# PeterouZh/CIPS-3D

Measured on AMD Instinct MI355X. Metric: rendered imgs/sec (G fwd+bwd), higher is better.
Workload: dtype f32 (dense layers as 3-pass split-operand MFMA with fp32 accumulate: SIREN forward on fp16 hi/lo planes, ~2e-7 rel., sigma in the fp32 class; INR head and all backward GEMMs on bf16 hi/lo planes, ~5e-6 rel. per layer; everything else fp32); 1 GPU; FFHQ r64, 24 SIREN evals/ray (num_steps 24, hierarchical False), batch 32/GPU, G fwd+bwd, all 9 CIPS blocks; global_batch=32, parallelism=dp1, rccl_ranks=0, inr_gemm_mode=bf16x3, launch=hipGraph replay, grad_reduce=none

## Files before the change

cips3d_amd/_lib.py:

```python
import ctypes as C
import os

_HERE = os.path.dirname(os.path.abspath(__file__))
LIB_PATH = os.path.join(_HERE, "lib", "libcips3d_hip.so")

vp = C.c_void_p
i32 = C.c_int
i64 = C.c_longlong
f32 = C.c_float


class SirenWeights(C.Structure):
    _fields_ = [(n, vp) for n in
                ("w0", "b0", "w1", "b1", "ws", "bs", "wc", "bc", "wf", "bf",
                 "g0", "p0", "g1", "p1", "gc", "pc")] + [("box_scale", f32), ("trig_mode", i32)]


class SirenGrads(C.Structure):
    _fields_ = [(n, vp) for n in ("dg0", "dp0", "dg1", "dp1", "dgc", "dpc", "dw0", "db0", "dw1", "db1", "dws", "dbs", "dwc",
                                  "dbc", "dwf", "dbf")]


class RayParams(C.Structure):
    _fields_ = [("xg", vp), ("yg", vp), ("zg", vp), ("cam2world", vp), ("jitter", vp), ("zvals", vp), ("zc", f32), ("H", i32),
                ("W", i32), ("S", i32)]


class GlinJob(C.Structure):
    _fields_ = [("x", vp), ("w", vp), ("bias", vp), ("y", vp), ("dy", vp), ("dw", vp), ("db", vp), ("in_dim", i32),
                ("out_dim", i32)]


class GemmDesc(C.Structure):
    _fields_ = [
        ("A", vp), ("B", vp), ("C", vp),
        ("M", i32), ("N", i32), ("K", i32),
        ("lda", i32), ("ldb", i32), ("ldc", i32),
        ("strideA", i64), ("strideB", i64), ("strideC", i64),
        ("batch", i32), ("a_kmajor", i32), ("b_nmajor", i32),
        ("alpha", f32), ("bias", vp), ("bias_m", vp),
        ("act", i32), ("slope", f32), ("act_gain", f32),
        ("resid", vp), ("C2", vp), ("add", vp),
        ("rgb_g", vp), ("rgb_w", vp), ("C_unmasked", vp), ("mask", vp),
    ]


class ModfcPrepJob(C.Structure):
    _fields_ = [("weight", C.c_void_p), ("s", C.c_void_p), ("wb_hi", C.c_void_p), ("wb_lo", C.c_void_p),
                ("wbt_hi", C.c_void_p), ("wbt_lo", C.c_void_p), ("demod", C.c_void_p), ("in_dim", C.c_int),
                ("out_dim", C.c_int)]


class ModfcBwdJob(C.Structure):
    _fields_ = [("weight", C.c_void_p), ("s", C.c_void_p), ("demod", C.c_void_p), ("gwb", C.c_void_p),
                ("cbuf", C.c_void_p), ("dweight", C.c_void_p), ("ds", C.c_void_p), ("in_dim", C.c_int),
                ("out_dim", C.c_int)]


class GemmX3Desc(C.Structure):
    _fields_ = [
        ("A_hi", vp), ("A_lo", vp), ("B_hi", vp), ("B_lo", vp),
        ("M", i32), ("N", i32), ("K", i32), ("lda", i32), ("ldb", i32),
        ("strideA", i64), ("strideB", i64), ("batch", i32),
        ("C", vp), ("ldc", i32), ("strideC", i64),
        ("P_hi", vp), ("P_lo", vp), ("ldp", i32), ("strideP", i64),
        ("T_hi", vp), ("T_lo", vp), ("ldt", i32), ("strideT", i64),
        ("mask_out", vp), ("add", vp), ("rgb_g", vp), ("rgb_w", vp), ("C_unmasked", vp), ("mask", vp),
        ("act", i32), ("slope", f32), ("res_hi", vp), ("res_lo", vp), ("gate_bits", i32),
        ("torgb_w", vp), ("torgb_part", vp),
        ("addp_hi", vp), ("addp_lo", vp), ("addp_gate", vp), ("addp_gain", f32),
        ("kernel", i32),
    ]


class ConvX3Desc(C.Structure):
    _fields_ = [("w_hi", vp), ("w_lo", vp), ("x_hi", vp), ("x_lo", vp), ("y", vp),
                ("B", i32), ("C", i32), ("H", i32), ("W", i32), ("O", i32), ("kh", i32), ("kw", i32),
                ("stride", i32), ("pad", i32), ("ksplit", i32), ("part", vp), ("bias", vp), ("act", i32), ("slope", f32),
                ("act_scale", f32)]


class ConvDgradS2Desc(C.Structure):
    _fields_ = [("w_hi", vp), ("w_lo", vp), ("dy_hi", vp), ("dy_lo", vp), ("dxp", vp),
                ("B", i32), ("C", i32), ("H", i32), ("W", i32), ("O", i32), ("kh", i32), ("kw", i32),
                ("w_off", i64 * 4), ("out_off", i64 * 4)]


class WPrepJob(C.Structure):
    _fields_ = [("w", vp), ("fwd_hi", vp), ("fwd_lo", vp), ("alt_hi", vp), ("alt_lo", vp), ("scale", f32),
                ("O", i32), ("C", i32), ("kh", i32), ("kw", i32), ("alt_kind", i32), ("bank_off", i32 * 4)]


class ConvWgradDesc(C.Structure):
    _fields_ = [("dy_hi", vp), ("dy_lo", vp), ("x_hi", vp), ("x_lo", vp), ("part", vp),
                ("B", i32), ("C", i32), ("H", i32), ("W", i32), ("O", i32), ("kh", i32), ("kw", i32),
                ("stride", i32), ("pad", i32), ("nchunks", i32)]


SIGNATURES = {
    "cips_version": (i32, []),
    "cips_arch": (C.c_char_p, []),
    "cips_rays_fwd": (i32, [vp, vp, vp, f32, vp, vp, vp, vp, vp, i32, i32, i32, i32, vp]),
    "cips_siren_fwd": (i32, [C.POINTER(SirenWeights), vp, vp, vp, i32, i32, vp]),
    "cips_siren_fwd_x3": (i32, [C.POINTER(SirenWeights), vp, vp, vp, i32, i32, vp]),
    "cips_siren_bwd_rows": (i32, [i32, i32]),
    "cips_siren_bwd_x3_chunks": (i32, [i32, i32]),
    "cips_siren_bwd_x3_gpart": (i32, []),
    "cips_siren_bwd_x3_sred": (i32, []),
    "cips_siren_bwd_x3": (i32, [C.POINTER(SirenWeights), vp, vp, vp, vp, vp, i32, i32, vp]),
    "cips_siren_fwd_x3_rays": (i32, [C.POINTER(SirenWeights), C.POINTER(RayParams), vp, vp, vp, i32, vp]),
    "cips_siren_bwd_x3_rays": (i32, [C.POINTER(SirenWeights), C.POINTER(RayParams), vp, vp, vp, vp, i32, vp]),
    "cips_siren_bwd_x3_finalize": (i32, [C.POINTER(SirenWeights), vp, vp, i32, i32, C.POINTER(SirenGrads), vp]),
    "cips_march_fwd_x3": (i32, [C.POINTER(SirenWeights), C.POINTER(RayParams), vp, f32, i32, i32, vp, vp, vp, vp, vp, vp, i32, vp, vp, vp]),
    "cips_siren_bwd_data": (i32, [C.POINTER(SirenWeights)] + [vp] * 14 + [i32, i32, vp]),
    "cips_siren_bwd_data_f32": (i32, [C.POINTER(SirenWeights)] + [vp] * 9 + [i32, i32, vp]),
    "cips_resample_fwd": (i32, [vp, vp, vp, f32, vp, vp, vp, vp, vp, vp, vp, vp, i32, i32, i32, i32, vp, C.POINTER(RayParams), vp]),
    "cips_composite_fwd": (i32, [vp, vp, vp, vp, vp, vp, vp, f32, vp, vp, vp, vp, vp, i32, i32, i32, i32, vp, vp, vp]),
    "cips_composite_bwd": (i32, [vp, vp, vp, vp, vp, vp, vp, f32, vp, vp, vp, vp, vp, vp, i32, i32, i32, i32, vp, vp]),
    "cips_gemm_f32": (i32, [C.POINTER(GemmDesc), vp]),
    "cips_gemm_bf16x3": (i32, [C.POINTER(GemmX3Desc), vp]),
    "cips_gemm_bf16x3_fuses_torgb": (i32, [C.POINTER(GemmX3Desc)]),
    "cips_gemm_bf16x3_takes_addp": (i32, [C.POINTER(GemmX3Desc)]),
    "cips_torgb_finish": (i32, [vp, i32, vp, vp, i64, i32, vp]),
    "cips_equal_linear_scratch": (i64, [i32, i32, i32, i32]),
    "cips_equal_linear": (i32, [i32, vp, vp, vp, f32, f32, vp, vp, i32, i32, i32, vp]),
    "cips_gemm_bf16x3_km": (i32, [C.POINTER(GemmX3Desc), vp]),
    "cips_gemm_bf16x3_km_grouped": (i32, [C.POINTER(GemmX3Desc), i32, vp]),
    "cips_gemm_bf16": (i32, [C.POINTER(GemmX3Desc), vp]),
    "cips_gemm_bf16_fuses_torgb": (i32, [C.POINTER(GemmX3Desc)]),
    "cips_gemm_bf16_takes_addp": (i32, [C.POINTER(GemmX3Desc)]),
    "cips_gemm_bf16_km": (i32, [C.POINTER(GemmX3Desc), vp]),
    "cips_gemm_bf16_km_grouped": (i32, [C.POINTER(GemmX3Desc), i32, vp]),
    "cips_lrelu_bwd_bias_slices": (i32, [i32]),
    "cips_lrelu_bwd_bias": (i32, [vp, vp, vp, vp, i64, i32, f32, f32, vp]),
    "cips_lrelu_bwd_bias_finish": (i32, [vp, vp, i32, i32, i32, vp]),
    "cips_lrelu_bwd_bias_nhwc_tiles": (i32, [i32]),
    "cips_lrelu_bwd_bias_nhwc": (i32, [vp, vp, vp, vp, vp, i32, i32, i32, f32, f32, vp]),
    "cips_conv1x1_smallk": (i32, [vp, vp, vp, i32, i32, i32, i32, vp]),
    "cips_conv1x1_smallk_bwd_data": (i32, [vp, vp, vp, i32, i32, i32, i32, vp]),
    "cips_conv1x1_smallk_bwd_weight_splits": (i32, [i32, i32]),
    "cips_conv1x1_smallk_bwd_weight": (i32, [vp, vp, vp, i32, i32, i32, i32, vp]),
    "cips_conv2d_x3": (i32, [C.POINTER(ConvX3Desc), vp]),
    "cips_conv2d_x3_wgrad": (i32, [C.POINTER(ConvWgradDesc), vp]),
    "cips_split_planes": (i32, [vp, vp, vp, vp, vp, i32, i32, i32, i32, i32, i32, i64, i64, i64, vp]),
    "cips_split_planes_nhwc": (i32, [vp, vp, vp, i32, i32, i32, vp]),
    "cips_conv2d_x3_ksplit": (i32, [i32, i32, i32, i32]),
    "cips_conv_weight_prep_max_jobs": (i32, []),
    "cips_conv_weight_prep_batch": (i32, [C.POINTER(WPrepJob), i32, vp]),
    "cips_conv2d_x3_dgrad_s2": (i32, [C.POINTER(ConvDgradS2Desc), vp]),
    "cips_conv_wgrad_finish": (i32, [vp, vp, i32, i32, i32, i32, f32, vp]),
    "cips_modfc_prep_x3": (i32, [vp, vp, vp, vp, vp, vp, vp, i32, i32, i32, f32, vp]),
    "cips_torgb_fwd_x3": (i32, [vp, vp, vp, vp, vp, i64, i32, i32, vp]),
    "cips_torgb_bwd_w_x3": (i32, [vp, vp, vp, vp, vp, vp, i64, i32, vp]),
    "cips_modfc_prep": (i32, [vp, vp, vp, vp, vp, i32, i32, i32, f32, vp]),
    "cips_modfc_prep_bwd": (i32, [vp, vp, vp, vp, vp, vp, vp, i32, i32, i32, vp]),
    "cips_modfc_max_jobs": (i32, []),
    "cips_modfc_prep_x3_batch": (i32, [C.POINTER(ModfcPrepJob), i32, i32, C.c_float, vp]),
    "cips_modfc_prep_bwd_batch": (i32, [C.POINTER(ModfcBwdJob), i32, i32, vp]),
    "cips_modfc_prep_bwd_batch_cores": (i32, [C.POINTER(ModfcBwdJob), i32, i32, vp]),
    "cips_cores_colsum_parts": (i32, []),
    "cips_opt_chunk": (i32, []),
    "cips_opt_step": (i32, [vp, vp, vp, i32, vp, vp, f32, f32, f32, f32, f32, f32, i32, vp, vp]),
    "cips_camera_pose": (i32, [vp, vp, i32, f32, f32, f32, f32, vp, vp, vp, i32, vp]),
    "cips_grouped_linear_max_jobs": (i32, []),
    "cips_grouped_linear_fwd": (i32, [C.POINTER(GlinJob), i32, i32, vp]),
    "cips_grouped_linear_scratch": (i64, [C.POINTER(GlinJob), i32, i32]),
    "cips_grouped_linear_bwd": (i32, [C.POINTER(GlinJob), i32, i32, vp, vp, i64, vp]),
    "cips_rownorm_fwd": (i32, [vp, vp, vp, vp, vp, i32, i32, i32, f32, vp]),
    "cips_rownorm_bwd": (i32, [vp] * 9 + [i32, i32, i32, f32, vp]),
    "cips_torgb_fwd": (i32, [vp, vp, vp, vp, i64, i32, i32, vp]),
    "cips_torgb_bwd_partials": (i32, [i64]),
    "cips_torgb_bwd_w": (i32, [vp, vp, vp, vp, vp, i64, i32, vp]),
    "cips_torgb_bwd_x": (i32, [vp, vp, vp, vp, f32, vp, vp, i64, i32, vp]),
    "cips_torgb_bwd_w_x3_batch": (i32, [vp, vp, i32, vp, vp, vp, vp, i64, i32, vp]),
    "cips_torgb_bwd_w_x3_batch_cores": (i32, [vp, vp, i32, vp, vp, vp, vp, i64, i32, vp]),
    "cips_torgb_bwd_x_x3": (i32, [vp, vp, vp, f32, vp, vp, vp, i64, i32, vp]),
    "cips_fused_bias_act": (i32, [vp, vp, vp, vp, i64, i32, i32, i32, i32, f32, f32, vp]),
    "cips_diffaug": (i32, [vp] * 10 + [i32] * 8 + [vp]),
    "cips_avgpool2": (i32, [vp, vp, i64, i32, i32, i32, vp]),
    "cips_axpby": (i32, [vp, vp, vp, f32, f32, i64, vp]),
    "cips_image_to_u8": (i32, [vp, vp, i32, i32, i32, i32, f32, f32, vp]),
    "cips_upfirdn2d": (i32, [vp, vp, vp] + [i32] * 14 + [vp]),
    "cips_upfirdn2d_parity": (i32, [vp, C.POINTER(i64 * 4), vp, vp] + [i32] * 7 + [vp]),
    "cips_im2col": (i32, [vp, vp] + [i32] * 8 + [vp]),
    "cips_im2col_x3": (i32, [vp, vp, vp, i32, i32, i32, i32, i32, i32, i32, i32, vp]),
    "cips_col2im": (i32, [vp, vp] + [i32] * 8 + [vp]),
}

_lib = None


def load():
    global _lib
    if _lib is not None:
        return _lib
    if not os.path.exists(LIB_PATH):
        raise RuntimeError(
            f"cips3d_amd: HIP extension not built ({LIB_PATH} missing). "
            "Run `python -m cips3d_amd.build` (needs hipcc). There is no CPU fallback.")
    lib = C.CDLL(LIB_PATH)
    for name, (res, args) in SIGNATURES.items():
        try:
            fn = getattr(lib, name)
        except AttributeError as e:
            raise RuntimeError(f"cips3d_amd: symbol {name} missing from {LIB_PATH}") from e
        fn.restype = res
        fn.argtypes = args
    _lib = lib
    return lib


def check(err, what):
    if err != 0:
        raise RuntimeError(f"cips3d_amd: {what} failed with hipError {err}")
```

cips3d_amd/csrc/render.hip:

```cpp
#include "common.h"
#include "../../include/cips3d_hip.h"
#include "raygen.h"

namespace {

__global__ __launch_bounds__(256) void rays_kernel(const float* __restrict__ xg, const float* __restrict__ yg,
                                                   const float* __restrict__ zg, float zc,
                                                   const float* __restrict__ c2w, const float* __restrict__ jitter,
                                                   float* __restrict__ points, float* __restrict__ zout,
                                                   float* __restrict__ dirs, int B, int H, int W, int S) {
  const long long total = (long long)B * H * W * S;
  const int n = H * W;
  for (long long idx = (long long)blockIdx.x * blockDim.x + threadIdx.x; idx < total;
       idx += (long long)gridDim.x * blockDim.x) {
    const int i = (int)(idx % S);
    const long long rr = idx / S;
    const int ray = (int)(rr % n);
    const int b = (int)(rr / n);
    const int row = ray / W, col = ray % W;
    const float x = xg[col], y = yg[row];
    const float nrm = sqrtf(x * x + y * y + zc * zc);
    const float dx = x / nrm, dy = y / nrm, dz = zc / nrm;
    float z = zg[i];
    float px = dx * z, py = dy * z, pz = dz * z;
    if (jitter) {
      const float off = (jitter[idx] - 0.5f) * (zg[1] - zg[0]);
      z = z + off;
      px = px + off * dx; py = py + off * dy; pz = pz + off * dz;
    }
    const float* M = c2w + (long long)b * 16;
    points[idx * 3 + 0] = ((M[0] * px + M[1] * py) + M[2] * pz) + M[3];
    points[idx * 3 + 1] = ((M[4] * px + M[5] * py) + M[6] * pz) + M[7];
    points[idx * 3 + 2] = ((M[8] * px + M[9] * py) + M[10] * pz) + M[11];
    zout[idx] = z;
    if (i == 0) {
      dirs[rr * 3 + 0] = (M[0] * dx + M[1] * dy) + M[2] * dz;
      dirs[rr * 3 + 1] = (M[4] * dx + M[5] * dy) + M[6] * dz;
      dirs[rr * 3 + 2] = (M[8] * dx + M[9] * dy) + M[10] * dz;
    }
  }
}

__device__ __forceinline__ float clamp_density(float x, int mode) {
  if (mode == 1) return (x > 20.f) ? x : log1pf(expf(x));
  return fmaxf(x, 0.f);
}
__device__ __forceinline__ float clamp_density_grad(float x, int mode) {
  if (mode == 1) return (x > 20.f) ? 1.f : 1.f / (1.f + expf(-x));
  return x > 0.f ? 1.f : 0.f;
}

struct ResampleArgs {
  const float *sigma, *z, *noise, *u, *origins, *dirs;
  const float* cdf_in;
  RayGen rg;
  int have_rg;
  float noise_std;
  float *fine_z, *fine_pts, *weights_out, *cdf_out;
  long long* inds_out;
  int B, n, S, clamp_mode;
};

constexpr int SEG = 8;

__global__ __launch_bounds__(256) void resample_kernel(ResampleArgs a) {
  extern __shared__ __attribute__((aligned(16))) float sm[];
  const int S = a.S;
  const int rays_per_block = blockDim.x / SEG;
  const int lr = threadIdx.x / SEG, sub = threadIdx.x % SEG;
  const long long R = (long long)a.B * a.n;
  const long long ray_raw = (long long)blockIdx.x * rays_per_block + lr;
  const bool active = ray_raw < R;
  const long long ray = active ? ray_raw : R - 1;
  float* zs = sm + lr * (4 * S);
  float* ws = zs + S;
  float* cdf = ws + S;
  float* bins = cdf + S;

  for (int i = sub; i < S; i += SEG) {
    zs[i] = a.z[ray * S + i];
    float sg = a.sigma[ray * S + i];
    if (a.noise) sg += a.noise[ray * S + i] * a.noise_std;
    ws[i] = sg;
  }
  __syncthreads();
  if (sub == 0) {
    double T = 1.0;
    for (int i = 0; i < S; ++i) {
      const float delta = (i + 1 < S) ? (zs[i + 1] - zs[i]) : 1e10f;
      const float dens = clamp_density(ws[i], a.clamp_mode);
      const float alpha = 1.f - expf(-delta * dens);
      const float Tf = (float)T;
      T *= (double)(1.f - alpha + 1e-10f);
      ws[i] = alpha * Tf;
    }
    float sum = 0.f;
    for (int k = 0; k < S - 2; ++k) sum += (ws[k + 1] + 1e-5f) + 1e-5f;
    double acc = 0.0;
    cdf[0] = 0.f;
    for (int k = 0; k < S - 2; ++k) {
      const float pdf = ((ws[k + 1] + 1e-5f) + 1e-5f) / sum;
      acc += (double)pdf;
      cdf[k + 1] = (float)acc;
    }
    for (int j = 0; j < S - 1; ++j) bins[j] = 0.5f * (zs[j] + zs[j + 1]);
    if (a.cdf_in)
      for (int j = 0; j < S - 1; ++j) cdf[j] = a.cdf_in[ray * (S - 1) + j];
  }
  __syncthreads();
  const int b = (int)(ray / a.n);
  float ox, oy, oz, dx, dy, dz;
  if (a.have_rg) {
    const float* M = a.rg.c2w + (long long)b * 16;
    const RayDir d = ray_dir(a.rg, (int)(ray - (long long)b * a.n));
    dx = (M[0] * d.dx + M[1] * d.dy) + M[2] * d.dz;
    dy = (M[4] * d.dx + M[5] * d.dy) + M[6] * d.dz;
    dz = (M[8] * d.dx + M[9] * d.dy) + M[10] * d.dz;
    ox = M[3]; oy = M[7]; oz = M[11];
  } else {
    ox = a.origins[b * 3 + 0]; oy = a.origins[b * 3 + 1]; oz = a.origins[b * 3 + 2];
    dx = a.dirs[ray * 3 + 0]; dy = a.dirs[ray * 3 + 1]; dz = a.dirs[ray * 3 + 2];
  }
  for (int i = sub; i < S; i += SEG) {
    const float u = a.u[ray * S + i];
    int ind = 0;
    for (int j = 0; j < S - 1; ++j) ind += (cdf[j] < u) ? 1 : 0;
    const int below = max(ind - 1, 0);
    const int above = min(ind, S - 2);
    const float c0 = cdf[below], c1 = cdf[above];
    const float b0 = bins[below], b1 = bins[above];
    float denom = c1 - c0;
    if (denom < 1e-5f) denom = 1.f;
    const float smp = b0 + (u - c0) / denom * (b1 - b0);
    if (!active) continue;
    a.fine_z[ray * S + i] = smp;
    if (a.fine_pts) {
      float* fp = a.fine_pts + (ray * S + i) * 3;
      fp[0] = ox + dx * smp; fp[1] = oy + dy * smp; fp[2] = oz + dz * smp;
    }
    if (a.inds_out) a.inds_out[ray * S + i] = ind;
    if (a.weights_out) a.weights_out[ray * S + i] = ws[i];
  }
  if (a.cdf_out && active)
    for (int j = sub; j < S - 1; j += SEG) a.cdf_out[ray * (S - 1) + j] = cdf[j];
}

struct CompArgs {
  const float *feat_c, *sig_c, *z_c, *feat_f, *sig_f, *z_f, *noise;
  float noise_std;
  float *fea, *depth, *weights, *zsorted;
  int* order;
  const int* order_in;
  const float* dfea;
  float *dfeat_c, *dsig_c, *dfeat_f, *dsig_f;
  long long R;
  int S, E, clamp_mode, flags;
  const unsigned char* clamp_pin;
  unsigned char* clamp_rec;
};

__device__ __forceinline__ bool clamp_pass(const CompArgs& a, float x, long long idx, bool store) {
  bool pass = x > 0.f;
  if (a.clamp_pin) pass = a.clamp_pin[idx] != 0;
  if (a.clamp_rec && store) a.clamp_rec[idx] = pass ? 1 : 0;
  return pass;
}

__device__ __forceinline__ const float* feat_row(const CompArgs& a, long long ray, int i) {
  if (a.feat_f) return (i < a.S) ? a.feat_f + (ray * a.S + i) * 32 : a.feat_c + (ray * a.S + (i - a.S)) * 32;
  return a.feat_c + (ray * a.S + i) * 32;
}

__global__ __launch_bounds__(256) void composite_fwd_kernel(CompArgs a) {
  extern __shared__ __attribute__((aligned(16))) float sm[];
  const int S = a.S, E = a.E;
  const int rays_per_block = blockDim.x / SEG;
  const int lr = threadIdx.x / SEG, sub = threadIdx.x % SEG;
  const long long ray_raw = (long long)blockIdx.x * rays_per_block + lr;
  const bool active = ray_raw < a.R;
  const long long ray = active ? ray_raw : a.R - 1;
  float* zall = sm + lr * (4 * E);
  float* sall = zall + E;
  int* ord = reinterpret_cast<int*>(sall + E);

  for (int i = sub; i < E; i += SEG) {
    if (a.feat_f) {
      zall[i] = (i < S) ? a.z_f[ray * S + i] : a.z_c[ray * S + (i - S)];
      sall[i] = (i < S) ? a.sig_f[ray * S + i] : a.sig_c[ray * S + (i - S)];
    } else {
      zall[i] = a.z_c[ray * S + i];
      sall[i] = a.sig_c[ray * S + i];
      ord[i] = i;
    }
  }
  __syncthreads();
  if (a.feat_f) {
    for (int i = sub; i < E; i += SEG) {
      const float zi = zall[i];
      int rank = 0;
      for (int j = 0; j < E; ++j) {
        const float zj = zall[j];
        rank += (zj < zi || (zj == zi && j < i)) ? 1 : 0;
      }
      ord[rank] = i;
    }
  }
  __syncthreads();

  float* al = reinterpret_cast<float*>(ord + E);
  for (int k = sub; k < E; k += SEG) {
    const int i = ord[k];
    const float zk = zall[i];
    const float delta = (k + 1 < E) ? (zall[ord[k + 1]] - zk) : 1e10f;
    float sg = sall[i];
    if (a.noise) sg += a.noise[ray * E + k] * a.noise_std;
    float dens = clamp_density(sg, a.clamp_mode);
    if ((a.clamp_pin || a.clamp_rec) && a.clamp_mode == 0) dens = clamp_pass(a, sg, ray * E + k, active) ? sg : 0.f;
    al[k] = 1.f - expf(-delta * dens);
  }
  __syncthreads();

  float4 F = make_float4(0.f, 0.f, 0.f, 0.f);
  float depth = 0.f, wsum = 0.f, wlast = 0.f, zlast = 0.f;
  float4 flast = make_float4(0.f, 0.f, 0.f, 0.f);
  double T = 1.0;
  for (int k0 = 0; k0 < E; k0 += 8) {
    float4 f[8];
#pragma unroll
    for (int j = 0; j < 8; ++j) {
      const int k = (k0 + j < E) ? k0 + j : E - 1;
      f[j] = *reinterpret_cast<const float4*>(feat_row(a, ray, ord[k]) + 4 * sub);
    }
#pragma unroll
    for (int j = 0; j < 8; ++j) {
      const int k = k0 + j;
      if (k < E) {
        const int i = ord[k];
        const float zk = zall[i];
        const float alpha = al[k];
        const float w = alpha * (float)T;
        T *= (double)(1.f - alpha + 1e-10f);
        F.x = fmaf(w, f[j].x, F.x); F.y = fmaf(w, f[j].y, F.y); F.z = fmaf(w, f[j].z, F.z); F.w = fmaf(w, f[j].w, F.w);
        depth = fmaf(w, zk, depth);
        wsum += w;
        if (k == E - 1) { wlast = w; zlast = zk; flast = f[j]; }
        if ((k % SEG) == sub && active) {
          if (a.weights && !(k == E - 1 && (a.flags & 1))) a.weights[ray * E + k] = w;
          if (a.order) a.order[ray * E + k] = i;
          if (a.zsorted) a.zsorted[ray * E + k] = zk;
        }
      }
    }
  }
  if (a.flags & 1) {
    const float extra = 1.f - wsum;
    F.x = fmaf(extra, flast.x, F.x); F.y = fmaf(extra, flast.y, F.y);
    F.z = fmaf(extra, flast.z, F.z); F.w = fmaf(extra, flast.w, F.w);
    depth = fmaf(extra, zlast, depth);
    if (a.weights && ((E - 1) % SEG) == sub && active) a.weights[ray * E + E - 1] = wlast + extra;
  }
  if (a.flags & 2) {
    const float extra = 1.f - wsum;
    F.x += extra; F.y += extra; F.z += extra; F.w += extra;
  }
  if (active) {
    *reinterpret_cast<float4*>(a.fea + ray * 32 + 4 * sub) = F;
    if (sub == 0 && a.depth) a.depth[ray] = depth;
  }
}

__global__ __launch_bounds__(256) void composite_bwd_kernel(CompArgs a) {
  extern __shared__ __attribute__((aligned(16))) float sm[];
  const int S = a.S, E = a.E;
  const int rays_per_block = blockDim.x / SEG;
  const int lr = threadIdx.x / SEG, sub = threadIdx.x % SEG;
  const long long ray_raw = (long long)blockIdx.x * rays_per_block + lr;
  const bool active = ray_raw < a.R;
  const long long ray = active ? ray_raw : a.R - 1;
  float* zall = sm + lr * (6 * E);
  float* xs = zall + E;
  float* Ts = xs + E;
  float* al = Ts + E;
  float* ss = al + E;
  int* ord = reinterpret_cast<int*>(ss + E);

  for (int k = sub; k < E; k += SEG) {
    const int i = a.order_in ? a.order_in[ray * E + k] : k;
    ord[k] = i;
    float zz, sg;
    if (a.feat_f) {
      zz = (i < S) ? a.z_f[ray * S + i] : a.z_c[ray * S + (i - S)];
      sg = (i < S) ? a.sig_f[ray * S + i] : a.sig_c[ray * S + (i - S)];
    } else {
      zz = a.z_c[ray * S + i];
      sg = a.sig_c[ray * S + i];
    }
    if (a.noise) sg += a.noise[ray * E + k] * a.noise_std;
    zall[k] = zz;
    xs[k] = sg;
  }
  __syncthreads();

  const float4 G = *reinterpret_cast<const float4*>(a.dfea + ray * 32 + 4 * sub);
  float gsum = G.x + G.y + G.z + G.w;
  gsum += __shfl_xor(gsum, 1);
  gsum += __shfl_xor(gsum, 2);
  gsum += __shfl_xor(gsum, 4);
  float wsum = 0.f;
  double T = 1.0;
  for (int k = 0; k < E; ++k) {
    const float delta = (k + 1 < E) ? (zall[k + 1] - zall[k]) : 1e10f;
    float dens = clamp_density(xs[k], a.clamp_mode);
    if (a.clamp_pin && a.clamp_mode == 0) dens = a.clamp_pin[ray * E + k] ? xs[k] : 0.f;
    const float alpha = 1.f - expf(-delta * dens);
    const float Tf = (float)T;
    wsum += alpha * Tf;
    T *= (double)(1.f - alpha + 1e-10f);
    const float4 f = *reinterpret_cast<const float4*>(feat_row(a, ray, ord[k]) + 4 * sub);
    float s = G.x * f.x + G.y * f.y + G.z * f.z + G.w * f.w;
    s += __shfl_xor(s, 1);
    s += __shfl_xor(s, 2);
    s += __shfl_xor(s, 4);
    if (sub == 0) { Ts[k] = Tf; al[k] = alpha; ss[k] = s; }
  }
  __syncthreads();
  float Q = 0.f;
  const float s_off = ((a.flags & 1) ? ss[E - 1] : 0.f) + ((a.flags & 2) ? gsum : 0.f);
  for (int k = E - 1; k >= 0; --k) {
    const int i = ord[k];
    const float alpha = al[k], Tk = Ts[k], s = ss[k] - s_off;
    float w = alpha * Tk;
    if ((a.flags & 1) && k == E - 1) w += 1.f - wsum;

    const float dalpha = Tk * (s - Q);
    Q = fmaf(alpha, s, (1.f - alpha + 1e-10f) * Q);
    float* drow;
    float* dsg;
    if (a.feat_f) {
      drow = (i < S) ? a.dfeat_f + (ray * S + i) * 32 : a.dfeat_c + (ray * S + (i - S)) * 32;
      dsg = (i < S) ? a.dsig_f + ray * S + i : a.dsig_c + ray * S + (i - S);
    } else {
      drow = a.dfeat_c + (ray * S + i) * 32;
      dsg = a.dsig_c + ray * S + i;
    }
    if (active) *reinterpret_cast<float4*>(drow + 4 * sub) = make_float4(w * G.x, w * G.y, w * G.z, w * G.w);
    if ((k % SEG) == sub && active) {
      const float delta = (k + 1 < E) ? (zall[k + 1] - zall[k]) : 1e10f;
      const float x = xs[k];
      float dens = clamp_density(x, a.clamp_mode);
      float dgrad = clamp_density_grad(x, a.clamp_mode);
      if (a.clamp_pin && a.clamp_mode == 0) {
        const bool pass = a.clamp_pin[ray * E + k] != 0;
        dens = pass ? x : 0.f;
        dgrad = pass ? 1.f : 0.f;
      }
      *dsg = dalpha * (delta * expf(-delta * dens)) * dgrad;
    }
  }
}

inline int rays_per_block_for(size_t bytes_per_ray) {
  int r = 32;
  while (r > 1 && (size_t)r * bytes_per_ray > 60 * 1024) r >>= 1;
  return r;
}

}

extern "C" int cips_rays_fwd(const float* xg, const float* yg, const float* zg, float zc,
                             const float* cam2world, const float* jitter, float* points, float* z,
                             float* dirs, int B, int H, int W, int S, cips_stream_t stream) {
  if (B <= 0 || H <= 0 || W <= 0 || S <= 1) return (int)hipErrorInvalidValue;
  long long total = (long long)B * H * W * S;
  int blocks = (int)((total + 255) / 256 < 8192 ? (total + 255) / 256 : 8192);
  hipLaunchKernelGGL(rays_kernel, dim3(blocks), dim3(256), 0, (hipStream_t)stream, xg, yg, zg, zc,
                     cam2world, jitter, points, z, dirs, B, H, W, S);
  return CIPS_CHECK_LAUNCH();
}

extern "C" int cips_resample_fwd(const float* sigma, const float* z, const float* noise, float noise_std,
                                 const float* u, const float* origins, const float* dirs, float* fine_z,
                                 float* fine_pts, float* weights_out, float* cdf_out, long long* inds_out,
                                 int B, int n, int S, int clamp_mode, const float* cdf_in, const cips_ray_params* rays,
                                 cips_stream_t stream) {
  if (B <= 0 || n <= 0 || S < 3 || !fine_z || (!rays && (!origins || !dirs || !fine_pts))) return (int)hipErrorInvalidValue;
  ResampleArgs a;
  a.cdf_in = cdf_in;
  a.rg = RayGen{}; a.have_rg = 0;
  if (rays) { const int rc = fill_raygen(a.rg, rays); if (rc) return rc; if (a.rg.n != n) return (int)hipErrorInvalidValue; a.have_rg = 1; }
  a.sigma = sigma; a.z = z; a.noise = noise; a.noise_std = noise_std; a.u = u; a.origins = origins;
  a.dirs = dirs; a.fine_z = fine_z; a.fine_pts = fine_pts; a.weights_out = weights_out;
  a.cdf_out = cdf_out; a.inds_out = inds_out; a.B = B; a.n = n; a.S = S; a.clamp_mode = clamp_mode;
  size_t per_ray = (size_t)4 * S * sizeof(float);
  int rpb = rays_per_block_for(per_ray);
  long long R = (long long)B * n;
  int blocks = (int)((R + rpb - 1) / rpb);
  hipLaunchKernelGGL(resample_kernel, dim3(blocks), dim3(rpb * SEG), rpb * per_ray, (hipStream_t)stream, a);
  return CIPS_CHECK_LAUNCH();
}

extern "C" int cips_composite_fwd(const float* feat_c, const float* sig_c, const float* z_c,
                                  const float* feat_f, const float* sig_f, const float* z_f,
                                  const float* noise, float noise_std, float* fea, float* depth,
                                  float* weights, int* order, float* zsorted, int R, int S,
                                  int clamp_mode, int flags, const unsigned char* clamp_in, unsigned char* clamp_out,
                                  cips_stream_t stream) {
  if (R <= 0 || S <= 0) return (int)hipErrorInvalidValue;
  CompArgs a = {};
  a.feat_c = feat_c; a.sig_c = sig_c; a.z_c = z_c; a.feat_f = feat_f; a.sig_f = sig_f; a.z_f = z_f;
  a.noise = noise; a.noise_std = noise_std; a.fea = fea; a.depth = depth; a.weights = weights;
  a.order = order; a.zsorted = zsorted; a.R = R; a.S = S; a.E = feat_f ? 2 * S : S;
  a.clamp_mode = clamp_mode; a.flags = flags;
  a.clamp_pin = clamp_in; a.clamp_rec = clamp_out;
  size_t per_ray = (size_t)4 * a.E * sizeof(float);
  int rpb = rays_per_block_for(per_ray);
  int blocks = (R + rpb - 1) / rpb;
  hipLaunchKernelGGL(composite_fwd_kernel, dim3(blocks), dim3(rpb * SEG), rpb * per_ray, (hipStream_t)stream, a);
  return CIPS_CHECK_LAUNCH();
}

extern "C" int cips_composite_bwd(const float* feat_c, const float* sig_c, const float* z_c,
                                  const float* feat_f, const float* sig_f, const float* z_f,
                                  const float* noise, float noise_std, const int* order, const float* dfea,
                                  float* dfeat_c, float* dsig_c, float* dfeat_f, float* dsig_f, int R, int S,
                                  int clamp_mode, int flags, const unsigned char* clamp_in, cips_stream_t stream) {
  if (R <= 0 || S <= 0 || (!order && feat_f)) return (int)hipErrorInvalidValue;
  CompArgs a = {};
  a.feat_c = feat_c; a.sig_c = sig_c; a.z_c = z_c; a.feat_f = feat_f; a.sig_f = sig_f; a.z_f = z_f;
  a.noise = noise; a.noise_std = noise_std; a.order_in = order; a.dfea = dfea;
  a.dfeat_c = dfeat_c; a.dsig_c = dsig_c; a.dfeat_f = dfeat_f; a.dsig_f = dsig_f;
  a.R = R; a.S = S; a.E = feat_f ? 2 * S : S; a.clamp_mode = clamp_mode; a.flags = flags;
  a.clamp_pin = clamp_in; a.clamp_rec = nullptr;
  size_t per_ray = (size_t)6 * a.E * sizeof(float);
  int rpb = rays_per_block_for(per_ray);
  int blocks = (R + rpb - 1) / rpb;
  hipLaunchKernelGGL(composite_bwd_kernel, dim3(blocks), dim3(rpb * SEG), rpb * per_ray, (hipStream_t)stream, a);
  return CIPS_CHECK_LAUNCH();
}
```

cips3d_amd/csrc/siren_bwd_x3.hip:

```cpp
#include "common.h"
#include "../../include/cips3d_hip.h"
#include "raygen.h"
#include <type_traits>

#ifdef CIPS_X3_PRIO
#define X3_PRIO(p) __builtin_amdgcn_s_setprio(p)
#else
#define X3_PRIO(p)
#endif

namespace {

typedef __bf16 bf16x8 __attribute__((ext_vector_type(8)));
typedef __bf16 bf16x2 __attribute__((ext_vector_type(2)));
typedef float f32x2 __attribute__((ext_vector_type(2)));
typedef short short4v __attribute__((ext_vector_type(4)));
typedef unsigned int u32x4 __attribute__((ext_vector_type(4)));
typedef unsigned char uchar;

constexpr int H = 128, HC = 64, CF = 32;

constexpr int O_W1H = 0, O_W1L = 32768;
constexpr int O_WCH = 65536, O_WCL = 81920;
constexpr int O_WFH = 98304, O_WFL = 102400;
// ... 151 lines not shown
    acc[m] = __builtin_amdgcn_mfma_f32_32x32x16_bf16(ah, bh, acc[m], 0, 0, 0);
    __builtin_amdgcn_sched_barrier(0);
    side(3 * it + 2);
    __builtin_amdgcn_sched_barrier(0);
  }
}

__device__ __forceinline__ unsigned opaque(unsigned v) { asm volatile("" : "+v"(v)); return v; }

struct LaneAddr {
  unsigned fb[2][2];
  unsigned tb[2][2];
  unsigned sb[2];
  unsigned ab;
  unsigned v16, v64;
};
__device__ __forceinline__ LaneAddr lane_addr(int lane, unsigned sbase) {
  const int l31 = lane & 31, hf = lane >> 5, s16 = lane & 15, mhalf = (lane >> 4) & 1;
  const int ul = 4 * mhalf + (s16 & 3);
  LaneAddr A;
  const int e = hf ^ ((l31 >> 2) & 7);
#pragma unroll
  for (int t = 0; t < 2; ++t)
#pragma unroll
    for (int sec = 0; sec < 2; ++sec) {
      A.fb[t][sec] = sbase + l31 * 64 + ((e ^ (4 * t) ^ (2 * sec)) << 3);
      A.tb[t][sec] = sbase + (4 * hf + (s16 >> 2)) * 64 + (((ul ^ hf) ^ (4 * t) ^ (2 * sec)) << 3);
    }
  const int gs = 4 * hf + (s16 >> 3);
  A.sb[0] = opaque(sbase + O_STG + (8 * hf + (s16 >> 2)) * 64 + ((ul ^ gs) << 3));
  A.sb[1] = opaque(sbase + O_STG + (8 * hf + (s16 >> 2)) * 64 + ((ul ^ gs ^ 2) << 3));
  A.ab = opaque(sbase + O_AUX + (8 * hf + (s16 >> 2)) * 16 + (s16 & 1) * 8);
  A.v16 = opaque(sbase + O_L0 + 16 * hf);
  A.v64 = opaque(sbase + O_L0 + 64 * hf);
  return A;
}

template <int NM, int Q, int R, int IMG, int PLANE, bool F16 = false>
__device__ __forceinline__ void layer_fwd(const LaneAddr& A, const Act<Q>& in, f32x16 (&acc)[NM]) {
  const unsigned b[2][2] = {{opaque(A.fb[0][0] + IMG), opaque(A.fb[0][1] + IMG)}, {opaque(A.fb[1][0] + IMG), opaque(A.fb[1][1] + IMG)}};
  auto load = [&](int s, int m, Frag& f) {
    const int c = (s >> 1) * R * 64 + m * 2048;
    put(f.h, 0, lds_b64(b[s & 1][0] + c));
    put(f.h, 2, lds_b64(b[s & 1][1] + c));
    put(f.l, 0, lds_b64(b[s & 1][0] + c + PLANE));
    put(f.l, 2, lds_b64(b[s & 1][1] + c + PLANE));
  };
  run_layer<NM, 2 * Q, F16>(load, in, acc);
}

template <int NM, int Q, int R, int IMG, int PLANE, typename SideF>
__device__ __forceinline__ void layer_fwd_mm(const LaneAddr& A, const Act<Q>& in, f32x16 (&acc)[NM], SideF side) {
  const unsigned b[2][2] = {{opaque(A.fb[0][0] + IMG), opaque(A.fb[0][1] + IMG)}, {opaque(A.fb[1][0] + IMG), opaque(A.fb[1][1] + IMG)}};
  auto load = [&](int s, int m, Frag& f) {
    const int c = (s >> 1) * R * 64 + m * 2048;
    put(f.h, 0, lds_b64(b[s & 1][0] + c));
    put(f.h, 2, lds_b64(b[s & 1][1] + c));
    put(f.l, 0, lds_b64(b[s & 1][0] + c + PLANE));
    put(f.l, 2, lds_b64(b[s & 1][1] + c + PLANE));
  };
  run_layer_mm<NM, 2 * Q>(load, in, acc, side);
}

template <int NM, int KS, int R, int IMG, int PLANE>
__device__ __forceinline__ void layer_tr(const LaneAddr& A, const Act<(KS + 1) / 2>& in, f32x16 (&acc)[NM]) {
  const unsigned b[2][2] = {{opaque(A.tb[0][0] + IMG), opaque(A.tb[0][1] + IMG)}, {opaque(A.tb[1][0] + IMG), opaque(A.tb[1][1] + IMG)}};
  auto load = [&](int ks, int m, Frag& f) {
    const int c = m * R * 64 + ks * 1024;
    put(f.h, 0, lds_tr(b[ks & 1][0] + c));
    put(f.h, 2, lds_tr(b[ks & 1][1] + c + 512));
    put(f.l, 0, lds_tr(b[ks & 1][0] + c + PLANE));
    put(f.l, 2, lds_tr(b[ks & 1][1] + c + 512 + PLANE));
  };
  run_layer<NM, KS>(load, in, acc);
}

template <int NM, int KS, int R, int IMG, int PLANE, typename SideF>
__device__ __forceinline__ void layer_tr_mm(const LaneAddr& A, const Act<(KS + 1) / 2>& in, f32x16 (&acc)[NM], SideF side) {
  const unsigned b[2][2] = {{opaque(A.tb[0][0] + IMG), opaque(A.tb[0][1] + IMG)}, {opaque(A.tb[1][0] + IMG), opaque(A.tb[1][1] + IMG)}};
  auto load = [&](int ks, int m, Frag& f) {
    const int c = m * R * 64 + ks * 1024;
    put(f.h, 0, lds_tr(b[ks & 1][0] + c));
    put(f.h, 2, lds_tr(b[ks & 1][1] + c + 512));
    put(f.l, 0, lds_tr(b[ks & 1][0] + c + PLANE));
    put(f.l, 2, lds_tr(b[ks & 1][1] + c + 512 + PLANE));
  };
  run_layer_mm<NM, KS>(load, in, acc, side);
}

template <int Q, int R, int HI, int LO>
__device__ __forceinline__ void stage(unsigned sbase, int row, int hf, const Act<Q>& v) {
  const unsigned rb = opaque(sbase + O_STG + row * 64);
  const int g = (row >> 1) & 7;
#pragma unroll
  for (int gg = 0; gg < 4; ++gg) {
    const unsigned o = rb + (((2 * gg + hf) ^ g) << 3);
#pragma unroll
    for (int q = 0; q < Q; ++q) {
      lds_st64(o + HI + q * R * 64, v.hi[q][2 * gg], v.hi[q][2 * gg + 1]);
      lds_st64(o + LO + q * R * 64, v.lo[q][2 * gg], v.lo[q][2 * gg + 1]);
    }
  }
}

template <int R, int HI, int LO>
__device__ __forceinline__ void stg_frag(unsigned sb0, unsigned sb1, int col0, int ks, Frag& f) {
  const int c = (col0 >> 5) * R * 64 + ks * 1024;
  put(f.h, 0, lds_tr(sb0 + HI + c)); put(f.h, 2, lds_tr(sb1 + HI + c + 256));
  put(f.l, 0, lds_tr(sb0 + LO + c)); put(f.l, 2, lds_tr(sb1 + LO + c + 256));
}
__device__ __forceinline__ f32x16 x3f(f32x16 acc, const Frag& a, const Frag& b) {
  return x3(acc, mk8(a.h[0], a.h[1], a.h[2], a.h[3]), mk8(a.l[0], a.l[1], a.l[2], a.l[3]),
            mk8(b.h[0], b.h[1], b.h[2], b.h[3]), mk8(b.l[0], b.l[1], b.l[2], b.l[3]));
}

template <bool HW>
__device__ __forceinline__ void bsincos(float x, float* s, float* c) {
  if (HW) {
    float rv = x * CIPS_INV_2PI;
    rv = rv - rintf(rv);
    *s = __builtin_amdgcn_sinf(rv);
    *c = __builtin_amdgcn_cosf(rv);
  } else {
    sincos_reduced(reduce_2pi(x), s, c);
  }
}

__device__ __forceinline__ void aux_frag(unsigned ab, int ks, unsigned mask, Frag& f) {
  const int c = ks * 256;
  put(f.h, 0, lds_tr(ab + c)); put(f.h, 2, lds_tr(ab + c + 64));
  put(f.l, 0, lds_tr(ab + c + 2048)); put(f.l, 2, lds_tr(ab + c + 2048 + 64));
#pragma unroll
  for (int i = 0; i < 4; ++i) { f.h[i] &= mask; f.l[i] &= mask; }
}
__device__ __forceinline__ f32x16 x2f(f32x16 acc, const Frag& a, const Frag& b) {
  const bf16x8 bh = mk8(b.h[0], b.h[1], b.h[2], b.h[3]);
  acc = __builtin_amdgcn_mfma_f32_32x32x16_bf16(mk8(a.l[0], a.l[1], a.l[2], a.l[3]), bh, acc, 0, 0, 0);
  acc = __builtin_amdgcn_mfma_f32_32x32x16_bf16(mk8(a.h[0], a.h[1], a.h[2], a.h[3]), bh, acc, 0, 0, 0);
  return acc;
}
__device__ __forceinline__ float4 ld4(const float* p) { return *reinterpret_cast<const float4*>(p); }

struct BwdX3Args {
  cips_siren_weights w;
  const float* points;
  const float* dfeat;
  const float* dsigma;
  float* sred;
  float* gpart;
  int B, P, chunk, chunks;
  unsigned long long* prof;
  int dbg;
  RayGen rg;
};
constexpr int GP_G1 = 0, GP_GC = H * H, GP_GF0 = GP_GC + HC * H, GP_GF1 = GP_GF0 + CF * HC, GPART = GP_GF1 + CF * HC;
constexpr int SRED = 4 * 32 * 8 + 8;

__device__ __forceinline__ float pow2_scale_for(float m, int& k) {
  const unsigned u = __float_as_uint(m);
  const int e = (int)((u >> 23) & 0xffu) - 127;
  k = 13 - e;
  if (!(m > 0.f) || e == 128) k = 0;
  k = k > 100 ? 100 : (k < -100 ? -100 : k);
  return __uint_as_float((unsigned)(k + 127) << 23);
}
template <bool PRE = false, bool F16 = false>
__device__ __forceinline__ void stage_weights_x3(uchar* sm, const cips_siren_weights& w, int b) {
  const int tid = threadIdx.x, nt = blockDim.x;
  const float pre = PRE ? CIPS_INV_2PI : 1.f;
  float s1 = 1.f, sc = 1.f, sf = 1.f, i1 = 1.f, ic = 1.f, isf = 1.f;
  if constexpr (F16) {
    float m1 = 0.f, mc = 0.f, mf = 0.f;
    for (int i = tid; i < H * 32; i += nt) {
      const float4 v = *reinterpret_cast<const float4*>(w.w1 + 4 * i);
      m1 = fmaxf(fmaxf(m1, fmaxf(fabsf(v.x), fabsf(v.y))), fmaxf(fabsf(v.z), fabsf(v.w)));
    }
    for (int i = tid; i < HC * 32; i += nt) {
      const float4 v = *reinterpret_cast<const float4*>(w.wc + 4 * i);
      mc = fmaxf(fmaxf(mc, fmaxf(fabsf(v.x), fabsf(v.y))), fmaxf(fabsf(v.z), fabsf(v.w)));
    }
    for (int i = tid; i < CF * 16; i += nt) {
      const float4 v = *reinterpret_cast<const float4*>(w.wf + 4 * i);
      mf = fmaxf(fmaxf(mf, fmaxf(fabsf(v.x), fabsf(v.y))), fmaxf(fabsf(v.z), fabsf(v.w)));
    }
#pragma unroll
    for (int o = 32; o > 0; o >>= 1) {
      m1 = fmaxf(m1, __shfl_xor(m1, o)); mc = fmaxf(mc, __shfl_xor(mc, o)); mf = fmaxf(mf, __shfl_xor(mf, o));
    }
    float* red = reinterpret_cast<float*>(sm + O_W1H);
    const int wv = tid >> 6, nw = nt >> 6;
    if ((tid & 63) == 0) { red[3 * wv] = m1; red[3 * wv + 1] = mc; red[3 * wv + 2] = mf; }
    __syncthreads();
    m1 = 0.f; mc = 0.f; mf = 0.f;
    for (int i = 0; i < nw; ++i) { m1 = fmaxf(m1, red[3 * i]); mc = fmaxf(mc, red[3 * i + 1]); mf = fmaxf(mf, red[3 * i + 2]); }
    __syncthreads();
    int k1, kc, kf;
    s1 = pow2_scale_for(m1 * pre, k1); sc = pow2_scale_for(mc * pre, kc); sf = pow2_scale_for(mf, kf);
    i1 = __uint_as_float((unsigned)(127 - k1) << 23); ic = __uint_as_float((unsigned)(127 - kc) << 23);
    isf = __uint_as_float((unsigned)(127 - kf) << 23);
  }
  for (int i = tid; i < H * 32; i += nt) {
    const int row = i >> 5, u = i & 31;
    float4 v = *reinterpret_cast<const float4*>(w.w1 + row * H + 4 * u);
    if (PRE) { v.x *= pre; v.y *= pre; v.z *= pre; v.w *= pre; }
    if (F16) { v.x *= s1; v.y *= s1; v.z *= s1; v.w *= s1; }
    uint2 ph, pl;
    split2t<F16>(v.x, v.y, ph.x, pl.x); split2t<F16>(v.z, v.w, ph.y, pl.y);
    const int o = img_addr<2>(row, u, H);
    *reinterpret_cast<uint2*>(sm + O_W1H + o) = ph;
    *reinterpret_cast<uint2*>(sm + O_W1L + o) = pl;
  }
  for (int i = tid; i < HC * 32; i += nt) {
    const int row = i >> 5, u = i & 31;
    float4 v = *reinterpret_cast<const float4*>(w.wc + row * H + 4 * u);
    if (PRE) { v.x *= pre; v.y *= pre; v.z *= pre; v.w *= pre; }
    if (F16) { v.x *= sc; v.y *= sc; v.z *= sc; v.w *= sc; }
    uint2 ph, pl;
    split2t<F16>(v.x, v.y, ph.x, pl.x); split2t<F16>(v.z, v.w, ph.y, pl.y);
    const int o = img_addr<2>(row, u, HC);
    *reinterpret_cast<uint2*>(sm + O_WCH + o) = ph;
    *reinterpret_cast<uint2*>(sm + O_WCL + o) = pl;
  }
  for (int i = tid; i < CF * 16; i += nt) {
    const int row = i >> 4, u = i & 15;
    float4 v = *reinterpret_cast<const float4*>(w.wf + row * HC + 4 * u);
    if (F16) { v.x *= sf; v.y *= sf; v.z *= sf; v.w *= sf; }
    uint2 ph, pl;
    split2t<F16>(v.x, v.y, ph.x, pl.x); split2t<F16>(v.z, v.w, ph.y, pl.y);
    const int o = img_addr<2>(row, u, CF);
    *reinterpret_cast<uint2*>(sm + O_WFH + o) = ph;
    *reinterpret_cast<uint2*>(sm + O_WFL + o) = pl;
  }
  float* L0 = reinterpret_cast<float*>(sm + O_L0);
  float* G1 = reinterpret_cast<float*>(sm + O_G1); float* C1 = reinterpret_cast<float*>(sm + O_C1);
  float* WS = reinterpret_cast<float*>(sm + O_WS);
  float* GC = reinterpret_cast<float*>(sm + O_GC); float* CC = reinterpret_cast<float*>(sm + O_CC);
  for (int f = tid; f < H; f += nt) {
    const float g0 = w.g0[b * H + f], gs = g0 * w.box_scale;
    float4 pk;
    pk.x = gs * w.w0[f * 3 + 0]; pk.y = gs * w.w0[f * 3 + 1]; pk.z = gs * w.w0[f * 3 + 2];
    pk.w = fmaf(g0, w.b0[f], w.p0[b * H + f]);
    if (PRE) { pk.x *= pre; pk.y *= pre; pk.z *= pre; pk.w *= pre; }
    reinterpret_cast<float4*>(L0)[f] = pk;
    const float g1 = w.g1[b * H + f];
    G1[f] = F16 ? g1 * i1 : g1; C1[f] = fmaf(g1, w.b1[f], w.p1[b * H + f]) * pre; WS[f] = w.ws[f];
  }
  for (int f = tid; f < HC; f += nt) {
    const float gc = w.gc[b * HC + f];
    GC[f] = F16 ? gc * ic : gc; CC[f] = fmaf(gc, w.bc[f], w.pc[b * HC + f]) * pre;
  }
  if (F16 && tid == 0) *reinterpret_cast<float*>(sm + O_AUX + 128) = isf;
}

#ifdef CIPS_TUNING
#define X3_TS(i)                                                                                   \
  __builtin_amdgcn_sched_barrier(0);                                                               \
  if (a.prof && blockIdx.x == 0 && blockIdx.y == 0 && lane0 == 0 && rnd < 8)                       \
    a.prof[(rnd * 4 + wave) * 16 + (i)] = __builtin_amdgcn_s_memtime();                            \
  __builtin_amdgcn_sched_barrier(0);
#else
#define X3_TS(i) __builtin_amdgcn_sched_barrier(0);
#endif

#include "siren_bwd_x4.inc"
#define X3F_TS(i)


struct FwdX3Args {
  cips_siren_weights w;
  const float* points;
  float* feat;
  float* sigma;
  float* zout;
  RayGen rg;
  int B, P, chunk;
};

template <bool HW, bool F16>
__global__ __launch_bounds__(512) void siren_fwd_x3_kernel(FwdX3Args a) {
  extern __shared__ __attribute__((aligned(1024))) uchar smem[];
  const int b = blockIdx.y;
  stage_weights_x3<HW, F16>(smem, a.w, b);
  if (threadIdx.x < CF) reinterpret_cast<float*>(smem + O_AUX)[threadIdx.x] = a.w.bf[threadIdx.x];
  __syncthreads();
  const int lane0 = threadIdx.x & 63, wave = __builtin_amdgcn_readfirstlane(threadIdx.x >> 6);
  const unsigned sbase = (unsigned)(uintptr_t)((__attribute__((address_space(3))) uchar*)smem);
  const float bs = a.w.bs[0];
  const float isf = F16 ? reinterpret_cast<const float*>(smem + O_AUX)[32] : 1.f;
  const int cstart = blockIdx.x * a.chunk;
  const int cend = min(cstart + a.chunk, a.P);
  for (int pbase = cstart + wave * 32; pbase < cend; pbase += 8 * 32) {
    int lane = lane0;
    asm volatile("" : "+v"(lane));
    const int l31 = lane & 31, hf = lane >> 5;
    const LaneAddr LA = lane_addr(lane, sbase);
    const int p = pbase + l31;
    const bool valid = p < cend;
    const long long gp = (long long)b * a.P + (valid ? p : cend - 1);
    float px, py, pz, zpt = 0.f;
    if (a.points) { px = a.points[gp * 3 + 0]; py = a.points[gp * 3 + 1]; pz = a.points[gp * 3 + 2]; }
    else gen_point(a.rg, b, valid ? p : cend - 1, px, py, pz, zpt);

#include "siren_fwd_chain.inc"
    if (valid) {
      float* fo = a.feat + gp * CF + 4 * hf;
      const float* bfv = reinterpret_cast<const float*>(smem + O_AUX);
// ... 135 lines not shown
          if (a.weights && !(s == S - 1 && (a.flags & 1))) a.weights[rs + s] = w;
        }
      }
      wx = nx; wy = ny; wz = nz; zs = zn;
      X3F_TS(7)
      __builtin_amdgcn_sched_barrier(0);
    }
    if (a.flags & 1) {
      const float extra = 1.f - wsum;
#pragma unroll
      for (int r = 0; r < 16; ++r) F[r] = fmaf(extra, flast[r], F[r]);
      depth = fmaf(extra, zlast, depth);
      if (a.weights && valid && hfs == 0) a.weights[rs + S - 1] = wlast + extra;
    }
    if (a.flags & 2) {
      const float extra = 1.f - wsum;
#pragma unroll
      for (int r = 0; r < 16; ++r) F[r] += extra;
    }
    if (valid) {
      float* o = a.fea + ((long long)b * n + ray) * CF + 4 * hfs;
#pragma unroll
      for (int gq = 0; gq < 4; ++gq)
        *reinterpret_cast<float4*>(o + 8 * gq) = make_float4(F[4 * gq], F[4 * gq + 1], F[4 * gq + 2], F[4 * gq + 3]);
      if (hfs == 0 && a.depth) a.depth[(long long)b * n + ray] = depth;
    }
  }
}

struct FinArgs {
  cips_siren_weights w;
  const float* sred; const float* gpart;
  cips_siren_grads o;
  int B, chunks;
};

__global__ __launch_bounds__(128) void siren_bwd_finalize_kernel(FinArgs a) {
  __shared__ float cols[8];
  __shared__ float red[128];
  const int task = blockIdx.x, j = threadIdx.x;
  const int B = a.B, C = a.chunks;
  auto colsum = [&](int b, int f, int col) {
    float s = 0.f;
    const float* p = a.sred + (long long)b * C * SRED + (f >> 5) * 256 + (f & 31) * 8 + col;
    for (int c = 0; c < C; ++c) s += p[(long long)c * SRED];
    return s;
  };
  auto block_sum = [&](float v) {
    red[j] = v;
    __syncthreads();
    for (int s_ = 64; s_ > 0; s_ >>= 1) {
      if (j < s_) red[j] += red[j + s_];
      __syncthreads();
    }
    const float r = red[0];
    __syncthreads();
    return r;
  };
  if (task < 192) {
    const bool l1 = task < 128;
    const int f = l1 ? task : task - 128;
    const int goff = l1 ? GP_G1 : GP_GC;
    const float* Wrow = (l1 ? a.w.w1 : a.w.wc) + f * H;
    const float* gain = l1 ? a.w.g1 : a.w.gc;
    const int gdim = l1 ? H : HC;
    const float bias = l1 ? a.w.b1[f] : a.w.bc[f];
    const float wj = Wrow[j];
    float acc_w = 0.f, acc_b = 0.f, acc_ws = 0.f, acc_b0 = 0.f, acc_w0[3] = {0.f, 0.f, 0.f};
    for (int b = 0; b < B; ++b) {
      float v = 0.f;
      const float* gp = a.gpart + (long long)b * C * GPART + goff + f * H + j;
      for (int c = 0; c < C; ++c) v += gp[(long long)c * GPART];
      const float gn = gain[b * gdim + f];
      acc_w = fmaf(gn, v, acc_w);
      if (j < 8) cols[j] = colsum(b, f, j);
      const float dot = block_sum(v * wj);
      if (j == 0) {
        const float dph = l1 ? cols[4] : cols[6];
        (l1 ? a.o.dp1 : a.o.dpc)[b * gdim + f] = dph;
        (l1 ? a.o.dg1 : a.o.dgc)[b * gdim + f] = fmaf(bias, dph, dot);
        acc_b = fmaf(gn, dph, acc_b);
        if (l1) {
          const float dp0 = cols[0], g0 = a.w.g0[b * H + f];
          float s0[3], dg0 = a.w.b0[f] * dp0;
#pragma unroll
          for (int c = 0; c < 3; ++c) { s0[c] = cols[1 + c] * a.w.box_scale; dg0 = fmaf(s0[c], a.w.w0[f * 3 + c], dg0); acc_w0[c] = fmaf(g0, s0[c], acc_w0[c]); }
          a.o.dp0[b * H + f] = dp0;
          a.o.dg0[b * H + f] = dg0;
          acc_b0 = fmaf(g0, dp0, acc_b0);
          acc_ws += cols[5];
        }
      }
      __syncthreads();
    }
    (l1 ? a.o.dw1 : a.o.dwc)[f * H + j] = acc_w;
    if (j == 0) {
      (l1 ? a.o.db1 : a.o.dbc)[f] = acc_b;
      if (l1) {
        a.o.db0[f] = acc_b0; a.o.dws[f] = acc_ws;
        a.o.dw0[f * 3 + 0] = acc_w0[0]; a.o.dw0[f * 3 + 1] = acc_w0[1]; a.o.dw0[f * 3 + 2] = acc_w0[2];
      }
    }
  } else if (task < 224) {
    const int ch = task - 192;
    if (j < HC) {
      float v = 0.f;
      for (int b = 0; b < B; ++b) {
        float vb = 0.f;
        const float* gp = a.gpart + (long long)b * C * GPART + ch * HC + j;
        for (int c = 0; c < C; ++c) vb += gp[(long long)c * GPART + GP_GF0] + gp[(long long)c * GPART + GP_GF1];
        v += vb;
      }
      a.o.dwf[ch * HC + j] = v;
    }
    if (j == 0) {
      float s = 0.f;
      for (int b = 0; b < B; ++b) s += colsum(b, ch, 7) + colsum(b, 64 + ch, 7);
      a.o.dbf[ch] = s;
    }
  } else if (j == 0) {
    float s = 0.f;
    for (int b = 0; b < B; ++b)
      for (int c = 0; c < C; ++c) {
        const float* p = a.sred + ((long long)b * C + c) * SRED + 1024;
        s += (p[0] + p[1]) + (p[2] + p[3]);
      }
    a.o.dbs[0] = s;
  }
}

}

static int x3_chunk(int B, int P) {
  int chunk = 4096;
  while (chunk > 512 && (long long)B * ((P + chunk - 1) / chunk) < 768) chunk >>= 1;
  return chunk;
}
extern "C" int cips_siren_bwd_x3_chunks(int B, int P) {
  const int chunk = x3_chunk(B, P);
  return (P + chunk - 1) / chunk;
}
extern "C" int cips_siren_bwd_x3_gpart(void) { return GPART; }
#ifdef CIPS_TUNING
static unsigned long long* g_prof = nullptr;
extern "C" int cips_siren_bwd_x3_prof(unsigned long long* host_out) {
  if (!g_prof) return (int)hipErrorNotReady;
  return (int)hipMemcpy(host_out, g_prof, 8 * 4 * 16 * 8, hipMemcpyDeviceToHost);
}
#endif
extern "C" int cips_siren_bwd_x3_sred(void) { return SRED; }


static int siren_bwd_x3_launch(const cips_siren_weights* w, const float* points, const cips_ray_params* rays,
                               const float* dfeat, const float* dsigma, float* sred, float* gpart, int B, int P,
                               cips_stream_t stream);

extern "C" int cips_siren_bwd_x3(const cips_siren_weights* w, const float* points, const float* dfeat,
                                 const float* dsigma, float* sred, float* gpart, int B, int P,
                                 cips_stream_t stream) {
  if (!points) return (int)hipErrorInvalidValue;
  return siren_bwd_x3_launch(w, points, nullptr, dfeat, dsigma, sred, gpart, B, P, stream);
}

extern "C" int cips_siren_bwd_x3_rays(const cips_siren_weights* w, const cips_ray_params* rays, const float* dfeat,
                                      const float* dsigma, float* sred, float* gpart, int B, cips_stream_t stream) {
  if (!rays) return (int)hipErrorInvalidValue;
  return siren_bwd_x3_launch(w, nullptr, rays, dfeat, dsigma, sred, gpart, B, rays->W * rays->H * rays->S, stream);
}

static int siren_bwd_x3_launch(const cips_siren_weights* w, const float* points, const cips_ray_params* rays,
                               const float* dfeat, const float* dsigma, float* sred, float* gpart, int B, int P,
                               cips_stream_t stream) {
  if (!w || !dfeat || !dsigma || !sred || !gpart || B <= 0 || P <= 0) return (int)hipErrorInvalidValue;
  BwdX3Args a;
  a.w = *w; a.points = points; a.dfeat = dfeat; a.dsigma = dsigma; a.sred = sred; a.gpart = gpart;
  a.B = B; a.P = P;
  a.rg = RayGen{};
  if (!points) { const int rc = fill_raygen(a.rg, rays); if (rc) return rc; }
  a.dbg = 0; a.prof = nullptr;
#ifdef CIPS_TUNING
  a.dbg = cips_tune_env("CIPS_X3_DBG", 0);
  static unsigned long long* prof = nullptr;
  static int want_prof = -1;
  if (want_prof < 0) {
    want_prof = cips_tune_env("CIPS_X3_PROF", 0) ? 1 : 0;
    if (want_prof && hipMalloc(&prof, 8 * 4 * 16 * 8) != hipSuccess) prof = nullptr;
  }
  a.prof = prof; g_prof = prof;
#endif
  a.chunk = x3_chunk(B, P);
  a.chunks = (P + a.chunk - 1) / a.chunk;
  dim3 grid(a.chunks, B);
  static bool attr4 = false;
  CIPS_PER_DEVICE(attr4, false);
  if (!attr4) {
    hipFuncSetAttribute((const void*)siren_bwd_x4_kernel<false>, hipFuncAttributeMaxDynamicSharedMemorySize, SMEM_BYTES);
    hipFuncSetAttribute((const void*)siren_bwd_x4_kernel<true>, hipFuncAttributeMaxDynamicSharedMemorySize, SMEM_BYTES);
    attr4 = true;
  }
  if (w->trig_mode & 1)
    hipLaunchKernelGGL(siren_bwd_x4_kernel<true>, grid, dim3(256), SMEM_BYTES, (hipStream_t)stream, a);
  else
    hipLaunchKernelGGL(siren_bwd_x4_kernel<false>, grid, dim3(256), SMEM_BYTES, (hipStream_t)stream, a);
  return CIPS_CHECK_LAUNCH();
}

static int siren_fwd_x3_launch(const cips_siren_weights* w, const float* points, const cips_ray_params* rays, float* feat,
                               float* sigma, float* zout, int B, int P, cips_stream_t stream);

extern "C" int cips_siren_fwd_x3(const cips_siren_weights* w, const float* points, float* feat, float* sigma, int B, int P,
                                 cips_stream_t stream) {
  if (!points) return (int)hipErrorInvalidValue;
  return siren_fwd_x3_launch(w, points, nullptr, feat, sigma, nullptr, B, P, stream);
}

extern "C" int cips_siren_fwd_x3_rays(const cips_siren_weights* w, const cips_ray_params* rays, float* feat, float* sigma,
                                      float* zout, int B, cips_stream_t stream) {
  if (!rays) return (int)hipErrorInvalidValue;
  return siren_fwd_x3_launch(w, nullptr, rays, feat, sigma, zout, B, rays->W * rays->H * rays->S, stream);
}

static int siren_fwd_x3_launch(const cips_siren_weights* w, const float* points, const cips_ray_params* rays, float* feat,
                               float* sigma, float* zout, int B, int P, cips_stream_t stream) {
  if (!w || !feat || !sigma || B <= 0 || P <= 0) return (int)hipErrorInvalidValue;
  FwdX3Args a;
  a.w = *w; a.points = points; a.feat = feat; a.sigma = sigma; a.zout = zout; a.B = B; a.P = P;
  a.rg = RayGen{};
  if (!points) { const int rc = fill_raygen(a.rg, rays); if (rc) return rc; }
  a.chunk = 4096;
  while (a.chunk > 512 && (long long)B * ((P + a.chunk - 1) / a.chunk) < 768) a.chunk >>= 1;
  dim3 grid((P + a.chunk - 1) / a.chunk, B);
  const int smem = O_STG;
  const bool hw = (w->trig_mode & 1) != 0, f16 = (w->trig_mode & 2) == 0;
  auto go = [&](auto HW_, auto F16_) {
    constexpr bool HW = decltype(HW_)::value, F16 = decltype(F16_)::value;
    static bool attr_set = false;
    CIPS_PER_DEVICE(attr_set, false);
    if (!attr_set) {
      (void)hipFuncSetAttribute((const void*)siren_fwd_x3_kernel<HW, F16>, hipFuncAttributeMaxDynamicSharedMemorySize, smem);
      attr_set = true;
    }
    hipLaunchKernelGGL((siren_fwd_x3_kernel<HW, F16>), grid, dim3(512), smem, (hipStream_t)stream, a);
  };
  using T = std::true_type; using F = std::false_type;
  if (hw) { if (f16) go(T{}, T{}); else go(T{}, F{}); }
  else { if (f16) go(F{}, T{}); else go(F{}, F{}); }
  return CIPS_CHECK_LAUNCH();
}

#ifdef CIPS_TUNING
static unsigned long long* g_mprof = nullptr;
extern "C" int cips_march_x3_prof(unsigned long long* host_out) {
  if (!g_mprof) return (int)hipErrorNotReady;
  return (int)hipMemcpy(host_out, g_mprof, 4 * 8 * 8 * 8, hipMemcpyDeviceToHost);
}
#endif
extern "C" int cips_march_fwd_x3(const cips_siren_weights* w, const cips_ray_params* rays, const float* noise,
                                 float noise_std, int clamp_mode, int flags, float* fea, float* depth, float* weights,
                                 float* feat, float* sigma, float* z, int B, const unsigned char* clamp_in,
                                 unsigned char* clamp_out, cips_stream_t stream) {
  if (!w || !fea || B <= 0) return (int)hipErrorInvalidValue;
  MarchArgs a;
  a.w = *w;
  const int rc = fill_raygen(a.rg, rays);
  if (rc) return rc;
  a.noise = noise; a.noise_std = noise_std; a.clamp_mode = clamp_mode; a.flags = flags;
  a.fea = fea; a.depth = depth; a.weights = weights; a.feat = feat; a.sigma = sigma; a.zout = z; a.B = B;
  a.clamp_pin = clamp_in; a.clamp_rec = clamp_out;
  a.desync = 0; a.one_wave = 0; a.prof = nullptr;
#ifdef CIPS_TUNING
  a.desync = cips_tune_env("CIPS_X3_MDESYNC", 0);
  a.one_wave = cips_tune_env("CIPS_X3_MONE", 0);
  if (cips_tune_env("CIPS_X3_MPROF", 0)) {
    if (!g_mprof && hipMalloc(&g_mprof, 4 * 8 * 8 * 8) != hipSuccess) g_mprof = nullptr;
    a.prof = g_mprof;
  }
#endif
  a.rays_per_wg = 256;
  const int n = a.rg.n;
  dim3 grid((n + a.rays_per_wg - 1) / a.rays_per_wg, B);
  const int smem = O_STG;
  const bool dbg = a.clamp_pin || a.clamp_rec;
  const bool hw = (w->trig_mode & 1) != 0, f16 = (w->trig_mode & 2) == 0;
  auto go = [&](auto HW_, auto DBG_, auto F16_) {
    constexpr bool HW = decltype(HW_)::value, DBG = decltype(DBG_)::value, F16 = decltype(F16_)::value;
    static bool attr_set = false;
    CIPS_PER_DEVICE(attr_set, false);
    if (!attr_set) {
      (void)hipFuncSetAttribute((const void*)siren_march_x3_kernel<HW, DBG, F16>, hipFuncAttributeMaxDynamicSharedMemorySize, smem);
      attr_set = true;
    }
    hipLaunchKernelGGL((siren_march_x3_kernel<HW, DBG, F16>), grid, dim3(512), smem, (hipStream_t)stream, a);
  };
  using T = std::true_type; using F = std::false_type;
  if (hw) {
    if (dbg) { if (f16) go(T{}, T{}, T{}); else go(T{}, T{}, F{}); }
    else { if (f16) go(T{}, F{}, T{}); else go(T{}, F{}, F{}); }
  } else {
    if (dbg) { if (f16) go(F{}, T{}, T{}); else go(F{}, T{}, F{}); }
    else { if (f16) go(F{}, F{}, T{}); else go(F{}, F{}, F{}); }
  }
  return CIPS_CHECK_LAUNCH();
}

extern "C" int cips_siren_bwd_x3_finalize(const cips_siren_weights* w, const float* sred, const float* gpart, int B,
                                          int chunks, const cips_siren_grads* out, cips_stream_t stream) {
  if (!w || !sred || !gpart || !out || B <= 0 || chunks <= 0) return (int)hipErrorInvalidValue;
  const float* const* po = reinterpret_cast<const float* const*>(out);
  for (int i = 0; i < 16; ++i) if (!po[i]) return (int)hipErrorInvalidValue;
  FinArgs a;
  a.w = *w; a.sred = sred; a.gpart = gpart; a.o = *out; a.B = B; a.chunks = chunks;
  hipLaunchKernelGGL(siren_bwd_finalize_kernel, dim3(225), dim3(128), 0, (hipStream_t)stream, a);
  return CIPS_CHECK_LAUNCH();
}
```

cips3d_amd/csrc/siren_bwd_x4.inc:

```
__device__ __forceinline__ void pinf(float& x) { asm volatile("" : "+v"(x)); }
__device__ __forceinline__ void pinf(float& a, float& b) { asm volatile("" : "+v"(a), "+v"(b)); }
__device__ __forceinline__ void pinf(float& a, float& b, float& c, float& d) { asm volatile("" : "+v"(a), "+v"(b), "+v"(c), "+v"(d)); }
__device__ __forceinline__ void pinu(unsigned& a, unsigned& b) { asm volatile("" : "+v"(a), "+v"(b)); }
__device__ __forceinline__ void pinu(unsigned& a, unsigned& b, unsigned& c, unsigned& d) { asm volatile("" : "+v"(a), "+v"(b), "+v"(c), "+v"(d)); }

template <bool HW> __device__ __forceinline__ float sin_rev(float x) {
  if (HW) return __builtin_amdgcn_sinf(__builtin_amdgcn_fractf(x));
  float s_, c_; sincos_reduced(reduce_2pi(x), &s_, &c_); return s_;
}

template <bool HW>
__global__ __launch_bounds__(256, 1) void siren_bwd_x4_kernel(BwdX3Args a) {
  extern __shared__ __attribute__((aligned(1024))) uchar smem[];
  const int b = blockIdx.y;
  stage_weights_x3<HW>(smem, a.w, b);
  __syncthreads();
  constexpr float TWO_PI = 6.283185307179586f;

  const int lane0 = threadIdx.x & 63, wave = __builtin_amdgcn_readfirstlane(threadIdx.x >> 6);
  const int cstart = blockIdx.x * a.chunk;
  const int cend = min(cstart + a.chunk, a.P);
  const unsigned sbase = (unsigned)(uintptr_t)((__attribute__((address_space(3))) uchar*)smem);

  f32x16 aG1[4], aGc[2], aGf[1], aS[1];
  zero_acc(aG1); zero_acc(aGc); zero_acc(aGf); zero_acc(aS);
  float r_dsg = 0.f;

  float px, py, pz, dsg;
  {
    const int p = cstart + wave * 32 + (lane0 & 31);
    const bool valid = p < cend;
    const long long gp = (long long)b * a.P + (valid ? p : cend - 1);
    if (a.points) { px = a.points[gp * 3 + 0]; py = a.points[gp * 3 + 1]; pz = a.points[gp * 3 + 2]; }
    else gen_point(a.rg, b, valid ? p : cend - 1, px, py, pz);
    dsg = valid ? a.dsigma[gp] : 0.f;
  }

  constexpr int NPRE = 0;
  Act<4> h1n;
  auto l0_groups = [&](auto G0c, auto G1c, float x, float y, float z) __attribute__((always_inline)) {
    constexpr int G0 = decltype(G0c)::value, G1 = decltype(G1c)::value;
    if (G0 >= G1) return;
    int ln = lane0;
    asm volatile("" : "+v"(ln));
    const unsigned sbase_ = (unsigned)(uintptr_t)((__attribute__((address_space(3))) uchar*)smem);
    const unsigned v64 = opaque(sbase_ + O_L0 + 64 * (ln >> 5));
    float4 pn[4];
#pragma unroll
    for (int e = 0; e < 4; ++e) pn[e] = lds_ld4(v64 + 128 * G0 + 16 * e);
#pragma unroll
    for (int grp = G0; grp < G1; ++grp) {
      float4 pk[4];
#pragma unroll
      for (int e = 0; e < 4; ++e) pk[e] = pn[e];
      if (grp + 1 < G1) {
#pragma unroll
        for (int e = 0; e < 4; ++e) pn[e] = lds_ld4(v64 + 128 * (grp + 1) + 16 * e);
      }
      __builtin_amdgcn_sched_barrier(0);
      float s4[4];
#pragma unroll
      for (int e = 0; e < 4; ++e) s4[e] = sin_rev<HW>(fmaf(pk[e].x, x, fmaf(pk[e].y, y, fmaf(pk[e].z, z, pk[e].w))));
      const int q = grp >> 2, g = grp & 3;
      split2(s4[0], s4[1], h1n.hi[q][2 * g], h1n.lo[q][2 * g]);
      split2(s4[2], s4[3], h1n.hi[q][2 * g + 1], h1n.lo[q][2 * g + 1]);
      pinu(h1n.hi[q][2 * g], h1n.lo[q][2 * g], h1n.hi[q][2 * g + 1], h1n.lo[q][2 * g + 1]);
      __builtin_amdgcn_sched_barrier(0);
    }
  };
  using IC0 = std::integral_constant<int, 0>; using ICA = std::integral_constant<int, (NPRE + 2) / 3>;
  using ICB = std::integral_constant<int, (2 * NPRE + 2) / 3>; using ICN = std::integral_constant<int, NPRE>;
  using IC16 = std::integral_constant<int, 16>;
  l0_groups(IC0{}, ICN{}, px, py, pz);

  int rnd = -1;
  for (int pbase = cstart; pbase < cend; pbase += 128) {
    ++rnd;
    X3_TS(0)
    int lane = lane0;
    asm volatile("" : "+v"(lane));
    const int l31 = lane & 31, hf = lane >> 5;
    const LaneAddr LA = lane_addr(lane, sbase);
    const int prow = wave * 32 + l31;
    const unsigned c7 = l31 & 7;
    const unsigned m_d1 = c7 < 4 ? ~0u : 0u, m_d2 = c7 == 4 ? ~0u : 0u, m_h2 = c7 == 5 ? ~0u : 0u;
    const unsigned m_dc = c7 == 6 ? ~0u : 0u, m_df = c7 == 7 ? ~0u : 0u;

    float4 df4[4];
    {
      const int p = pbase + prow;
      const bool valid = p < cend;
      const float* dp = a.dfeat + ((long long)b * a.P + (valid ? p : cend - 1)) * CF + 4 * hf;
#pragma unroll
      for (int g = 0; g < 4; ++g) df4[g] = valid ? ld4(dp + 8 * g) : make_float4(0.f, 0.f, 0.f, 0.f);
    }
    if (hf == 0) {
      uint4 ah, al;
      split2(1.f, px, ah.x, al.x); split2(py, pz, ah.y, al.y); split2(1.f, dsg, ah.z, al.z); split2(1.f, 1.f, ah.w, al.w);
      const u32x4 vh = {ah.x, ah.y, ah.z, ah.w}, vl = {al.x, al.y, al.z, al.w};
      *LDS_PTR(u32x4, sbase + O_AUX + prow * 16) = vh;
      *LDS_PTR(u32x4, sbase + O_AUX + 2048 + prow * 16) = vl;
      r_dsg += dsg;
    }

    const float dsg_s = HW ? dsg * CIPS_INV_2PI : dsg;

    f32x16 acc[4];
    zero_acc(acc);
    float cs2[4][16];
    Act<4> h2p;
    float rv[4], sn[4];
    float4 gq, cq;
    auto film2_slot = [&](int q, int g, int j) __attribute__((always_inline)) {
      const float gg[4] = {gq.x, gq.y, gq.z, gq.w}, cc[4] = {cq.x, cq.y, cq.z, cq.w};
      if (HW) {
        if (j == 0) {
#pragma unroll
          for (int e = 0; e < 4; ++e) rv[e] = fmaf(gg[e], acc[q][4 * g + e], cc[e]);
          rv[0] = __builtin_amdgcn_fractf(rv[0]); rv[1] = __builtin_amdgcn_fractf(rv[1]);
          pinf(rv[0], rv[1], rv[2], rv[3]);
        } else if (j == 1) {
          rv[2] = __builtin_amdgcn_fractf(rv[2]); rv[3] = __builtin_amdgcn_fractf(rv[3]);
          sn[0] = __builtin_amdgcn_sinf(rv[0]); sn[1] = __builtin_amdgcn_sinf(rv[1]);
          pinf(rv[2], rv[3], sn[0], sn[1]);
        } else if (j == 2) {
          cs2[q][4 * g + 0] = __builtin_amdgcn_cosf(rv[0]); cs2[q][4 * g + 1] = __builtin_amdgcn_cosf(rv[1]);
          sn[2] = __builtin_amdgcn_sinf(rv[2]);
          pinf(cs2[q][4 * g + 0], cs2[q][4 * g + 1]); pinf(sn[2]);
        } else if (j == 3) {
          sn[3] = __builtin_amdgcn_sinf(rv[3]);
          cs2[q][4 * g + 2] = __builtin_amdgcn_cosf(rv[2]); cs2[q][4 * g + 3] = __builtin_amdgcn_cosf(rv[3]);
          pinf(cs2[q][4 * g + 2], cs2[q][4 * g + 3]); pinf(sn[3]);
        }
      } else if (j == 0) {
#pragma unroll
        for (int e = 0; e < 4; ++e) bsincos<false>(fmaf(gg[e], acc[q][4 * g + e], cc[e]), &sn[e], &cs2[q][4 * g + e]);
        pinf(sn[0], sn[1], sn[2], sn[3]);
      }
      if (j == 4) { split2(sn[0], sn[1], h2p.hi[q][2 * g], h2p.lo[q][2 * g]); pinu(h2p.hi[q][2 * g], h2p.lo[q][2 * g]); }
      if (j == 5) {
        split2(sn[2], sn[3], h2p.hi[q][2 * g + 1], h2p.lo[q][2 * g + 1]);
        pinu(h2p.hi[q][2 * g + 1], h2p.lo[q][2 * g + 1]);
        if (4 * q + g + 1 < 16) {
          gq = lds_ld4(LA.v16 + (O_G1 - O_L0) + 32 * (4 * q + g + 1)); cq = lds_ld4(LA.v16 + (O_C1 - O_L0) + 32 * (4 * q + g + 1));
        }
      }
    };
    {
      l0_groups(ICN{}, IC16{}, px, py, pz);
      gq = lds_ld4(LA.v16 + (O_G1 - O_L0)); cq = lds_ld4(LA.v16 + (O_C1 - O_L0));
      layer_fwd_mm<4, 4, H, O_W1H, O_W1L - O_W1H>(LA, h1n, acc, [&](int slot) __attribute__((always_inline)) {
        const int m = slot / 24, j = slot % 24;
        if (m >= 1) film2_slot(m - 1, j / 6, j % 6);
      });
    }
    X3_TS(1)
#pragma unroll
    for (int j = 0; j < 6; ++j) { film2_slot(3, 0, j); __builtin_amdgcn_sched_barrier(0); }

    X3_TS(2)
    f32x16 accc[2];
    zero_acc(accc);
    float csc[2][16];
    Act<2> hcp;
    float4 gcq, ccq;
    auto filmc_slot = [&](int q, int g, int j) __attribute__((always_inline)) {
      const float gg[4] = {gcq.x, gcq.y, gcq.z, gcq.w}, cc[4] = {ccq.x, ccq.y, ccq.z, ccq.w};
      if (HW) {
        if (j == 0) {
#pragma unroll
          for (int e = 0; e < 4; ++e) rv[e] = fmaf(gg[e], accc[q][4 * g + e], cc[e]);
          rv[0] = __builtin_amdgcn_fractf(rv[0]); rv[1] = __builtin_amdgcn_fractf(rv[1]);
          pinf(rv[0], rv[1], rv[2], rv[3]);
        } else if (j == 1) {
          rv[2] = __builtin_amdgcn_fractf(rv[2]); rv[3] = __builtin_amdgcn_fractf(rv[3]);
          sn[0] = __builtin_amdgcn_sinf(rv[0]); sn[1] = __builtin_amdgcn_sinf(rv[1]);
          pinf(rv[2], rv[3], sn[0], sn[1]);
        } else if (j == 2) {
          csc[q][4 * g + 0] = __builtin_amdgcn_cosf(rv[0]); csc[q][4 * g + 1] = __builtin_amdgcn_cosf(rv[1]);
          sn[2] = __builtin_amdgcn_sinf(rv[2]);
          pinf(csc[q][4 * g + 0], csc[q][4 * g + 1]); pinf(sn[2]);
        } else if (j == 3) {
          sn[3] = __builtin_amdgcn_sinf(rv[3]);
          csc[q][4 * g + 2] = __builtin_amdgcn_cosf(rv[2]); csc[q][4 * g + 3] = __builtin_amdgcn_cosf(rv[3]);
          pinf(csc[q][4 * g + 2], csc[q][4 * g + 3]); pinf(sn[3]);
        }
      } else if (j == 0) {
#pragma unroll
        for (int e = 0; e < 4; ++e) bsincos<false>(fmaf(gg[e], accc[q][4 * g + e], cc[e]), &sn[e], &csc[q][4 * g + e]);
        pinf(sn[0], sn[1], sn[2], sn[3]);
      }
      if (j == 4) { split2(sn[0], sn[1], hcp.hi[q][2 * g], hcp.lo[q][2 * g]); pinu(hcp.hi[q][2 * g], hcp.lo[q][2 * g]); }
      if (j == 5) {
        split2(sn[2], sn[3], hcp.hi[q][2 * g + 1], hcp.lo[q][2 * g + 1]);
        pinu(hcp.hi[q][2 * g + 1], hcp.lo[q][2 * g + 1]);
        if (4 * q + g + 1 < 8) {
          gcq = lds_ld4(LA.v16 + (O_GC - O_L0) + 32 * (4 * q + g + 1)); ccq = lds_ld4(LA.v16 + (O_CC - O_L0) + 32 * (4 * q + g + 1));
        }
      }
    };
    gcq = lds_ld4(LA.v16 + (O_GC - O_L0)); ccq = lds_ld4(LA.v16 + (O_CC - O_L0));
    layer_fwd_mm<2, 4, HC, O_WCH, O_WCL - O_WCH>(LA, h2p, accc, [&](int slot) __attribute__((always_inline)) {
      if (slot < 18) film2_slot(3, 1 + slot / 6, slot % 6);
      else if (slot >= 24) filmc_slot(0, (slot - 24) / 6, (slot - 24) % 6);
    });
#pragma unroll
    for (int j = 0; j < 24; ++j) { filmc_slot(1, j / 6, j % 6); __builtin_amdgcn_sched_barrier(0); }

    X3_TS(3)
    Act<1> dfp;
#pragma unroll
    for (int g = 0; g < 4; ++g) {
      split2(df4[g].x, df4[g].y, dfp.hi[0][2 * g], dfp.lo[0][2 * g]);
      split2(df4[g].z, df4[g].w, dfp.hi[0][2 * g + 1], dfp.lo[0][2 * g + 1]);
    }

    if (!CIPS_TUNE(a.dbg & 1)) {
      constexpr int DFH = 0, DFL = 8192, HCH = 16384, HCL = 32768;
      stage<1, 128, DFH, DFL>(sbase, prow, hf, dfp);
      stage<2, 128, HCH, HCL>(sbase, prow, hf, hcp);
      __syncthreads();
      const int jt = wave & 1, kh = wave >> 1;
      const unsigned mdf = jt == 0 ? m_df : 0u;
      Frag fa[2], fb[2], fx[2];
      const unsigned d0 = opaque(LA.sb[0] + kh * 4096), d1 = opaque(LA.sb[1] + kh * 4096);
      const unsigned h0 = opaque(d0 + jt * 8192), h1_ = opaque(d1 + jt * 8192);
      const unsigned ax = opaque(LA.ab + kh * 1024);
      stg_frag<128, DFH, DFL>(d0, d1, 0, 0, fa[0]);
      stg_frag<128, HCH, HCL>(h0, h1_, 0, 0, fb[0]);
      aux_frag(ax, 0, mdf, fx[0]);
#pragma unroll
      for (int k = 0; k < 4; ++k) {
        if (k + 1 < 4) {
          stg_frag<128, DFH, DFL>(d0, d1, 0, k + 1, fa[(k + 1) & 1]);
          stg_frag<128, HCH, HCL>(h0, h1_, 0, k + 1, fb[(k + 1) & 1]);
          aux_frag(ax, k + 1, mdf, fx[(k + 1) & 1]);
        }
        __builtin_amdgcn_sched_barrier(0);
        aGf[0] = x3f(aGf[0], fa[k & 1], fb[k & 1]);
        aS[0] = x2f(aS[0], fa[k & 1], fx[k & 1]);
        __builtin_amdgcn_sched_barrier(0);
      }
      __syncthreads();
    }

    X3_TS(4)
    zero_acc(accc);
    layer_tr<2, 2, CF, O_WFH, O_WFL - O_WFH>(LA, dfp, accc);
    Act<2> dacp, dpcp;
    {
      float4 gn = lds_ld4(LA.v16 + (O_GC - O_L0));
#pragma unroll
      for (int grp = 0; grp < 8; ++grp) {
        const float4 g4 = gn;
        if (grp + 1 < 8) gn = lds_ld4(LA.v16 + (O_GC - O_L0) + 32 * (grp + 1));
        __builtin_amdgcn_sched_barrier(0);
        const int q = grp >> 2, g = grp & 3;
        const float gg[4] = {g4.x, g4.y, g4.z, g4.w};
        float v[4], w_[4];
#pragma unroll
        for (int e = 0; e < 4; ++e) { v[e] = accc[q][4 * g + e] * csc[q][4 * g + e]; w_[e] = gg[e] * v[e]; }
        split2(v[0], v[1], dacp.hi[q][2 * g], dacp.lo[q][2 * g]);
        split2(v[2], v[3], dacp.hi[q][2 * g + 1], dacp.lo[q][2 * g + 1]);
        split2(w_[0], w_[1], dpcp.hi[q][2 * g], dpcp.lo[q][2 * g]);
        split2(w_[2], w_[3], dpcp.hi[q][2 * g + 1], dpcp.lo[q][2 * g + 1]);
        __builtin_amdgcn_sched_barrier(0);
      }
    }

    pin(dacp); pin(h2p);
    X3_TS(5)
    if (!CIPS_TUNE(a.dbg & 2)) {
      constexpr int DAH = 0, DAL = 8192, H2H = 16384, H2L = 32768;
      const int it = wave & 1, jt0 = 2 * (wave >> 1);
      const unsigned mdc = wave < 2 ? m_dc : 0u;
      const unsigned i0 = opaque(LA.sb[0] + it * 4096), i1 = opaque(LA.sb[1] + it * 4096);
      const unsigned j0 = opaque(LA.sb[0] + jt0 * 4096), j1 = opaque(LA.sb[1] + jt0 * 4096);
      const unsigned w0 = opaque(LA.sb[0] + wave * 4096), w1 = opaque(LA.sb[1] + wave * 4096);
#pragma unroll
      for (int sp = 0; sp < 2; ++sp) {
        if ((wave >> 1) == sp) {
          stage<2, 64, DAH, DAL>(sbase, (wave & 1) * 32 + l31, hf, dacp);
          stage<4, 64, H2H, H2L>(sbase, (wave & 1) * 32 + l31, hf, h2p);
        }
        __syncthreads();
        Frag fa, fb0, fb1, fh, fx, fy;
        stg_frag<64, DAH, DAL>(i0, i1, 0, 0, fa);
        stg_frag<64, H2H, H2L>(j0, j1, 0, 0, fb0);
        stg_frag<64, H2H, H2L>(j0, j1, 32, 0, fb1);
#pragma unroll
        for (int k = 0; k < 4; ++k) {
          stg_frag<64, H2H, H2L>(w0, w1, 0, k, fh);
          aux_frag(LA.ab, 4 * sp + k, m_h2, fx);
          aux_frag(LA.ab, 4 * sp + k, mdc, fy);
          __builtin_amdgcn_sched_barrier(0);
          aGc[0] = x3f(aGc[0], fa, fb0);
          aGc[1] = x3f(aGc[1], fa, fb1);
          aS[0] = x2f(aS[0], fa, fy);
          __builtin_amdgcn_sched_barrier(0);
          if (k + 1 < 4) {
            stg_frag<64, DAH, DAL>(i0, i1, 0, k + 1, fa);
            stg_frag<64, H2H, H2L>(j0, j1, 0, k + 1, fb0);
            stg_frag<64, H2H, H2L>(j0, j1, 32, k + 1, fb1);
          }
          __builtin_amdgcn_sched_barrier(0);
          aS[0] = x3f(aS[0], fh, fx);
          __builtin_amdgcn_sched_barrier(0);
        }
        __syncthreads();
      }
    }

    X3_TS(6)
    zero_acc(acc);
    Act<4> da2p;
    Act<4> h1p;
    Act<4> da1p;
    float npx, npy, npz, ndsg;
    {
      Act<4> dp2p;
      float v4[4], w4_[4];
      float4 gq2, wq2;
      auto dh2_slot = [&](int q, int g, int j) __attribute__((always_inline)) {
        if (j == 0) {
          const float gg[4] = {gq2.x, gq2.y, gq2.z, gq2.w}, ww[4] = {wq2.x, wq2.y, wq2.z, wq2.w};
#pragma unroll
          for (int e = 0; e < 4; ++e) {
            v4[e] = fmaf(ww[e], dsg_s, acc[q][4 * g + e]) * cs2[q][4 * g + e];
            w4_[e] = gg[e] * v4[e];
          }
          pinf(v4[0], v4[1], v4[2], v4[3]); pinf(w4_[0], w4_[1], w4_[2], w4_[3]);
          if (4 * q + g + 1 < 16) {
            gq2 = lds_ld4(LA.v16 + (O_G1 - O_L0) + 32 * (4 * q + g + 1)); wq2 = lds_ld4(LA.v16 + (O_WS - O_L0) + 32 * (4 * q + g + 1));
          }
        } else if (j == 1) {
          split2(v4[0], v4[1], da2p.hi[q][2 * g], da2p.lo[q][2 * g]);
          split2(v4[2], v4[3], da2p.hi[q][2 * g + 1], da2p.lo[q][2 * g + 1]);
          pinu(da2p.hi[q][2 * g], da2p.lo[q][2 * g], da2p.hi[q][2 * g + 1], da2p.lo[q][2 * g + 1]);
        } else {
          split2(w4_[0], w4_[1], dp2p.hi[q][2 * g], dp2p.lo[q][2 * g]);
          split2(w4_[2], w4_[3], dp2p.hi[q][2 * g + 1], dp2p.lo[q][2 * g + 1]);
          pinu(dp2p.hi[q][2 * g], dp2p.lo[q][2 * g], dp2p.hi[q][2 * g + 1], dp2p.lo[q][2 * g + 1]);
        }
      };
      gq2 = lds_ld4(LA.v16 + (O_G1 - O_L0)); wq2 = lds_ld4(LA.v16 + (O_WS - O_L0));
      layer_tr_mm<4, 4, HC, O_WCH, O_WCL - O_WCH>(LA, dpcp, acc, [&](int slot) __attribute__((always_inline)) {
        const int m = slot / 12, j = slot % 12;
        if (m >= 1) dh2_slot(m - 1, j / 3, j % 3);
      });
#pragma unroll
      for (int j = 0; j < 12; ++j) { dh2_slot(3, j / 3, j % 3); __builtin_amdgcn_sched_barrier(0); }

      {
        const int p = pbase + 128 + prow;
        const bool valid = p < cend;
        const long long gp = (long long)b * a.P + (valid ? p : cend - 1);
        if (a.points) { npx = a.points[gp * 3 + 0]; npy = a.points[gp * 3 + 1]; npz = a.points[gp * 3 + 2]; }
        else gen_point(a.rg, b, valid ? p : cend - 1, npx, npy, npz);
        ndsg = valid ? a.dsigma[gp] : 0.f;
      }
      f32x16 acc1[4];
      zero_acc(acc1);
      float4 pq[4];
      float ar[4], s1[4], c1[4], d1[4];
      auto dh1_slot = [&](int q, int g, int j) __attribute__((always_inline)) {
// ... 185 lines not shown
```

cips3d_amd/csrc/small_ops.hip:

```cpp
#include "common.h"
#include "../../include/cips3d_hip.h"

namespace {

constexpr int GL_MAX = 32;
constexpr int GL_ROWS = 32;

struct GLJobs {
  const float* x[GL_MAX]; const float* w[GL_MAX]; const float* bias[GL_MAX]; float* y[GL_MAX];
  const float* dy[GL_MAX]; float* dw[GL_MAX]; float* db[GL_MAX];
  int in_dim[GL_MAX], out_dim[GL_MAX];
  int tile0[GL_MAX + 1];
  int njobs;
};

__device__ __forceinline__ int find_job(const GLJobs& J, int tile) {
  int j = 0;
  while (j + 1 < J.njobs && tile >= J.tile0[j + 1]) ++j;
  return j;
}

__global__ __launch_bounds__(256) void glin_fwd_kernel(GLJobs J, int B, int opw) {
  extern __shared__ __attribute__((aligned(16))) float xs[];
  const int job = find_job(J, blockIdx.x);
// ... 124 lines not shown
  for (int oo = 0; oo < oend; ++oo) {
    const float4 wv = on ? reinterpret_cast<const float4*>(w + (long long)oo * in_dim)[i4] : make_float4(0.f, 0.f, 0.f, 0.f);
#pragma unroll
    for (int r = 0; r < GLX_ROWS; ++r) {
      const float g = (b0 + r < B) ? dy[(long long)(b0 + r) * out_dim + oo] : 0.f;
      acc[r].x = fmaf(g, wv.x, acc[r].x); acc[r].y = fmaf(g, wv.y, acc[r].y);
      acc[r].z = fmaf(g, wv.z, acc[r].z); acc[r].w = fmaf(g, wv.w, acc[r].w);
    }
  }
  if (on) {
#pragma unroll
    for (int r = 0; r < GLX_ROWS; ++r)
      if (b0 + r < B) reinterpret_cast<float4*>(part + ((long long)blockIdx.x * B + b0 + r) * in_dim)[i4] = acc[r];
  }
}

__global__ __launch_bounds__(256) void glin_sum_kernel(const float* __restrict__ part, float* __restrict__ dx, int nchunks, long long n) {
  const long long i = (long long)blockIdx.x * 256 + threadIdx.x;
  if (i >= n) return;
  float s = 0.f;
  for (int c = 0; c < nchunks; ++c) s += part[(long long)c * n + i];
  dx[i] = s;
}

int fill(GLJobs& J, const cips_glin_job* jobs, int njobs, int outs_per_tile) {
  if (!jobs || njobs <= 0 || njobs > GL_MAX) return (int)hipErrorInvalidValue;
  J.njobs = njobs;
  int t = 0;
  for (int j = 0; j < njobs; ++j) {
    const cips_glin_job& q = jobs[j];
    if (!q.x || !q.w || q.in_dim <= 0 || q.out_dim <= 0 || (q.in_dim & 3) || q.in_dim > 512) return (int)hipErrorInvalidValue;
    J.x[j] = q.x; J.w[j] = q.w; J.bias[j] = q.bias; J.y[j] = q.y; J.dy[j] = q.dy; J.dw[j] = q.dw; J.db[j] = q.db;
    J.in_dim[j] = q.in_dim; J.out_dim[j] = q.out_dim;
    J.tile0[j] = t;
    t += (q.out_dim + outs_per_tile - 1) / outs_per_tile;
  }
  J.tile0[njobs] = t;
  return 0;
}


constexpr int RN_MAXC = 1024;

__device__ __forceinline__ float rn_block_sum(float v, float* red) {
  const int t = threadIdx.x;
  red[t] = v;
  __syncthreads();
  for (int s_ = 128; s_ > 0; s_ >>= 1) {
    if (t < s_) red[t] += red[t + s_];
    __syncthreads();
  }
  const float r = red[0];
  __syncthreads();
  return r;
}

__global__ __launch_bounds__(256) void rownorm_fwd_kernel(const float* __restrict__ x, const float* __restrict__ gamma,
                                                          const float* __restrict__ beta, float* __restrict__ y,
                                                          float* __restrict__ stats, int cols, int mode, float slope) {
  __shared__ float red[256];
  const int row = blockIdx.x, t = threadIdx.x;
  const float* xr = x + (long long)row * cols;
  float v[RN_MAXC / 256];
#pragma unroll
  for (int q = 0; q < RN_MAXC / 256; ++q) v[q] = (t + 256 * q < cols) ? xr[t + 256 * q] : 0.f;
  float out[RN_MAXC / 256];
  if (mode & 4) {
    float ss = 0.f;
#pragma unroll
    for (int q = 0; q < RN_MAXC / 256; ++q) ss = fmaf(v[q], v[q], ss);
    const float r = rsqrtf(rn_block_sum(ss, red) / (float)cols + 1e-8f);
#pragma unroll
    for (int q = 0; q < RN_MAXC / 256; ++q) out[q] = v[q] * r;
    if (t == 0) { stats[2 * row] = 0.f; stats[2 * row + 1] = r; }
  } else {
    float mean = 0.f, rstd = 1.f;
    if (mode & 1) {
      float s1 = 0.f;
#pragma unroll
      for (int q = 0; q < RN_MAXC / 256; ++q) s1 += v[q];
      mean = rn_block_sum(s1, red) / (float)cols;
      float s2 = 0.f;
#pragma unroll
      for (int q = 0; q < RN_MAXC / 256; ++q) { const float dlt = (t + 256 * q < cols) ? v[q] - mean : 0.f; s2 = fmaf(dlt, dlt, s2); }
      rstd = rsqrtf(rn_block_sum(s2, red) / (float)cols + 1e-5f);
    }
#pragma unroll
    for (int q = 0; q < RN_MAXC / 256; ++q) {
      const int c = t + 256 * q;
      float o = v[q];
      if ((mode & 1) && c < cols) o = (v[q] - mean) * rstd * gamma[c] + beta[c];
      if (mode & 2) o = o > 0.f ? o : o * slope;
      out[q] = o;
    }
    if (t == 0) { stats[2 * row] = mean; stats[2 * row + 1] = rstd; }
  }
#pragma unroll
  for (int q = 0; q < RN_MAXC / 256; ++q)
    if (t + 256 * q < cols) y[(long long)row * cols + t + 256 * q] = out[q];
}

__global__ __launch_bounds__(64) void rownorm_bwd_kernel(const float* __restrict__ x, const float* __restrict__ yout,
                                                         const float* __restrict__ gamma, const float* __restrict__ stats,
                                                         const float* __restrict__ dy, float* __restrict__ dx,
                                                         float* __restrict__ dyhat, int cols, int mode, float slope) {
  const int row = blockIdx.x, t = threadIdx.x;
  const long long base = (long long)row * cols;
  auto gate = [&](int c) {
    float gg = dy[base + c];
    if (mode & 2) gg *= (yout[base + c] > 0.f) ? 1.f : slope;
    return gg;
  };
  if (mode & 4) {
    const float r = stats[2 * row + 1];
    float s = 0.f;
    for (int c = t; c < cols; c += 64) s = fmaf(gate(c), x[base + c] * r, s);
    const float m = wave_sum_dpp(s) / (float)cols;
    for (int c = t; c < cols; c += 64) dx[base + c] = r * (gate(c) - x[base + c] * r * m);
    return;
  }
  if (!(mode & 1)) {
    for (int c = t; c < cols; c += 64) dx[base + c] = gate(c);
    return;
  }
  const float mean = stats[2 * row], rstd = stats[2 * row + 1];
  float s1 = 0.f, s2 = 0.f;
  for (int c = t; c < cols; c += 64) {
    const float g = gate(c);
    const float gx = g * gamma[c];
    dyhat[base + c] = g;
    s1 += gx;
    s2 = fmaf(gx, (x[base + c] - mean) * rstd, s2);
  }
  const float m1 = wave_sum_dpp(s1) / (float)cols;
  const float m2 = wave_sum_dpp(s2) / (float)cols;
  for (int c = t; c < cols; c += 64) {
    const float gx = dyhat[base + c] * gamma[c];
    dx[base + c] = rstd * (gx - m1 - (x[base + c] - mean) * rstd * m2);
  }
}

__global__ __launch_bounds__(256) void rownorm_bwd_affine_kernel(const float* __restrict__ x, const float* __restrict__ stats,
                                                                 const float* __restrict__ dyhat, float* __restrict__ dgamma,
                                                                 float* __restrict__ dbeta, int rows, int cols) {
  const int c = blockIdx.x * 256 + threadIdx.x;
  if (c >= cols) return;
  float a = 0.f, b = 0.f;
  for (int r = 0; r < rows; ++r) {
    const float g = dyhat[(long long)r * cols + c];
    a = fmaf(g, (x[(long long)r * cols + c] - stats[2 * r]) * stats[2 * r + 1], a);
    b += g;
  }
  dgamma[c] = a; dbeta[c] = b;
}


__global__ __launch_bounds__(64) void camera_pose_kernel(const float* __restrict__ th_raw, const float* __restrict__ ph_raw,
                                                         int uniform, float hs, float hm, float vs, float vm,
                                                         float phi_lo, float phi_hi, float* __restrict__ pitch_yaw,
                                                         float* __restrict__ origin, float* __restrict__ c2w, int B) {
  const int i = blockIdx.x * 64 + threadIdx.x;
  if (i >= B) return;
  float th, ph;
  if (uniform) {
    th = __fadd_rn(__fmul_rn(__fmul_rn(__fsub_rn(th_raw[i], 0.5f), 2.f), hs), hm);
    ph = __fadd_rn(__fmul_rn(__fmul_rn(__fsub_rn(ph_raw[i], 0.5f), 2.f), vs), vm);
  } else {
    th = __fadd_rn(__fmul_rn(th_raw[i], hs), hm);
    ph = __fadd_rn(__fmul_rn(ph_raw[i], vs), vm);
  }
  ph = fminf(fmaxf(ph, phi_lo), phi_hi);
  const float sp = sinf(ph), cp = cosf(ph), st = sinf(th), ct = cosf(th);
  const float ox = __fmul_rn(sp, ct), oy = cp, oz = __fmul_rn(sp, st);
  auto norm3 = [](float x, float y, float z) { return sqrtf(__fadd_rn(__fadd_rn(__fmul_rn(x, x), __fmul_rn(y, y)), __fmul_rn(z, z))); };
  float n = norm3(-ox, -oy, -oz);
  float fx = -ox / n, fy = -oy / n, fz = -oz / n;
  n = norm3(fx, fy, fz);
  fx /= n; fy /= n; fz /= n;
  float lx = fz, ly = 0.f, lz = -fx;
  n = norm3(lx, ly, lz);
  lx /= n; ly /= n; lz /= n;
  float ux = __fsub_rn(__fmul_rn(fy, lz), __fmul_rn(fz, ly));
  float uy = __fsub_rn(__fmul_rn(fz, lx), __fmul_rn(fx, lz));
  float uz = __fsub_rn(__fmul_rn(fx, ly), __fmul_rn(fy, lx));
  n = norm3(ux, uy, uz);
  ux /= n; uy /= n; uz /= n;
  pitch_yaw[2 * i] = ph; pitch_yaw[2 * i + 1] = th;
  origin[3 * i] = ox; origin[3 * i + 1] = oy; origin[3 * i + 2] = oz;
  float* m = c2w + 16 * i;
  m[0] = -lx; m[1] = ux; m[2] = -fx; m[3] = ox;
  m[4] = -ly; m[5] = uy; m[6] = -fy; m[7] = oy;
  m[8] = -lz; m[9] = uz; m[10] = -fz; m[11] = oz;
  m[12] = 0.f; m[13] = 0.f; m[14] = 0.f; m[15] = 1.f;
}

}

extern "C" int cips_grouped_linear_max_jobs(void) { return GL_MAX; }

extern "C" int cips_grouped_linear_fwd(const cips_glin_job* jobs, int njobs, int B, cips_stream_t stream) {
  GLJobs J;
  int rc = fill(J, jobs, njobs, 16);
  if (rc) return rc;
  if (B <= 0) return (int)hipErrorInvalidValue;
  int opw = 4;
  if (J.tile0[njobs] < 128) { opw = 1; rc = fill(J, jobs, njobs, 4); if (rc) return rc; }
  int max_in = 0;
  for (int j = 0; j < njobs; ++j) { if (!jobs[j].y) return (int)hipErrorInvalidValue; max_in = jobs[j].in_dim > max_in ? jobs[j].in_dim : max_in; }
  const size_t smem = (size_t)GL_ROWS * max_in * sizeof(float);
  static bool attr_set = false;
  CIPS_PER_DEVICE(attr_set, false);
  if (!attr_set) { (void)hipFuncSetAttribute((const void*)glin_fwd_kernel, hipFuncAttributeMaxDynamicSharedMemorySize, GL_ROWS * 512 * 4); attr_set = true; }
  hipLaunchKernelGGL(glin_fwd_kernel, dim3(J.tile0[njobs]), dim3(256), smem, (hipStream_t)stream, J, B, opw);
  return CIPS_CHECK_LAUNCH();
}

extern "C" int cips_grouped_linear_bwd(const cips_glin_job* jobs, int njobs, int B, float* dx, float* scratch,
                                       long long scratch_floats, cips_stream_t stream) {
  GLJobs J;
  int rc = fill(J, jobs, njobs, 16);
  if (rc) return rc;
  if (B <= 0) return (int)hipErrorInvalidValue;
  for (int j = 0; j < njobs; ++j) if (!jobs[j].dy || !jobs[j].dw) return (int)hipErrorInvalidValue;
  rc = fill(J, jobs, njobs, 4);
  if (rc) return rc;
  hipLaunchKernelGGL(glin_bwd_w_kernel<4>, dim3(J.tile0[njobs]), dim3(128), 0, (hipStream_t)stream, J, B);
  if (dx) {
    const int in_dim = jobs[0].in_dim;
    for (int j = 1; j < njobs; ++j) if (jobs[j].in_dim != in_dim || jobs[j].x != jobs[0].x) return (int)hipErrorInvalidValue;
    GLJobs K;
    rc = fill(K, jobs, njobs, 64);
    if (rc) return rc;
    const bool fine = K.tile0[njobs] < 64;
    if (fine) { rc = fill(K, jobs, njobs, 16); if (rc) return rc; }
    const int nchunks = K.tile0[njobs];
    if (!scratch || scratch_floats < (long long)nchunks * B * in_dim) return (int)hipErrorInvalidValue;
    const dim3 gx(nchunks, (B + GLX_ROWS - 1) / GLX_ROWS);
    if (fine) hipLaunchKernelGGL(glin_bwd_x_kernel<16>, gx, dim3(128), 0, (hipStream_t)stream, K, B, in_dim, scratch);
    else hipLaunchKernelGGL(glin_bwd_x_kernel<64>, gx, dim3(128), 0, (hipStream_t)stream, K, B, in_dim, scratch);
    const long long n = (long long)B * in_dim;
    hipLaunchKernelGGL(glin_sum_kernel, dim3((unsigned)((n + 255) / 256)), dim3(256), 0, (hipStream_t)stream, scratch, dx, nchunks, n);
  }
  return CIPS_CHECK_LAUNCH();
}

extern "C" long long cips_grouped_linear_scratch(const cips_glin_job* jobs, int njobs, int B) {
  if (!jobs || njobs <= 0) return 0;
  long long chunks = 0;
  for (int j = 0; j < njobs; ++j) chunks += (jobs[j].out_dim + 63) / 64;
  if (chunks < 64) {
    chunks = 0;
    for (int j = 0; j < njobs; ++j) chunks += (jobs[j].out_dim + 15) / 16;
  }
  return chunks * B * jobs[0].in_dim;
}

extern "C" int cips_rownorm_fwd(const float* x, const float* gamma, const float* beta, float* y, float* stats, int rows,
                                int cols, int mode, float slope, cips_stream_t stream) {
  if (!x || !y || !stats || rows <= 0 || cols <= 0 || cols > RN_MAXC || ((mode & 1) && (!gamma || !beta)) || ((mode & 4) && (mode & 3)))
    return (int)hipErrorInvalidValue;
  hipLaunchKernelGGL(rownorm_fwd_kernel, dim3(rows), dim3(256), 0, (hipStream_t)stream, x, gamma, beta, y, stats, cols, mode, slope);
  return CIPS_CHECK_LAUNCH();
}

extern "C" int cips_rownorm_bwd(const float* x, const float* y, const float* gamma, const float* stats, const float* dy,
                                float* dx, float* dyhat, float* dgamma, float* dbeta, int rows, int cols, int mode, float slope,
                                cips_stream_t stream) {
  if (!x || !y || !stats || !dy || !dx || rows <= 0 || cols <= 0 || cols > RN_MAXC || ((mode & 4) && (mode & 3))) return (int)hipErrorInvalidValue;
  if ((mode & 1) && (!gamma || !dyhat || !dgamma || !dbeta)) return (int)hipErrorInvalidValue;
  hipStream_t st = (hipStream_t)stream;
  hipLaunchKernelGGL(rownorm_bwd_kernel, dim3(rows), dim3(64), 0, st, x, y, gamma, stats, dy, dx, dyhat, cols, mode, slope);
  if (mode & 1)
    hipLaunchKernelGGL(rownorm_bwd_affine_kernel, dim3((cols + 255) / 256), dim3(256), 0, st, x, stats, dyhat, dgamma, dbeta, rows, cols);
  return CIPS_CHECK_LAUNCH();
}

namespace {
__global__ __launch_bounds__(256) void eql_sum_chunks_kernel(const float* __restrict__ part, float* __restrict__ y, int nch, int n,
                                                             int O, const float* __restrict__ bias, float bias_scale) {
  for (int i = blockIdx.x * 256 + threadIdx.x; i < n; i += gridDim.x * 256) {
    float v = part[i];
    for (int c = 1; c < nch; ++c) v += part[(long long)c * n + i];
    if (bias) v += bias[i % O] * bias_scale;
    y[i] = v;
  }
}
__global__ __launch_bounds__(256) void eql_fwd_small_kernel(const float* __restrict__ x, const float* __restrict__ w,
                                                            const float* __restrict__ bias, float bias_scale, float s,
                                                            float* __restrict__ y, int K, int O) {
  __shared__ float red[256];
  const int b = blockIdx.x;
  for (int o = 0; o < O; ++o) {
    float t = 0.f;
    for (int k = threadIdx.x; k < K; k += 256) t = fmaf(x[(long long)b * K + k], w[(long long)o * K + k], t);
    red[threadIdx.x] = t;
    __syncthreads();
    for (int h = 128; h > 0; h >>= 1) {
      if ((int)threadIdx.x < h) red[threadIdx.x] += red[threadIdx.x + h];
      __syncthreads();
    }
    if (threadIdx.x == 0) y[(long long)b * O + o] = s * red[0] + (bias ? bias[o] * bias_scale : 0.f);
    __syncthreads();
  }
}
__global__ __launch_bounds__(256) void eql_dx_small_kernel(const float* __restrict__ g, const float* __restrict__ w, float s,
                                                           float* __restrict__ dx, int B, int K, int O) {
  const long long n = (long long)B * K;
  for (long long i = (long long)blockIdx.x * 256 + threadIdx.x; i < n; i += (long long)gridDim.x * 256) {
    const int b = (int)(i / K), k = (int)(i - (long long)b * K);
    float t = 0.f;
    for (int o = 0; o < O; ++o) t = fmaf(g[(long long)b * O + o], w[(long long)o * K + k], t);
    dx[i] = s * t;
  }
}
__global__ __launch_bounds__(256) void eql_dw_small_kernel(const float* __restrict__ g, const float* __restrict__ x, float s,
                                                           float* __restrict__ dw, int B, int K, int O) {
  const long long n = (long long)O * K;
  for (long long i = (long long)blockIdx.x * 256 + threadIdx.x; i < n; i += (long long)gridDim.x * 256) {
    const int o = (int)(i / K), k = (int)(i - (long long)o * K);
    float t = 0.f;
    for (int b = 0; b < B; ++b) t = fmaf(g[(long long)b * O + o], x[(long long)b * K + k], t);
    dw[i] = s * t;
  }
}
__host__ int eql_chunks(int K) { return (K >= 2048 && K % 512 == 0) ? K / 512 : 1; }
}

extern "C" long long cips_equal_linear_scratch(int mode, int B, int K, int O) {
  if (mode != 0 || (O & 3) || (K & 3)) return 0;
  const int nch = eql_chunks(K);
  return nch > 1 ? (long long)nch * B * O : 0;
}

extern "C" int cips_equal_linear(int mode, const float* a, const float* b, const float* bias, float bias_scale, float s,
                                 float* out, float* scratch, int B, int K, int O, cips_stream_t stream) {
  if (!a || !b || !out || B <= 0 || K <= 0 || O <= 0 || mode < 0 || mode > 2) return (int)hipErrorInvalidValue;
  hipStream_t st = (hipStream_t)stream;
  const bool wide = !(O & 3) && !(K & 3);
  if (!wide) {
    if (mode == 0) hipLaunchKernelGGL(eql_fwd_small_kernel, dim3(B), dim3(256), 0, st, a, b, bias, bias_scale, s, out, K, O);
    else {
      const long long n = mode == 1 ? (long long)B * K : (long long)O * K;
      const int blocks = (int)((n + 255) / 256 < 2048 ? (n + 255) / 256 : 2048);
      if (mode == 1) hipLaunchKernelGGL(eql_dx_small_kernel, dim3(blocks), dim3(256), 0, st, a, b, s, out, B, K, O);
      else hipLaunchKernelGGL(eql_dw_small_kernel, dim3(blocks), dim3(256), 0, st, a, b, s, out, B, K, O);
    }
    return CIPS_CHECK_LAUNCH();
  }
  cips_gemm_desc d = {};
  d.alpha = s; d.batch = 1;
  if (mode == 0) {
    const int nch = eql_chunks(K);
    if (nch > 1 && !scratch) return (int)hipErrorInvalidValue;
    d.A = a; d.B = b; d.C = nch > 1 ? scratch : out;
    d.M = B; d.N = O; d.K = K / nch; d.lda = K; d.ldb = K; d.ldc = O; d.b_nmajor = 1;
    d.batch = nch; d.strideA = K / nch; d.strideB = K / nch; d.strideC = (long long)B * O;
    if (nch == 1 && bias) {  }
    int rc = cips_gemm_f32(&d, stream);
    if (rc) return rc;
    if (nch > 1 || bias) {
      const int n = B * O;
      hipLaunchKernelGGL(eql_sum_chunks_kernel, dim3((n + 255) / 256 < 1024 ? (n + 255) / 256 : 1024), dim3(256), 0, st,
                         nch > 1 ? scratch : out, out, nch, n, O, bias, bias_scale);
    }
    return CIPS_CHECK_LAUNCH();
  }
  if (mode == 1) {
    d.A = a; d.B = b; d.C = out; d.M = B; d.N = K; d.K = O; d.lda = O; d.ldb = K; d.ldc = K;
  } else {
    d.A = a; d.B = b; d.C = out; d.M = O; d.N = K; d.K = B; d.lda = O; d.ldb = K; d.ldc = K; d.a_kmajor = 1;
  }
  return cips_gemm_f32(&d, stream);
}

extern "C" int cips_camera_pose(const float* theta_raw, const float* phi_raw, int uniform, float h_stddev, float h_mean,
                                float v_stddev, float v_mean, float* pitch_yaw, float* origin, float* cam2world, int B,
                                cips_stream_t stream) {
  if (!theta_raw || !phi_raw || !pitch_yaw || !origin || !cam2world || B <= 0) return (int)hipErrorInvalidValue;
  const float lo = 1e-5f, hi = (float)(3.14159265358979323846 - 1e-5);
  hipLaunchKernelGGL(camera_pose_kernel, dim3((B + 63) / 64), dim3(64), 0, (hipStream_t)stream, theta_raw, phi_raw, uniform,
                     h_stddev, h_mean, v_stddev, v_mean, lo, hi, pitch_yaw, origin, cam2world, B);
  return CIPS_CHECK_LAUNCH();
}
```

cips3d_amd/generator.py:

```python
import math
import os
import random
from collections import OrderedDict

import numpy as np
import torch
import torch.nn as nn
import torch.nn.functional as F

from . import ops


def frequency_init(freq):
    def init(m):
        with torch.no_grad():
            if isinstance(m, nn.Linear):
                num_input = m.weight.size(-1)
                m.weight.uniform_(-np.sqrt(6 / num_input) / freq, np.sqrt(6 / num_input) / freq)
    return init


def kaiming_leaky_init(m):
    if m.__class__.__name__.find('Linear') != -1:
        torch.nn.init.kaiming_normal_(m.weight, a=0.2, mode='fan_in', nonlinearity='leaky_relu')


class PixelNorm(nn.Module):

    def forward(self, input):
        assert input.dim() == 2
        return input * torch.rsqrt(torch.mean(input ** 2, dim=1, keepdim=True) + 1e-8)


class MultiHeadMappingNetwork(nn.Module):

    def __init__(self, z_dim, hidden_dim, base_layers, head_layers, head_dim_dict,
                 add_norm=False, norm_out=False, **kwargs):
        super().__init__()
        self.z_dim = z_dim
        self.head_dim_dict = head_dim_dict
        out_dim = z_dim
        self.module_name_list = []
        self.norm = PixelNorm()
        base_net = []
        for i in range(base_layers):
            in_dim = out_dim
            out_dim = hidden_dim
            layer = nn.Linear(in_features=in_dim, out_features=out_dim)
            layer.apply(kaiming_leaky_init)
            base_net.append(layer)
            if head_layers > 0 or i != base_layers - 1:
                if add_norm:
                    base_net.append(nn.LayerNorm(out_dim))
                base_net.append(nn.LeakyReLU(0.2, inplace=True))
        if len(base_net) > 0:
            if norm_out and head_layers <= 0:
                base_net.append(nn.LayerNorm(out_dim))
            self.base_net = nn.Sequential(*base_net)
            self.num_z = 1
            self.module_name_list.append('base_net')
        else:
            self.base_net = None
            self.num_z = len(head_dim_dict)
        head_in_dim = out_dim
        for name, head_dim in head_dim_dict.items():
            if head_layers > 0:
                head_net = []
                out_dim = head_in_dim
                for i in range(head_layers):
                    in_dim = out_dim
                    out_dim = head_dim if i == head_layers - 1 else hidden_dim
                    hl = nn.Linear(in_features=in_dim, out_features=out_dim)
                    hl.apply(kaiming_leaky_init)
                    head_net.append(hl)
                    if i != head_layers - 1:
                        head_net.append(nn.LeakyReLU(0.2, inplace=True))
                    elif norm_out:
                        head_net.append(nn.LayerNorm(out_dim))
                head_net = nn.Sequential(*head_net)
                self.module_name_list.append(name)
            else:
                head_net = nn.Identity()
            self.add_module(name, head_net)

    def _base_hip(self, z):
        x = ops.RowNormFunction.apply(z, None, None, 4)
        mods = list(self.base_net)
        i = 0
        while i < len(mods):
            m = mods[i]
            if isinstance(m, nn.Linear):
                x = ops.grouped_linear([(x, m)])[0]
                i += 1
                ln = mods[i] if i < len(mods) and isinstance(mods[i], nn.LayerNorm) else None
                if ln is not None:
                    i += 1
                act = i < len(mods) and isinstance(mods[i], nn.LeakyReLU)
                if act:
                    i += 1
                if ln is not None or act:
                    x = ops.RowNormFunction.apply(x, ln.weight if ln is not None else None, ln.bias if ln is not None else None,
                                                  (1 if ln is not None else 0) | (2 if act else 0))
            else:
                x = m(x)
                i += 1
        return x

    def _hip_ok(self, z):
        return (z.is_cuda and z.dim() == 2 and z.dtype == torch.float32 and z.shape[0] <= 256 and z.shape[1] <= 512 and z.shape[1] % 4 == 0
                and all(not isinstance(m, nn.Linear) or (m.in_features <= 512 and m.in_features % 4 == 0 and m.out_features <= 1024)
                        for m in self.base_net))

    def forward(self, z):
        if self.base_net is not None:
            if self._hip_ok(z):
                base_fea = self._base_hip(z)
            else:
                z = self.norm(z)
                base_fea = self.base_net(z)
            head_inputs = {name: base_fea for name in self.head_dim_dict.keys()}
        else:
            head_inputs = {name: self.norm(z[idx]) for idx, name in enumerate(self.head_dim_dict.keys())}
        return {name: getattr(self, name)(head_inputs[name]) for name in self.head_dim_dict.keys()}


class FiLMLayer(nn.Module):

    def __init__(self, in_dim, out_dim, style_dim, use_style_fc=True, **kwargs):
        super().__init__()
        assert use_style_fc
        self.in_dim, self.out_dim, self.style_dim, self.use_style_fc = in_dim, out_dim, style_dim, use_style_fc
        self.linear = nn.Linear(in_dim, out_dim)
        self.linear.apply(frequency_init(25))
        self.gain_fc = nn.Linear(style_dim, out_dim)
        self.bias_fc = nn.Linear(style_dim, out_dim)
        self.gain_fc.weight.data.mul_(0.25)
        self.bias_fc.weight.data.mul_(0.25)

    def film(self, style):
        return self.gain_fc(style) * 15 + 30, self.bias_fc(style)


def _film_all(layers, styles):
    ys = ops.grouped_linear([(st, m) for lay, st in zip(layers, styles) for m in (lay.gain_fc, lay.bias_fc)])
    return [(ys[2 * i] * 15 + 30, ys[2 * i + 1]) for i in range(len(layers))]


class NeRFNetwork(nn.Module):

    def __init__(self, in_dim=3, hidden_dim=256, hidden_layers=2, style_dim=512, rgb_dim=3, device=None,
                 name_prefix='nerf', **kwargs):
        super().__init__()
        if not (in_dim == 3 and rgb_dim == 32 and hidden_layers >= 1):
            raise NotImplementedError(
                "the ray set-up produces 3-vectors and the composite / CIPS head take 32 colour features "
                "(in_dim 3, rgb_dim 32: every shipped config, ffhq_exp.yaml:51-58)")
        self.fused = hidden_dim == 128 and hidden_layers == 2
        self.device = device
        self.in_dim, self.hidden_dim, self.rgb_dim = in_dim, hidden_dim, rgb_dim
        self.style_dim, self.hidden_layers, self.name_prefix = style_dim, hidden_layers, name_prefix
        self.module_name_list = []
        self.style_dim_dict = {}
        self.network = nn.ModuleList()
        self.module_name_list.append('network')
        _out = in_dim
        for idx in range(hidden_layers):
            _in, _out = _out, hidden_dim
            layer = FiLMLayer(in_dim=_in, out_dim=_out, style_dim=style_dim, use_style_fc=True)
            self.network.append(layer)
            self.style_dim_dict[f'{name_prefix}_w{idx}'] = layer.style_dim
        self.final_layer = nn.Linear(hidden_dim, 1)
        self.module_name_list.append('final_layer')
        self.color_layer_sine = FiLMLayer(in_dim=hidden_dim, out_dim=hidden_dim // 2, style_dim=style_dim,
                                          use_style_fc=True)
        self.style_dim_dict[f'{name_prefix}_rgb'] = self.color_layer_sine.style_dim
        self.module_name_list.append('color_layer_sine')
        self.color_layer_linear = nn.Sequential(nn.Linear(hidden_dim // 2, rgb_dim))
        self.color_layer_linear.apply(kaiming_leaky_init)
        self.module_name_list.append('color_layer_linear')
        self.dim_styles = sum(self.style_dim_dict.values())

    def _evaluate_unfused(self, points, style_dict):
        if not points.is_cuda:
            raise RuntimeError("NeRFNetwork runs on the GPU only (there is no CPU path)")
        p = self.name_prefix
        x = points * (2.0 / 0.24)
        for idx, layer in enumerate(self.network):
            gain, bias = layer.film(style_dict[f'{p}_w{idx}'])
            x = torch.sin(gain.unsqueeze(1) * layer.linear(x) + bias.unsqueeze(1))
        sigma = self.final_layer(x).squeeze(-1)
        gain, bias = self.color_layer_sine.film(style_dict[f'{p}_rgb'])
        c = torch.sin(gain.unsqueeze(1) * self.color_layer_sine.linear(x) + bias.unsqueeze(1))
        return self.color_layer_linear(c), sigma

    def evaluate(self, points, style_dict):
        if not self.fused:
            return self._evaluate_unfused(points, style_dict)
        p = self.name_prefix
        (g0, p0), (g1, p1), (gc, pc) = _film_all([self.network[0], self.network[1], self.color_layer_sine],
                                                 [style_dict[f'{p}_w0'], style_dict[f'{p}_w1'], style_dict[f'{p}_rgb']])
        return ops.SirenFunction.apply(
            points, g0, p0, g1, p1, gc, pc,
            self.network[0].linear.weight, self.network[0].linear.bias,
            self.network[1].linear.weight, self.network[1].linear.bias,
            self.final_layer.weight, self.final_layer.bias,
            self.color_layer_sine.linear.weight, self.color_layer_sine.linear.bias,
            self.color_layer_linear[0].weight, self.color_layer_linear[0].bias)

    def evaluate_rays(self, style_dict, geom, xg, yg, zg, cam2world, jitter=None, zvals=None):
        p = self.name_prefix
        (g0, p0), (g1, p1), (gc, pc) = _film_all([self.network[0], self.network[1], self.color_layer_sine],
                                                 [style_dict[f'{p}_w0'], style_dict[f'{p}_w1'], style_dict[f'{p}_rgb']])
        return ops.SirenRaysFunction.apply(
            geom, xg, yg, zg, cam2world, jitter, zvals, g0, p0, g1, p1, gc, pc,
            self.network[0].linear.weight, self.network[0].linear.bias,
            self.network[1].linear.weight, self.network[1].linear.bias,
            self.final_layer.weight, self.final_layer.bias,
            self.color_layer_sine.linear.weight, self.color_layer_sine.linear.bias,
            self.color_layer_linear[0].weight, self.color_layer_linear[0].bias)

    def march(self, style_dict, geom, xg, yg, zg, cam2world, jitter, noise):
        p = self.name_prefix
        (g0, p0), (g1, p1), (gc, pc) = _film_all([self.network[0], self.network[1], self.color_layer_sine],
                                                 [style_dict[f'{p}_w0'], style_dict[f'{p}_w1'], style_dict[f'{p}_rgb']])
        return ops.RayMarchFunction.apply(
            geom, xg, yg, zg, cam2world, jitter, noise, g0, p0, g1, p1, gc, pc,
            self.network[0].linear.weight, self.network[0].linear.bias,
            self.network[1].linear.weight, self.network[1].linear.bias,
            self.final_layer.weight, self.final_layer.bias,
            self.color_layer_sine.linear.weight, self.color_layer_sine.linear.bias,
            self.color_layer_linear[0].weight, self.color_layer_linear[0].bias)

    def forward(self, input, style_dict, ray_directions=None, **kwargs):
        feat, sigma = self.evaluate(input, style_dict)
        return torch.cat([feat, sigma.unsqueeze(-1)], dim=-1)

    forward_with_frequencies_phase_shifts = forward


class SinStyleMod(nn.Module):
# ... 593 lines not shown
```

cips3d_amd/ops.py:

```python
import ctypes as C
import ctypes as _ct
import math
import os as _os
import weakref

import torch

from . import _lib
from ._lib import GemmDesc, GemmX3Desc, SirenWeights, check

LRELU_SLOPE = 0.2


def _p(t):
    return C.c_void_p(t.data_ptr()) if t is not None else None


def _stream():
    return C.c_void_p(torch.cuda.current_stream().cuda_stream)


def _chk(*tensors):
    for t in tensors:
        if t is None:
# ... 1 lines not shown
        if not t.is_cuda:
            raise RuntimeError("cips3d_amd ops need tensors on the GPU (no CPU fallback)")
        if t.device.index != torch.cuda.current_device():
            raise RuntimeError(f"tensor on {t.device} but the current device is cuda:{torch.cuda.current_device()}; "
                               "call torch.cuda.set_device first")
        if t.dtype != torch.float32 and t.dtype not in (torch.int32, torch.int64, torch.bfloat16):
            raise RuntimeError(f"cips3d_amd ops are fp32 (got {t.dtype})")
        if not t.is_contiguous():
            raise RuntimeError("cips3d_amd ops need contiguous tensors")


def _c(t):
    return t.contiguous().float() if t is not None else None




def camera_pose(theta_raw, phi_raw, uniform, h_stddev, h_mean, v_stddev, v_mean):
    lib = _lib.load()
    dev = theta_raw.device
    B = theta_raw.shape[0]
    th, ph = _c(theta_raw), _c(phi_raw)
    py = torch.empty(B, 2, device=dev); origin = torch.empty(B, 3, device=dev); c2w = torch.empty(B, 4, 4, device=dev)
    check(lib.cips_camera_pose(_p(th), _p(ph), 1 if uniform else 0, float(h_stddev), float(h_mean), float(v_stddev),
                               float(v_mean), _p(py), _p(origin), _p(c2w), B, _stream()), "cips_camera_pose")
    return py, origin, c2w


_GRIDS = {}


def pixel_grids(W, H, S, ray_start, ray_end, device):
    key = (W, H, S, float(ray_start), float(ray_end), str(device))
    g = _GRIDS.get(key)
    if g is None:
        g = (torch.linspace(-1, 1, W, device=device), torch.linspace(1, -1, H, device=device),
             torch.linspace(ray_start, ray_end, S, device=device))
        if torch.device(device).type == "cuda" and torch.cuda.is_current_stream_capturing():
            return g
        if len(_GRIDS) > 64:
            _GRIDS.clear()
        _GRIDS[key] = g
    return g

def rays_fwd(xg, yg, zg, zc, cam2world, jitter, B, H, W, S):
    lib = _lib.load()
    dev = cam2world.device
    n = H * W
    points = torch.empty(B, n, S, 3, device=dev)
    z = torch.empty(B, n, S, device=dev)
    dirs = torch.empty(B, n, 3, device=dev)
    xg, yg, zg, cam2world, jitter = _c(xg), _c(yg), _c(zg), _c(cam2world), _c(jitter)
    _chk(xg, yg, zg, cam2world, jitter)
    check(lib.cips_rays_fwd(_p(xg), _p(yg), _p(zg), float(zc), _p(cam2world), _p(jitter),
                            _p(points), _p(z), _p(dirs), B, H, W, S, _stream()), "cips_rays_fwd")
    return points, z, dirs


def gemm(A, Bm, Cm, M, N, K, lda, ldb, ldc, batch=1, strideA=0, strideB=0, strideC=0,
         a_kmajor=False, b_nmajor=False, alpha=1.0, bias=None, bias_m=None, act=0, slope=LRELU_SLOPE,
         act_gain=1.0, resid=None, C2=None, add=None, rgb_g=None, rgb_w=None, C_unmasked=None, mask=None):
    lib = _lib.load()
    d = GemmDesc()
    d.A, d.B, d.C = _p(A), _p(Bm), _p(Cm)
    d.M, d.N, d.K = M, N, K
    d.lda, d.ldb, d.ldc = lda, ldb, ldc
    d.strideA, d.strideB, d.strideC = strideA, strideB, strideC
    d.batch = batch
    d.a_kmajor = 1 if a_kmajor else 0
    d.b_nmajor = 1 if b_nmajor else 0
    d.alpha = alpha
    d.bias, d.bias_m = _p(bias), _p(bias_m)
    d.act, d.slope, d.act_gain = act, slope, act_gain
    d.resid, d.C2, d.add = _p(resid), _p(C2), _p(add)
    d.rgb_g, d.rgb_w = _p(rgb_g), _p(rgb_w)
    d.C_unmasked, d.mask = _p(C_unmasked), _p(mask)
    check(lib.cips_gemm_f32(C.byref(d), _stream()), "cips_gemm_f32")
    return Cm


def bmm_nn(x, w, out=None, **epi):
    B, M, K = x.shape
    N = w.shape[-1]
    if out is None:
        out = torch.empty(B, M, N, device=x.device)
    gemm(x, w, out, M, N, K, K, N, N, batch=B, strideA=M * K, strideB=K * N, strideC=M * N, **epi)
    return out


def bmm_tn(a, b, out=None):
    B, K, Ma = a.shape
    N = b.shape[-1]
    if out is None:
        out = torch.empty(B, Ma, N, device=a.device)
    gemm(a, b, out, Ma, N, K, Ma, N, N, batch=B, strideA=K * Ma, strideB=K * N, strideC=Ma * N, a_kmajor=True)
    return out


_SIREN_NAMES = ("w0", "b0", "w1", "b1", "ws", "bs", "wc", "bc", "wf", "bf", "g0", "p0", "g1", "p1", "gc", "pc")
BOX_SCALE = 2.0 / 0.24
TRIG_MODE = 1


def _siren_struct(t):
    s = SirenWeights()
    for n in _SIREN_NAMES:
        setattr(s, n, _p(t[n]))
    s.box_scale = BOX_SCALE
    s.trig_mode = TRIG_MODE
    return s


def _split_k(P, target=8):
    for s in range(target, 0, -1):
        if P % s == 0 and (P // s) % 32 == 0:
            return s
    return 1


SIREN_FWD_MODE = __import__("os").environ.get("CIPS_SIREN_FWD", "x3")
SIREN_BWD_MODE = __import__("os").environ.get("CIPS_SIREN_BWD", "x3")


class SirenFunction(torch.autograd.Function):

    @staticmethod
    def forward(ctx, points, g0, p0, g1, p1, gc, pc, w0, b0, w1, b1, ws, bs, wc, bc, wf, bf):
        lib = _lib.load()
        t = dict(w0=w0, b0=b0, w1=w1, b1=b1, ws=ws, bs=bs, wc=wc, bc=bc, wf=wf, bf=bf,
                 g0=g0, p0=p0, g1=g1, p1=p1, gc=gc, pc=pc)
        t = {k: _c(v.detach()) for k, v in t.items()}
        points = _c(points.detach())
        _chk(points, *t.values())
        B, P, _ = points.shape
        feat = torch.empty(B, P, 32, device=points.device)
        sigma = torch.empty(B, P, device=points.device)
        sw = _siren_struct(t)
        fwd = lib.cips_siren_fwd_x3 if SIREN_FWD_MODE == "x3" else lib.cips_siren_fwd
        check(fwd(C.byref(sw), _p(points), _p(feat), _p(sigma), B, P, _stream()), "cips_siren_fwd")
        ctx.save_for_backward(points, *[t[n] for n in _SIREN_NAMES])
        return feat, sigma

    @staticmethod
    def backward(ctx, dfeat, dsigma):
        points = ctx.saved_tensors[0]
        t = dict(zip(_SIREN_NAMES, ctx.saved_tensors[1:]))
        B, P, _ = points.shape
        dev = points.device
        dfeat = _c(dfeat) if dfeat is not None else torch.zeros(B, P, 32, device=dev)
        dsigma = _c(dsigma) if dsigma is not None else torch.zeros(B, P, device=dev)
        return (None,) + _siren_backward(t, dfeat, dsigma, B, P, points=points)


def _siren_backward(t, dfeat, dsigma, B, P, points=None, rays=None):
    lib = _lib.load()
    dev = dfeat.device
    sw = _siren_struct(t)
    if True:
        if SIREN_BWD_MODE == "x3" or points is None:
            chunks = lib.cips_siren_bwd_x3_chunks(B, P)
            gw = lib.cips_siren_bwd_x3_gpart()
            sw_ = lib.cips_siren_bwd_x3_sred()
            sred = torch.empty(B * chunks, sw_, device=dev)
            gpart = torch.empty(B * chunks, gw, device=dev)
            if points is not None:
                check(lib.cips_siren_bwd_x3(C.byref(sw), _p(points), _p(dfeat), _p(dsigma), _p(sred), _p(gpart), B, P,
                                            _stream()), "cips_siren_bwd_x3")
            else:
                check(lib.cips_siren_bwd_x3_rays(C.byref(sw), C.byref(rays), _p(dfeat), _p(dsigma), _p(sred), _p(gpart), B,
                                                 _stream()), "cips_siren_bwd_x3_rays")
            from ._lib import SirenGrads
            shapes = dict(dg0=(B, 128), dp0=(B, 128), dg1=(B, 128), dp1=(B, 128), dgc=(B, 64), dpc=(B, 64), dw0=(128, 3),
                          db0=(128,), dw1=(128, 128), db1=(128,), dws=(1, 128), dbs=(1,), dwc=(64, 128), dbc=(64,),
                          dwf=(32, 64), dbf=(32,))
            outs = {k: torch.empty(*v, device=dev) for k, v in shapes.items()}
            sg = SirenGrads()
            for k, v in outs.items():
                setattr(sg, k, _p(v))
            SRr = sred.view(B, chunks, sw_).sum(1) if chunks > 1 else sred
            Gpr = gpart.view(B, chunks, gw).sum(1) if chunks > 1 else gpart
            check(lib.cips_siren_bwd_x3_finalize(C.byref(sw), _p(SRr), _p(Gpr), B, 1, C.byref(sg), _stream()),
                  "cips_siren_bwd_x3_finalize")
            return tuple(outs[k] for k in ("dg0", "dp0", "dg1", "dp1", "dgc", "dpc", "dw0", "db0", "dw1", "db1", "dws",
                                           "dbs", "dwc", "dbc", "dwf", "dbf"))
        elif SIREN_BWD_MODE == "staged_f32":
            BP = B * P
            h1, h2, da2 = (torch.empty(BP, 128, device=dev) for _ in range(3))
            hc, dac = (torch.empty(BP, 64, device=dev) for _ in range(2))
            rows = lib.cips_siren_bwd_rows(B, P)
            red = torch.empty(rows, 868, device=dev)
            check(lib.cips_siren_bwd_data_f32(C.byref(sw), _p(points), _p(dfeat), _p(dsigma), _p(h1), _p(h2), _p(hc), _p(da2), _p(dac),
                                              _p(red), B, P, _stream()), "cips_siren_bwd_data_f32")
            R = red.view(B, rows // B, 868).sum(1)
            sp = _split_k(P, 16)
            Kc = P // sp
            G1 = torch.empty(B * sp, 128, 128, device=dev)
            gemm(da2, h1, G1, 128, 128, Kc, 128, 128, 128, batch=B * sp, strideA=Kc * 128, strideB=Kc * 128, strideC=128 * 128,
                 a_kmajor=True)
            G1 = G1.view(B, sp, 128, 128).sum(1)
            Gc = torch.empty(B * sp, 64, 128, device=dev)
            gemm(dac, h2, Gc, 64, 128, Kc, 64, 128, 128, batch=B * sp, strideA=Kc * 64, strideB=Kc * 128, strideC=64 * 128,
                 a_kmajor=True)
            Gc = Gc.view(B, sp, 64, 128).sum(1)
            spf = _split_k(BP, 1024)
            Kf = BP // spf
            Gf = torch.empty(spf, 32, 64, device=dev)
            gemm(dfeat, hc, Gf, 32, 64, Kf, 32, 64, 64, batch=spf, strideA=Kf * 32, strideB=Kf * 64, strideC=32 * 64, a_kmajor=True)
            dwf = Gf.sum(0)
        else:
            BP = B * P
            h1, h2, da2 = (Planes.empty(BP, 128, device=dev) for _ in range(3))
            hc, dac = (Planes.empty(BP, 64, device=dev) for _ in range(2))
            rows = lib.cips_siren_bwd_rows(B, P)
            red = torch.empty(rows, 868, device=dev)
            check(lib.cips_siren_bwd_data(C.byref(sw), _p(points), _p(dfeat), _p(dsigma), _p(h1.hi), _p(h1.lo),
                                          _p(h2.hi), _p(h2.lo), _p(hc.hi), _p(hc.lo), _p(da2.hi), _p(da2.lo),
                                          _p(dac.hi), _p(dac.lo), _p(red), B, P, _stream()), "cips_siren_bwd_data")
            R = red.view(B, rows // B, 868).sum(1)
            sp = _split_k(P, 16)
            Kc = P // sp
            G1 = torch.empty(B * sp, 128, 128, device=dev)
            gemm_x3_km(da2, h1, 128, 128, Kc, 128, 128, B * sp, Kc * 128, Kc * 128, G1)
            G1 = G1.view(B, sp, 128, 128).sum(1)
            Gc = torch.empty(B * sp, 64, 128, device=dev)
            gemm_x3_km(dac, h2, 64, 128, Kc, 64, 128, B * sp, Kc * 64, Kc * 128, Gc)
            Gc = Gc.view(B, sp, 64, 128).sum(1)
            hcf = hc.float()
            spf = _split_k(BP, 1024)
            Kf = BP // spf
            Gf = torch.empty(spf, 32, 64, device=dev)
            gemm(dfeat, hcf, Gf, 32, 64, Kf, 32, 64, 64, batch=spf, strideA=Kf * 32, strideB=Kf * 64,
                 strideC=32 * 64, a_kmajor=True)
            dwf = Gf.sum(0)
        g0, g1, gc = t["g0"], t["g1"], t["gc"]
        w0, b0, w1, b1, wc, bc = t["w0"], t["b0"], t["w1"], t["b1"], t["wc"], t["bc"]
        dp0 = R[:, 0:128]
        S0 = R[:, 128:512].view(B, 3, 128).transpose(1, 2) * BOX_SCALE
        dg0 = (S0 * w0.unsqueeze(0)).sum(-1) + b0.unsqueeze(0) * dp0
        dw0 = (g0.unsqueeze(-1) * S0).sum(0)
        db0 = (g0 * dp0).sum(0)
        dp1 = R[:, 512:640]
        dg1 = (G1 * w1.unsqueeze(0)).sum(-1) + b1.unsqueeze(0) * dp1
        dw1 = (g1.unsqueeze(-1) * G1).sum(0)
        db1 = (g1 * dp1).sum(0)
        dpc = R[:, 640:704]
        dgc = (Gc * wc.unsqueeze(0)).sum(-1) + bc.unsqueeze(0) * dpc
        dwc = (gc.unsqueeze(-1) * Gc).sum(0)
        dbc = (gc * dpc).sum(0)
        dws = R[:, 704:832].sum(0, keepdim=True)
        dbf = R[:, 832:864].sum(0)
        dbs = R[:, 864].sum().view(1)
        return (dg0, dp0, dg1, dp1, dgc, dpc, dw0, db0, dw1, db1, dws, dbs, dwc, dbc, dwf, dbf)


def resample_fwd(sigma, z, noise, noise_std, u, origins, dirs, B, n, S, clamp_mode=0, debug=False, cdf_in=None, rays=None):
    lib = _lib.load()
    dev = sigma.device
    sigma, z, noise, u, origins, dirs = _c(sigma), _c(z), _c(noise), _c(u), _c(origins), _c(dirs)
    _chk(sigma, z, noise, u, origins, dirs)
    R = B * n
    fine_z = torch.empty(R, S, device=dev)
    fine_pts = torch.empty(R, S, 3, device=dev) if rays is None else None
    w = cdf = inds = None
    if debug:
        w = torch.empty(R, S, device=dev)
        cdf = torch.empty(R, S - 1, device=dev)
        inds = torch.empty(R, S, device=dev, dtype=torch.int64)
    check(lib.cips_resample_fwd(_p(sigma), _p(z), _p(noise), float(noise_std), _p(u), _p(origins), _p(dirs),
                                _p(fine_z), _p(fine_pts), _p(w), _p(cdf), _p(inds), B, n, S, clamp_mode,
                                _p(_c(cdf_in)) if cdf_in is not None else None,
                                C.byref(rays) if rays is not None else None, _stream()), "cips_resample_fwd")
    if debug:
        return fine_z, fine_pts, w, cdf, inds
    return fine_z, fine_pts


_CLAMP = {"relu": 0, "softplus": 1}


class CompositeFunction(torch.autograd.Function):

    @staticmethod
    def forward(ctx, feat_c, sig_c, z_c, feat_f, sig_f, z_f, noise, noise_std, clamp_mode, flags):
        lib = _lib.load()
        feat_c, sig_c, z_c = _c(feat_c.detach()), _c(sig_c.detach()), _c(z_c.detach())
        hier = feat_f is not None
        if hier:
            feat_f, sig_f, z_f = _c(feat_f.detach()), _c(sig_f.detach()), _c(z_f.detach())
        noise = _c(noise) if (noise is not None and noise_std != 0.0) else None
        _chk(feat_c, sig_c, z_c, feat_f, sig_f, z_f, noise)
        R, S, _ = feat_c.shape
        E = 2 * S if hier else S
        dev = feat_c.device
        fea = torch.empty(R, 32, device=dev)
        depth = torch.empty(R, device=dev)
        weights = torch.empty(R, E, device=dev)
        order = torch.empty(R, E, device=dev, dtype=torch.int32)
        zs = torch.empty(R, E, device=dev)
        pin, rec = _clamp_debug_forward(R, E, clamp_mode, dev)
        check(lib.cips_composite_fwd(_p(feat_c), _p(sig_c), _p(z_c), _p(feat_f), _p(sig_f), _p(z_f), _p(noise),
                                     float(noise_std), _p(fea), _p(depth), _p(weights), _p(order), _p(zs),
                                     R, S, clamp_mode, flags, _p(pin), _p(rec), _stream()), "cips_composite_fwd")
        if rec is not None and CLAMP_REC is not None:
            CLAMP_REC.append(rec.reshape(R, E))
        ctx.clamp_mask = pin
        ctx.save_for_backward(feat_c, sig_c, z_c, feat_f, sig_f, z_f, noise, order)
        ctx.meta = (float(noise_std), clamp_mode, flags, hier)
        ctx.mark_non_differentiable(depth, weights, order, zs)
        return fea, depth, weights, order, zs

    @staticmethod
    def backward(ctx, dfea, *unused):
        lib = _lib.load()
        feat_c, sig_c, z_c, feat_f, sig_f, z_f, noise, order = ctx.saved_tensors
        noise_std, clamp_mode, flags, hier = ctx.meta
        R, S, _ = feat_c.shape
        dfea = _c(dfea)
        dfeat_c = torch.empty_like(feat_c)
        dsig_c = torch.empty_like(sig_c)
        dfeat_f = torch.empty_like(feat_f) if hier else None
        dsig_f = torch.empty_like(sig_f) if hier else None
        check(lib.cips_composite_bwd(_p(feat_c), _p(sig_c), _p(z_c), _p(feat_f), _p(sig_f), _p(z_f), _p(noise),
                                     noise_std, _p(order), _p(dfea), _p(dfeat_c), _p(dsig_c), _p(dfeat_f),
                                     _p(dsig_f), R, S, clamp_mode, flags, _p(ctx.clamp_mask), _stream()), "cips_composite_bwd")
        _tail_gate_publish(dfea.device)
        return dfeat_c, dsig_c, None, dfeat_f, dsig_f, None, None, None, None, None




class GroupedLinearFunction(torch.autograd.Function):

    @staticmethod
    def forward(ctx, x, *wb):
        lib = _lib.load()
        from ._lib import GlinJob
        x = _c(x.detach())
        ws = [_c(w.detach()) for w in wb[0::2]]
        bs = [_c(b.detach()) if b is not None else None for b in wb[1::2]]
        _chk(x, *ws, *[b for b in bs if b is not None])
        B, in_dim = x.shape
        n = len(ws)
        if n > lib.cips_grouped_linear_max_jobs() or in_dim % 4 or in_dim > 512:
            raise RuntimeError("grouped linear: at most 32 jobs, in_dim a multiple of 4 and <= 512")
        jobs = (GlinJob * n)()
        ys = []
        for j, (w, b) in zip(jobs, zip(ws, bs)):
            y = torch.empty(B, w.shape[0], device=x.device)
            j.x, j.w, j.bias, j.y = _p(x), _p(w), _p(b), _p(y)
            j.in_dim, j.out_dim = in_dim, w.shape[0]
            ys.append(y)
        check(lib.cips_grouped_linear_fwd(jobs, n, B, _stream()), "cips_grouped_linear_fwd")
        ctx.save_for_backward(x, *ws)
        ctx.has_bias = [b is not None for b in bs]
        return tuple(ys)

    @staticmethod
    def backward(ctx, *dys):
        lib = _lib.load()
        from ._lib import GlinJob
        x, *ws = ctx.saved_tensors
        B, in_dim = x.shape
        n = len(ws)
        jobs = (GlinJob * n)()
        dws, dbs, keep = [], [], []
        for j, w, dy, hb in zip(jobs, ws, dys, ctx.has_bias):
            dy = _c(dy) if dy is not None else torch.zeros(B, w.shape[0], device=x.device)
            keep.append(dy)
            dw = torch.empty_like(w)
            db = torch.empty(w.shape[0], device=x.device) if hb else None
            j.x, j.w, j.dy, j.dw, j.db = _p(x), _p(w), _p(dy), _p(dw), _p(db)
            j.in_dim, j.out_dim = in_dim, w.shape[0]
            dws.append(dw); dbs.append(db)
        dx = scratch = None
        nscr = 0
        if ctx.needs_input_grad[0]:
            dx = torch.empty_like(x)
            nscr = lib.cips_grouped_linear_scratch(jobs, n, B)
            scratch = torch.empty(nscr, device=x.device)
        check(lib.cips_grouped_linear_bwd(jobs, n, B, _p(dx), _p(scratch), nscr, _stream()), "cips_grouped_linear_bwd")
        out = [dx]
        for dw, db in zip(dws, dbs):
            out += [dw, db]
        return tuple(out)


def grouped_linear(pairs):
    out = [None] * len(pairs)
    groups = {}
    for idx, (x, lin) in enumerate(pairs):
        groups.setdefault(id(x), []).append(idx)
    mx = 32
    for idxs in groups.values():
        x = pairs[idxs[0]][0]
        if x.dim() != 2 or x.shape[1] % 4 or x.shape[1] > 512 or x.shape[0] > 256 or not x.is_cuda:
            for i in idxs:
                out[i] = pairs[i][1](pairs[i][0])
            continue
        for c0 in range(0, len(idxs), mx):
            chunk = idxs[c0:c0 + mx]
            args = []
            for i in chunk:
                lin = pairs[i][1]
                args += [lin.weight, lin.bias]
            ys = GroupedLinearFunction.apply(x, *args)
            for i, y in zip(chunk, ys):
                out[i] = y
    return out


class RowNormFunction(torch.autograd.Function):

    @staticmethod
    def forward(ctx, x, gamma, beta, mode):
        lib = _lib.load()
        x = _c(x.detach())
        gamma = _c(gamma.detach()) if gamma is not None else None
        beta = _c(beta.detach()) if beta is not None else None
        _chk(x, gamma, beta)
        rows, cols = x.shape
        y = torch.empty_like(x)
        stats = torch.empty(rows, 2, device=x.device)
        check(lib.cips_rownorm_fwd(_p(x), _p(gamma), _p(beta), _p(y), _p(stats), rows, cols, mode, LRELU_SLOPE, _stream()),
              "cips_rownorm_fwd")
        ctx.save_for_backward(x, y, gamma, stats)
        ctx.mode = mode
        return y

    @staticmethod
    def backward(ctx, dy):
        lib = _lib.load()
        x, y, gamma, stats = ctx.saved_tensors
        rows, cols = x.shape
        dy = _c(dy)
        dx = torch.empty_like(x)
        ln = bool(ctx.mode & 1)
        dyhat = torch.empty_like(x) if ln else None
        dgamma = torch.empty(cols, device=x.device) if ln else None
        dbeta = torch.empty(cols, device=x.device) if ln else None
        check(lib.cips_rownorm_bwd(_p(x), _p(y), _p(gamma), _p(stats), _p(dy), _p(dx), _p(dyhat), _p(dgamma), _p(dbeta), rows,
                                   cols, ctx.mode, LRELU_SLOPE, _stream()), "cips_rownorm_bwd")
        return dx, dgamma, dbeta, None


MARCH_FUSED = True


def march_available():
    return MARCH_FUSED and SIREN_FWD_MODE == "x3" and SIREN_BWD_MODE == "x3"


def _ray_params(xg, yg, zg, zc, cam2world, jitter, H, W, S, zvals=None):
    from ._lib import RayParams
    r = RayParams()
    r.xg, r.yg, r.zg, r.cam2world, r.jitter, r.zvals = _p(xg), _p(yg), _p(zg), _p(cam2world), _p(jitter), _p(zvals)
    r.zc, r.H, r.W, r.S = float(zc), H, W, S
    return r


class SirenRaysFunction(torch.autograd.Function):

    @staticmethod
    def forward(ctx, geom, xg, yg, zg, cam2world, jitter, zvals, g0, p0, g1, p1, gc, pc, w0, b0, w1, b1, ws, bs, wc, bc,
                wf, bf):
        lib = _lib.load()
        B, H, W, S, zc = geom
        t = dict(w0=w0, b0=b0, w1=w1, b1=b1, ws=ws, bs=bs, wc=wc, bc=bc, wf=wf, bf=bf,
                 g0=g0, p0=p0, g1=g1, p1=p1, gc=gc, pc=pc)
        t = {k: _c(v.detach()) for k, v in t.items()}
        xg, yg, zg, cam2world = _c(xg), _c(yg), _c(zg), _c(cam2world)
        jitter = _c(jitter) if jitter is not None else None
        zvals = _c(zvals.detach()) if zvals is not None else None
        _chk(xg, yg, zg, cam2world, jitter, zvals, *t.values())
        dev = cam2world.device
        P = H * W * S
        feat = torch.empty(B, P, 32, device=dev)
        sigma = torch.empty(B, P, device=dev)
        z = torch.empty(B, P, device=dev) if zvals is None else zvals
        sw = _siren_struct(t)
        rp = _ray_params(xg, yg, zg, zc, cam2world, jitter, H, W, S, zvals)
        check(lib.cips_siren_fwd_x3_rays(C.byref(sw), C.byref(rp), _p(feat), _p(sigma), _p(z) if zvals is None else None, B,
                                         _stream()), "cips_siren_fwd_x3_rays")
        ctx.save_for_backward(xg, yg, zg, cam2world, jitter, zvals, *[t[k] for k in _SIREN_NAMES])
        ctx.geom = geom
        ctx.mark_non_differentiable(z)
        return feat, sigma, z

    @staticmethod
    def backward(ctx, dfeat, dsigma, _dz):
        xg, yg, zg, cam2world, jitter, zvals = ctx.saved_tensors[:6]
        t = dict(zip(_SIREN_NAMES, ctx.saved_tensors[6:]))
        B, H, W, S, zc = ctx.geom
        P = H * W * S
        dev = cam2world.device
        dfeat = _c(dfeat) if dfeat is not None else torch.zeros(B, P, 32, device=dev)
        dsigma = _c(dsigma) if dsigma is not None else torch.zeros(B, P, device=dev)
        rp = _ray_params(xg, yg, zg, zc, cam2world, jitter, H, W, S, zvals)
        return (None,) * 7 + _siren_backward(t, dfeat, dsigma, B, P, rays=rp)


class RayMarchFunction(torch.autograd.Function):

    @staticmethod
    def forward(ctx, geom, xg, yg, zg, cam2world, jitter, noise, g0, p0, g1, p1, gc, pc, w0, b0, w1, b1, ws, bs, wc, bc,
                wf, bf):
        lib = _lib.load()
        B, H, W, S, zc, noise_std, clamp_mode, flags, grad_mode = geom
        t = dict(w0=w0, b0=b0, w1=w1, b1=b1, ws=ws, bs=bs, wc=wc, bc=bc, wf=wf, bf=bf,
                 g0=g0, p0=p0, g1=g1, p1=p1, gc=gc, pc=pc)
        t = {k: _c(v.detach()) for k, v in t.items()}
        xg, yg, zg, cam2world = _c(xg), _c(yg), _c(zg), _c(cam2world)
        jitter = _c(jitter) if jitter is not None else None
        noise = _c(noise) if (noise is not None and noise_std != 0.0) else None
        _chk(xg, yg, zg, cam2world, jitter, noise, *t.values())
        dev = cam2world.device
        n = H * W
        train = grad_mode and any(ctx.needs_input_grad)
        fea = torch.empty(B, n, 32, device=dev)
        depth = torch.empty(B, n, device=dev)
        feat = torch.empty(B, n * S, 32, device=dev) if train else None
        sigma = torch.empty(B, n * S, device=dev) if train else None
        z = torch.empty(B, n * S, device=dev) if train else None
        sw = _siren_struct(t)
        rp = _ray_params(xg, yg, zg, zc, cam2world, jitter, H, W, S)
        pin, rec = _clamp_debug_forward(B * n, S, clamp_mode, dev)
        check(lib.cips_march_fwd_x3(C.byref(sw), C.byref(rp), _p(noise), float(noise_std), clamp_mode, flags, _p(fea),
                                    _p(depth), None, _p(feat), _p(sigma), _p(z), B, _p(pin), _p(rec), _stream()),
              "cips_march_fwd_x3")
        if rec is not None and CLAMP_REC is not None:
            CLAMP_REC.append(rec.reshape(B * n, S))
        ctx.clamp_mask = pin
        if train:
            ctx.save_for_backward(xg, yg, zg, cam2world, jitter, noise, feat, sigma, z, *[t[k] for k in _SIREN_NAMES])
        ctx.geom = geom
        ctx.mark_non_differentiable(depth)
        return fea, depth

    @staticmethod
    def backward(ctx, dfea, _ddepth):
        lib = _lib.load()
        xg, yg, zg, cam2world, jitter, noise, feat, sigma, z = ctx.saved_tensors[:9]
        t = dict(zip(_SIREN_NAMES, ctx.saved_tensors[9:]))
        B, H, W, S, zc, noise_std, clamp_mode, flags, _ = ctx.geom
        n = H * W
        R = B * n
        dfea = _c(dfea)
        dfeat = torch.empty_like(feat)
        dsig = torch.empty_like(sigma)
        check(lib.cips_composite_bwd(_p(feat), _p(sigma), _p(z), None, None, None, _p(noise), float(noise_std), None,
                                     _p(dfea), _p(dfeat), _p(dsig), None, None, R, S, clamp_mode, flags, _p(ctx.clamp_mask),
                                     _stream()), "cips_composite_bwd")
        _tail_gate_publish(dfea.device)
        rp = _ray_params(xg, yg, zg, zc, cam2world, jitter, H, W, S)
        grads = _siren_backward(t, dfeat, dsig, B, n * S, rays=rp)
        return (None,) * 7 + grads


def modfc_prep(W, s, eps=1e-8):
    lib = _lib.load()
    in_dim, out_dim = W.shape
    B = s.shape[0]
    dev = W.device
    wb = torch.empty(B, in_dim, out_dim, device=dev)
    wbt = torch.empty(B, out_dim, in_dim, device=dev)
    demod = torch.empty(B, out_dim, device=dev)
    check(lib.cips_modfc_prep(_p(W), _p(s), _p(wb), _p(wbt), _p(demod), B, in_dim, out_dim, eps, _stream()),
          "cips_modfc_prep")
    return wb, wbt, demod


def modfc_prep_bwd(W, s, demod, gwb):
    lib = _lib.load()
    in_dim, out_dim = W.shape
    B = s.shape[0]
    dev = W.device
    cbuf = torch.empty(B, out_dim, device=dev)
    dW = torch.empty(in_dim, out_dim, device=dev)
    ds = torch.empty(B, in_dim, device=dev)
    check(lib.cips_modfc_prep_bwd(_p(W), _p(s), _p(demod), _p(gwb), _p(cbuf), _p(dW), _p(ds), B, in_dim, out_dim,
                                  _stream()), "cips_modfc_prep_bwd")
    return dW, ds


def torgb_fwd(x2d, w, b, rgb2d, accumulate):
    lib = _lib.load()
    M, K = x2d.shape
    check(lib.cips_torgb_fwd(_p(x2d), _p(w), _p(b), _p(rgb2d), M, K, 1 if accumulate else 0, _stream()),
          "cips_torgb_fwd")


def torgb_bwd_w(x2d, drgb2d):
    lib = _lib.load()
    M, K = x2d.shape
    chunks = lib.cips_torgb_bwd_partials(M)
    part = torch.empty(chunks, 4, K, device=x2d.device)
    dw = torch.empty(3, K, device=x2d.device)
    db = torch.empty(3, device=x2d.device)
    check(lib.cips_torgb_bwd_w(_p(x2d), _p(drgb2d), _p(part), _p(dw), _p(db), M, K, _stream()), "cips_torgb_bwd_w")
    return dw, db


def torgb_bwd_x_x3(drgb2d, w, gate_bits, out_unmasked, P):
    lib = _lib.load()
    M, K = drgb2d.shape[0], w.shape[1]
    check(lib.cips_torgb_bwd_x_x3(_p(drgb2d), _p(_c(w)), _p(gate_bits), LRELU_SLOPE, _p(out_unmasked), _p(P.hi), _p(P.lo), M, K,
                                  _stream()), "cips_torgb_bwd_x_x3")


def torgb_bwd_x(drgb2d, w, add, mask, out_unmasked, out):
    lib = _lib.load()
    M = drgb2d.shape[0]
    K = w.shape[1]
    check(lib.cips_torgb_bwd_x(_p(drgb2d), _p(w), _p(add), _p(mask), LRELU_SLOPE, _p(out_unmasked), _p(out), M, K,
                               _stream()), "cips_torgb_bwd_x")


GATE_PIN = None
GATE_REC = None
FINE_Z_PIN = None
FINE_Z_REC = None


CLAMP_PIN = None
CLAMP_REC = None


class clamp_debug:

    def __init__(self, pin=None, rec=None):
        self.pin, self.rec = pin, rec

    def __enter__(self):
        global CLAMP_PIN, CLAMP_REC
        self.old = (CLAMP_PIN, CLAMP_REC)
        CLAMP_PIN = iter(self.pin) if self.pin is not None else None
        CLAMP_REC = self.rec
        return self

    def __exit__(self, *exc):
        global CLAMP_PIN, CLAMP_REC
        CLAMP_PIN, CLAMP_REC = self.old


def _clamp_debug_forward(R, E, clamp_mode, dev):
    if (CLAMP_PIN is None and CLAMP_REC is None) or clamp_mode != 0:
        return None, None
    pin = None
    if CLAMP_PIN is not None:
        pin = next(CLAMP_PIN).to(device=dev, dtype=torch.uint8).reshape(-1).contiguous()
        if pin.numel() != R * E:
            raise ValueError(f"clamp_debug: pinned mask of {pin.numel()} entries for {R} rays x {E} positions")
    return pin, (torch.empty(R * E, dtype=torch.uint8, device=dev) if CLAMP_REC is not None else None)


class resample_debug:

    def __init__(self, pin=None, rec=None):
        self.pin, self.rec = pin, rec

    def __enter__(self):
        global FINE_Z_PIN, FINE_Z_REC
        self.old = (FINE_Z_PIN, FINE_Z_REC)
        FINE_Z_PIN = iter(self.pin) if self.pin is not None else None
        FINE_Z_REC = self.rec
        return self

    def __exit__(self, *exc):
        global FINE_Z_PIN, FINE_Z_REC
        FINE_Z_PIN, FINE_Z_REC = self.old


class gate_debug:

    def __init__(self, pin=None, rec=None):
        self.pin, self.rec = pin, rec

    def __enter__(self):
        global GATE_PIN, GATE_REC
        self.old = (GATE_PIN, GATE_REC)
        GATE_PIN = iter(self.pin) if self.pin is not None else None
        GATE_REC = self.rec
        return self

    def __exit__(self, *exc):
        global GATE_PIN, GATE_REC
        if exc[0] is None and GATE_PIN is not None:
            assert next(GATE_PIN, None) is None, "pinned gate planes left over"
        GATE_PIN, GATE_REC = self.old


def _next_pin(B, n, C, dev):
    if GATE_PIN is None:
        return None
    p = next(GATE_PIN)
    assert p.dtype == torch.uint8 and tuple(p.shape) == (B, n, C // 8), (tuple(p.shape), (B, n, C // 8))
    return p.to(dev).contiguous()


def _bits_to_pm1(p):
    sh = torch.arange(8, device=p.device)
    g = ((p.unsqueeze(-1).to(torch.int32) >> sh) & 1).reshape(*p.shape[:-1], p.shape[-1] * 8)
    return (g * 2 - 1).float()


def _sign_to_bits(a):
    w = (1 << torch.arange(8, device=a.device)).to(torch.int32)
    return ((a > 0).reshape(*a.shape[:-1], a.shape[-1] // 8, 8).to(torch.int32) * w).sum(-1).to(torch.uint8)
# ... 922 lines not shown
```

include/cips3d_hip.h:

```cpp
#ifndef CIPS3D_HIP_H
#define CIPS3D_HIP_H

#ifdef __cplusplus
extern "C" {
#endif

typedef void* cips_stream_t;

int cips_version(void);
const char* cips_arch(void);

int cips_rays_fwd(const float* xg, const float* yg, const float* zg, float zc,
                  const float* cam2world, const float* jitter,
                  float* points, float* z, float* dirs,
                  int B, int H, int W, int S, cips_stream_t stream);

typedef struct cips_siren_weights {
  const float* w0;
  const float* b0;
  const float* w1;
  const float* b1;
  const float* ws;
  const float* bs;
  const float* wc;
  const float* bc;
  const float* wf;
  const float* bf;
  const float* g0;
  const float* p0;
  const float* g1;
  const float* p1;
  const float* gc;
  const float* pc;
  float box_scale;
  int trig_mode;
} cips_siren_weights;

int cips_siren_fwd(const cips_siren_weights* w, const float* points,
                   float* feat, float* sigma, int B, int P, cips_stream_t stream);

int cips_siren_bwd_rows(int B, int P);
int cips_siren_bwd_data(const cips_siren_weights* w, const float* points,
                        const float* dfeat, const float* dsigma,
                        void* h1_hi, void* h1_lo, void* h2_hi, void* h2_lo, void* hc_hi, void* hc_lo,
                        void* da2_hi, void* da2_lo, void* dac_hi, void* dac_lo,
                        float* red, int B, int P, cips_stream_t stream);
int cips_siren_bwd_data_f32(const cips_siren_weights* w, const float* points, const float* dfeat, const float* dsigma, float* h1,
                            float* h2, float* hc, float* da2, float* dac, float* red, int B, int P, cips_stream_t stream);

int cips_siren_fwd_x3(const cips_siren_weights* w, const float* points, float* feat, float* sigma,
                      int B, int P, cips_stream_t stream);

int cips_siren_bwd_x3_chunks(int B, int P);
int cips_siren_bwd_x3_gpart(void);
int cips_siren_bwd_x3_sred(void);
int cips_siren_bwd_x3(const cips_siren_weights* w, const float* points, const float* dfeat,
                      const float* dsigma, float* sred, float* gpart, int B, int P, cips_stream_t stream);

typedef struct cips_siren_grads {
  float *dg0, *dp0, *dg1, *dp1, *dgc, *dpc;
  float *dw0, *db0, *dw1, *db1, *dws, *dbs, *dwc, *dbc, *dwf, *dbf;
} cips_siren_grads;
int cips_siren_bwd_x3_finalize(const cips_siren_weights* w, const float* sred, const float* gpart, int B, int chunks,
                               const cips_siren_grads* out, cips_stream_t stream);

typedef struct cips_ray_params {
  const float* xg; const float* yg; const float* zg;
  const float* cam2world;
  const float* jitter;
  const float* zvals;
  float zc;
  int H, W, S;
} cips_ray_params;

int cips_siren_fwd_x3_rays(const cips_siren_weights* w, const cips_ray_params* rays, float* feat, float* sigma,
                           float* zout, int B, cips_stream_t stream);

int cips_siren_bwd_x3_rays(const cips_siren_weights* w, const cips_ray_params* rays, const float* dfeat,
                           const float* dsigma, float* sred, float* gpart, int B, cips_stream_t stream);

int cips_march_fwd_x3(const cips_siren_weights* w, const cips_ray_params* rays, const float* noise, float noise_std,
                      int clamp_mode, int flags, float* fea, float* depth, float* weights, float* feat, float* sigma,
                      float* z, int B, const unsigned char* clamp_in, unsigned char* clamp_out, cips_stream_t stream);

int cips_resample_fwd(const float* sigma, const float* z, const float* noise, float noise_std,
                      const float* u, const float* origins, const float* dirs,
                      float* fine_z, float* fine_pts,
                      float* weights_out, float* cdf_out, long long* inds_out,
                      int B, int n, int S, int clamp_mode, const float* cdf_in, const cips_ray_params* rays,
                      cips_stream_t stream);

int cips_composite_fwd(const float* feat_c, const float* sig_c, const float* z_c,
                       const float* feat_f, const float* sig_f, const float* z_f,
                       const float* noise, float noise_std,
                       float* fea, float* depth, float* weights, int* order, float* zsorted,
                       int R, int S, int clamp_mode, int flags, const unsigned char* clamp_in, unsigned char* clamp_out,
                       cips_stream_t stream);

int cips_composite_bwd(const float* feat_c, const float* sig_c, const float* z_c,
                       const float* feat_f, const float* sig_f, const float* z_f,
                       const float* noise, float noise_std, const int* order,
                       const float* dfea,
                       float* dfeat_c, float* dsig_c, float* dfeat_f, float* dsig_f,
                       int R, int S, int clamp_mode, int flags, const unsigned char* clamp_in, cips_stream_t stream);

typedef struct cips_gemm_desc {
  const float* A; const float* B; float* C;
  int M, N, K;
  int lda, ldb, ldc;
  long long strideA, strideB, strideC;
  int batch;
  int a_kmajor;
  int b_nmajor;
  float alpha;
  const float* bias;
  const float* bias_m;
  int act;
  float slope; float act_gain;
  const float* resid;
  float* C2;
  const float* add;
  const float* rgb_g;
  const float* rgb_w;
  float* C_unmasked;
  const float* mask;
} cips_gemm_desc;

int cips_gemm_f32(const cips_gemm_desc* d, cips_stream_t stream);

typedef struct cips_gemm_x3_desc {
  const void* A_hi; const void* A_lo; const void* B_hi; const void* B_lo;
  int M, N, K;
  int lda, ldb;
  long long strideA, strideB;
  int batch;
  float* C; int ldc; long long strideC;
  void* P_hi; void* P_lo; int ldp; long long strideP;
  void* T_hi; void* T_lo; int ldt; long long strideT;
  void* mask_out;
  const float* add;
  const float* rgb_g; const float* rgb_w;
  float* C_unmasked;
  const void* mask;
  int act; float slope;
  const void* res_hi; const void* res_lo;
  int gate_bits;
  const float* torgb_w; float* torgb_part;
  const void* addp_hi; const void* addp_lo; const void* addp_gate; float addp_gain;
  int kernel;
} cips_gemm_x3_desc;

int cips_gemm_bf16x3(const cips_gemm_x3_desc* d, cips_stream_t stream);
int cips_gemm_bf16x3_fuses_torgb(const cips_gemm_x3_desc* d);
int cips_gemm_bf16x3_takes_addp(const cips_gemm_x3_desc* d);
int cips_torgb_finish(const float* part, int nblocks, const float* bias, float* rgb, long long M, int accumulate,
                      cips_stream_t stream);
int cips_gemm_bf16x3_km(const cips_gemm_x3_desc* d, cips_stream_t stream);
int cips_gemm_bf16x3_km_grouped(const cips_gemm_x3_desc* descs, int ngroups, cips_stream_t stream);

int cips_gemm_bf16(const cips_gemm_x3_desc* d, cips_stream_t stream);
int cips_gemm_bf16_fuses_torgb(const cips_gemm_x3_desc* d);
int cips_gemm_bf16_takes_addp(const cips_gemm_x3_desc* d);
int cips_gemm_bf16_km(const cips_gemm_x3_desc* d, cips_stream_t stream);
int cips_gemm_bf16_km_grouped(const cips_gemm_x3_desc* descs, int ngroups, cips_stream_t stream);

typedef struct cips_conv_x3_desc {
  const void* w_hi; const void* w_lo;
  const void* x_hi; const void* x_lo;
  float* y;
  int B, C, H, W, O, kh, kw, stride, pad;
  int ksplit;
  float* part;
  const float* bias;
  int act;
  float slope, act_scale;
} cips_conv_x3_desc;
int cips_conv2d_x3(const cips_conv_x3_desc* d, cips_stream_t stream);
int cips_conv2d_x3_ksplit(int B, int O, int N, int K);
typedef struct cips_conv_dgrad_s2_desc {
  const void* w_hi; const void* w_lo;
  const void* dy_hi; const void* dy_lo;
  float* dxp;
  int B, C, H, W, O, kh, kw;
  long long w_off[4], out_off[4];
} cips_conv_dgrad_s2_desc;
int cips_conv2d_x3_dgrad_s2(const cips_conv_dgrad_s2_desc* d, cips_stream_t stream);
#define CIPS_WPREP_MAX_JOBS 24
typedef struct cips_wprep_job {
  const float* w;
  void* fwd_hi; void* fwd_lo;
  void* alt_hi; void* alt_lo;
  float scale;
  int O, C, kh, kw, alt_kind;
  int bank_off[4];
} cips_wprep_job;
int cips_conv_weight_prep_max_jobs(void);
int cips_conv_weight_prep_batch(const cips_wprep_job* jobs, int njobs, cips_stream_t stream);
typedef struct cips_conv_wgrad_desc {
  const void* dy_hi; const void* dy_lo;
  const void* x_hi; const void* x_lo;
  float* part;
  int B, C, H, W, O, kh, kw, stride, pad, nchunks;
} cips_conv_wgrad_desc;
int cips_conv2d_x3_wgrad(const cips_conv_wgrad_desc* d, cips_stream_t stream);
int cips_conv_wgrad_finish(const float* part, float* dw, int nchunks, int taps, int O, int C, float scale,
                           cips_stream_t stream);
int cips_split_planes_nhwc(const float* x, void* t_hi, void* t_lo, int B, int C, int n, cips_stream_t stream);

int cips_split_planes(const float* x, void* p_hi, void* p_lo, void* t_hi, void* t_lo, int rows, int cols,
                      int ldx, int ldp, int ldt, int batch, long long stride_x, long long stride_p,
                      long long stride_t, cips_stream_t stream);

int cips_modfc_prep(const float* weight, const float* s, float* wb, float* wbt, float* demod,
                    int B, int in_dim, int out_dim, float eps, cips_stream_t stream);
int cips_modfc_prep_x3(const float* weight, const float* s, void* wb_hi, void* wb_lo, void* wbt_hi,
                       void* wbt_lo, float* demod, int B, int in_dim, int out_dim, float eps,
                       cips_stream_t stream);
int cips_modfc_prep_bwd(const float* weight, const float* s, const float* demod, const float* gwb,
                        float* cbuf, float* dweight, float* ds, int B, int in_dim, int out_dim,
                        cips_stream_t stream);

typedef struct cips_modfc_prep_job {
  const float* weight; const float* s;
  void *wb_hi, *wb_lo, *wbt_hi, *wbt_lo;
  float* demod;
  int in_dim, out_dim;
} cips_modfc_prep_job;
typedef struct cips_modfc_bwd_job {
  const float* weight; const float* s; const float* demod; const float* gwb;
  float *cbuf, *dweight, *ds;
  int in_dim, out_dim;
} cips_modfc_bwd_job;
int cips_modfc_max_jobs(void);
int cips_modfc_prep_x3_batch(const cips_modfc_prep_job* jobs, int njobs, int B, float eps, cips_stream_t stream);
int cips_modfc_prep_bwd_batch(const cips_modfc_bwd_job* jobs, int njobs, int B, cips_stream_t stream);
int cips_cores_colsum_parts(void);
int cips_modfc_prep_bwd_batch_cores(const cips_modfc_bwd_job* jobs, int njobs, int B, cips_stream_t stream);

typedef struct cips_glin_job {
  const float* x; const float* w; const float* bias; float* y;
  const float* dy; float* dw; float* db;
  int in_dim, out_dim;
} cips_glin_job;
int cips_grouped_linear_max_jobs(void);
int cips_grouped_linear_fwd(const cips_glin_job* jobs, int njobs, int B, cips_stream_t stream);
long long cips_grouped_linear_scratch(const cips_glin_job* jobs, int njobs, int B);
int cips_grouped_linear_bwd(const cips_glin_job* jobs, int njobs, int B, float* dx, float* scratch,
                            long long scratch_floats, cips_stream_t stream);

int cips_rownorm_fwd(const float* x, const float* gamma, const float* beta, float* y, float* stats, int rows, int cols,
                     int mode, float slope, cips_stream_t stream);
int cips_rownorm_bwd(const float* x, const float* y, const float* gamma, const float* stats, const float* dy, float* dx,
                     float* dyhat, float* dgamma, float* dbeta, int rows, int cols, int mode, float slope,
                     cips_stream_t stream);

int cips_torgb_fwd(const float* x, const float* w, const float* bias, float* rgb,
                   long long M, int K, int accumulate, cips_stream_t stream);
int cips_torgb_bwd_partials(long long M);
int cips_torgb_bwd_w(const float* x, const float* drgb, float* partials, float* dw, float* dbias,
                     long long M, int K, cips_stream_t stream);
int cips_torgb_fwd_x3(const void* x_hi, const void* x_lo, const float* w, const float* bias, float* rgb,
                      long long M, int K, int accumulate, cips_stream_t stream);
int cips_torgb_bwd_w_x3(const void* x_hi, const void* x_lo, const float* drgb, float* partials, float* dw,
                        float* dbias, long long M, int K, cips_stream_t stream);
int cips_torgb_bwd_w_x3_batch(const void* const* x_hi, const void* const* x_lo, int njobs, const float* drgb,
                              float* partials, float* dw, float* dbias, long long M, int K, cips_stream_t stream);
int cips_torgb_bwd_w_x3_batch_cores(const void* const* x_hi, const void* const* x_lo, int njobs, const float* drgb,
                                    float* partials, float* dw, float* dbias, long long M, int K, cips_stream_t stream);
int cips_torgb_bwd_x(const float* drgb, const float* w, const float* add, const float* mask, float slope,
                     float* out_unmasked, float* out, long long M, int K, cips_stream_t stream);
int cips_torgb_bwd_x_x3(const float* drgb, const float* w, const void* gate_bits, float slope, float* out_unmasked,
                        void* p_hi, void* p_lo, long long M, int K, cips_stream_t stream);

int cips_camera_pose(const float* theta_raw, const float* phi_raw, int uniform, float h_stddev, float h_mean,
                     float v_stddev, float v_mean, float* pitch_yaw, float* origin, float* cam2world, int B,
                     cips_stream_t stream);

int cips_fused_bias_act(const float* x, const float* bias, const float* refer, float* y,
                        long long numel, int size_b, int step_b,
                        int act, int grad, float alpha, float scale, cips_stream_t stream);

int cips_upfirdn2d(const float* input, const float* kernel, float* out,
                   int major, int in_h, int in_w, int minor, int kernel_h, int kernel_w,
                   int up_x, int up_y, int down_x, int down_y,
                   int pad_x0, int pad_x1, int pad_y0, int pad_y1, cips_stream_t stream);
int cips_upfirdn2d_parity(const float* dxp, const long long* blk_off, const float* kernel, float* out, int major,
                          int in_h, int in_w, int pad_x0, int pad_x1, int pad_y0, int pad_y1, cips_stream_t stream);

long long cips_equal_linear_scratch(int mode, int B, int K, int O);
int cips_equal_linear(int mode, const float* a, const float* b, const float* bias, float bias_scale, float s, float* out,
                      float* scratch, int B, int K, int O, cips_stream_t stream);

int cips_diffaug(const float* x, float* y, const float* rb, const float* rs, const float* rc, const long long* tx,
                 const long long* ty, const long long* ox, const long long* oy, float* sums, int B, int C, int H, int W,
                 int cut_h, int cut_w, int adjoint, int affine, cips_stream_t stream);
int cips_avgpool2(const float* x, float* y, long long planes, int H, int W, int adjoint, cips_stream_t stream);
int cips_axpby(const float* x, const float* y, float* out, float a, float b, long long n, cips_stream_t stream);

int cips_image_to_u8(const float* x, unsigned char* out, int B, int C, int H, int W, float lo, float hi,
                     cips_stream_t stream);

int cips_lrelu_bwd_bias_slices(int HW);
int cips_lrelu_bwd_bias(const float* grad, const float* refer, float* grad_in, float* part, long long planes, int HW,
                        float alpha, float scale, cips_stream_t stream);
int cips_lrelu_bwd_bias_finish(const float* part, float* grad_bias, int B, int C, int S, cips_stream_t stream);
int cips_lrelu_bwd_bias_nhwc_tiles(int HW);
int cips_lrelu_bwd_bias_nhwc(const float* grad, const float* refer, void* t_hi, void* t_lo, float* part, int B, int C, int HW,
                             float alpha, float scale, cips_stream_t stream);

int cips_conv1x1_smallk(const float* x, const float* w, float* y, int B, int C, int O, int HW, cips_stream_t stream);
int cips_conv1x1_smallk_bwd_data(const float* dy, const float* w, float* dx, int B, int C, int O, int HW,
                                 cips_stream_t stream);
int cips_conv1x1_smallk_bwd_weight_splits(int O, int HW);
int cips_conv1x1_smallk_bwd_weight(const float* dy, const float* x, float* part, int B, int C, int O, int HW,
                                   cips_stream_t stream);

int cips_im2col(const float* x, float* col, int B, int C, int H, int W,
                int kh, int kw, int stride, int pad, cips_stream_t stream);
int cips_im2col_x3(const float* x, void* col_hi, void* col_lo, int B, int C, int H, int W, int kh, int kw,
                   int stride, int pad, cips_stream_t stream);
int cips_col2im(const float* col, float* dx, int B, int C, int H, int W,
                int kh, int kw, int stride, int pad, cips_stream_t stream);

typedef struct cips_opt_tensor {
  float* param; const float* grad; float* exp_avg; float* exp_avg_sq; float* ema; long long n; long long step;
} cips_opt_tensor;
int cips_opt_chunk(void);
int cips_opt_step(const cips_opt_tensor* table_dev, const int* chunk_tensor_dev, const long long* chunk_off_dev,
                  int nchunks, double* partial_dev, float* total_norm_dev, float max_norm, float lr,
                  float beta1, float beta2, float eps, float ema_decay, int write_grad,
                  long long* steps_dev, cips_stream_t stream);

#ifdef __cplusplus
}
#endif
#endif
```

Measured before the change: 2040 img/s.

## Skip dfeat materialization in composite bwd and fuse mapping-net backward

Result: no change. 2053 img/s (median of 6 runs) (+0.7%).

```diff
diff --git a/cips3d_amd/_lib.py b/cips3d_amd/_lib.py
--- a/cips3d_amd/_lib.py
+++ b/cips3d_amd/_lib.py
@@ -29,6 +29,16 @@
 class GlinJob(C.Structure):
     _fields_ = [("x", vp), ("w", vp), ("bias", vp), ("y", vp), ("dy", vp), ("dw", vp), ("db", vp), ("in_dim", i32),
                 ("out_dim", i32)]
+
+
+MAPPING_MAX_LAYERS = 8
+
+
+class MappingBwdDesc(C.Structure):
+    _fields_ = [("x0", vp), ("stats", vp), ("dy", vp), ("dz", vp), ("w", vp * MAPPING_MAX_LAYERS),
+                ("act", vp * MAPPING_MAX_LAYERS), ("dw", vp * MAPPING_MAX_LAYERS), ("db", vp * MAPPING_MAX_LAYERS),
+                ("in_dim", i32 * MAPPING_MAX_LAYERS), ("out_dim", i32 * MAPPING_MAX_LAYERS),
+                ("lrelu", i32 * MAPPING_MAX_LAYERS), ("B", i32), ("layers", i32), ("slope", f32)]
 
 
 class GemmDesc(C.Structure):
@@ -110,6 +120,7 @@
     "cips_siren_bwd_x3": (i32, [C.POINTER(SirenWeights), vp, vp, vp, vp, vp, i32, i32, vp]),
     "cips_siren_fwd_x3_rays": (i32, [C.POINTER(SirenWeights), C.POINTER(RayParams), vp, vp, vp, i32, vp]),
     "cips_siren_bwd_x3_rays": (i32, [C.POINTER(SirenWeights), C.POINTER(RayParams), vp, vp, vp, vp, i32, vp]),
+    "cips_siren_bwd_x3_rays_w": (i32, [C.POINTER(SirenWeights), C.POINTER(RayParams), vp, vp, vp, vp, vp, i32, vp]),
     "cips_siren_bwd_x3_finalize": (i32, [C.POINTER(SirenWeights), vp, vp, i32, i32, C.POINTER(SirenGrads), vp]),
     "cips_march_fwd_x3": (i32, [C.POINTER(SirenWeights), C.POINTER(RayParams), vp, f32, i32, i32, vp, vp, vp, vp, vp, vp, i32, vp, vp, vp]),
     "cips_siren_bwd_data": (i32, [C.POINTER(SirenWeights)] + [vp] * 14 + [i32, i32, vp]),
@@ -117,6 +128,7 @@
     "cips_resample_fwd": (i32, [vp, vp, vp, f32, vp, vp, vp, vp, vp, vp, vp, vp, i32, i32, i32, i32, vp, C.POINTER(RayParams), vp]),
     "cips_composite_fwd": (i32, [vp, vp, vp, vp, vp, vp, vp, f32, vp, vp, vp, vp, vp, i32, i32, i32, i32, vp, vp, vp]),
     "cips_composite_bwd": (i32, [vp, vp, vp, vp, vp, vp, vp, f32, vp, vp, vp, vp, vp, vp, i32, i32, i32, i32, vp, vp]),
+    "cips_composite_bwd_w": (i32, [vp, vp, vp, vp, f32, vp, vp, vp, i32, i32, i32, i32, vp, vp]),
     "cips_gemm_f32": (i32, [C.POINTER(GemmDesc), vp]),
     "cips_gemm_bf16x3": (i32, [C.POINTER(GemmX3Desc), vp]),
     "cips_gemm_bf16x3_fuses_torgb": (i32, [C.POINTER(GemmX3Desc)]),
@@ -168,6 +180,7 @@
     "cips_grouped_linear_bwd": (i32, [C.POINTER(GlinJob), i32, i32, vp, vp, i64, vp]),
     "cips_rownorm_fwd": (i32, [vp, vp, vp, vp, vp, i32, i32, i32, f32, vp]),
     "cips_rownorm_bwd": (i32, [vp] * 9 + [i32, i32, i32, f32, vp]),
+    "cips_mapping_bwd": (i32, [C.POINTER(MappingBwdDesc), vp]),
     "cips_torgb_fwd": (i32, [vp, vp, vp, vp, i64, i32, i32, vp]),
     "cips_torgb_bwd_partials": (i32, [i64]),
     "cips_torgb_bwd_w": (i32, [vp, vp, vp, vp, vp, i64, i32, vp]),
diff --git a/cips3d_amd/csrc/render.hip b/cips3d_amd/csrc/render.hip
--- a/cips3d_amd/csrc/render.hip
+++ b/cips3d_amd/csrc/render.hip
@@ -153,6 +153,7 @@
   const int* order_in;
   const float* dfea;
   float *dfeat_c, *dsig_c, *dfeat_f, *dsig_f;
+  float* wsamp;
   long long R;
   int S, E, clamp_mode, flags;
   const unsigned char* clamp_pin;
@@ -343,8 +344,9 @@
       drow = a.dfeat_c + (ray * S + i) * 32;
       dsg = a.dsig_c + ray * S + i;
     }
-    if (active) *reinterpret_cast<float4*>(drow + 4 * sub) = make_float4(w * G.x, w * G.y, w * G.z, w * G.w);
+    if (active && !a.wsamp) *reinterpret_cast<float4*>(drow + 4 * sub) = make_float4(w * G.x, w * G.y, w * G.z, w * G.w);
     if ((k % SEG) == sub && active) {
+      if (a.wsamp) a.wsamp[ray * S + i] = w;
       const float delta = (k + 1 < E) ? (zall[k + 1] - zall[k]) : 1e10f;
       const float x = xs[k];
       float dens = clamp_density(x, a.clamp_mode);
@@ -437,3 +439,19 @@
   hipLaunchKernelGGL(composite_bwd_kernel, dim3(blocks), dim3(rpb * SEG), rpb * per_ray, (hipStream_t)stream, a);
   return CIPS_CHECK_LAUNCH();
 }
+
+extern "C" int cips_composite_bwd_w(const float* feat, const float* sigma, const float* z, const float* noise,
+                                    float noise_std, const float* dfea, float* w, float* dsigma, int R, int S,
+                                    int clamp_mode, int flags, const unsigned char* clamp_in, cips_stream_t stream) {
+  if (R <= 0 || S <= 0 || !feat || !sigma || !z || !dfea || !w || !dsigma) return (int)hipErrorInvalidValue;
+  CompArgs a = {};
+  a.feat_c = feat; a.sig_c = sigma; a.z_c = z; a.noise = noise; a.noise_std = noise_std; a.dfea = dfea;
+  a.wsamp = w; a.dsig_c = dsigma;
+  a.R = R; a.S = S; a.E = S; a.clamp_mode = clamp_mode; a.flags = flags;
+  a.clamp_pin = clamp_in; a.clamp_rec = nullptr;
+  size_t per_ray = (size_t)6 * a.E * sizeof(float);
+  int rpb = rays_per_block_for(per_ray);
+  int blocks = (R + rpb - 1) / rpb;
+  hipLaunchKernelGGL(composite_bwd_kernel, dim3(blocks), dim3(rpb * SEG), rpb * per_ray, (hipStream_t)stream, a);
+  return CIPS_CHECK_LAUNCH();
+}
diff --git a/cips3d_amd/csrc/siren_bwd_x3.hip b/cips3d_amd/csrc/siren_bwd_x3.hip
--- a/cips3d_amd/csrc/siren_bwd_x3.hip
+++ b/cips3d_amd/csrc/siren_bwd_x3.hip
@@ -327,6 +327,8 @@
   unsigned long long* prof;
   int dbg;
   RayGen rg;
+  const float* wsamp;
+  const float* dfea;
 };
 constexpr int GP_G1 = 0, GP_GC = H * H, GP_GF0 = GP_GC + HC * H, GP_GF1 = GP_GF0 + CF * HC, GPART = GP_GF1 + CF * HC;
 constexpr int SRED = 4 * 32 * 8 + 8;
@@ -768,28 +770,38 @@
 
 
 static int siren_bwd_x3_launch(const cips_siren_weights* w, const float* points, const cips_ray_params* rays,
-                               const float* dfeat, const float* dsigma, float* sred, float* gpart, int B, int P,
-                               cips_stream_t stream);
+                               const float* dfeat, const float* wsamp, const float* dfea, const float* dsigma, float* sred,
+                               float* gpart, int B, int P, cips_stream_t stream);
 
 extern "C" int cips_siren_bwd_x3(const cips_siren_weights* w, const float* points, const float* dfeat,
                                  const float* dsigma, float* sred, float* gpart, int B, int P,
                                  cips_stream_t stream) {
   if (!points) return (int)hipErrorInvalidValue;
-  return siren_bwd_x3_launch(w, points, nullptr, dfeat, dsigma, sred, gpart, B, P, stream);
+  return siren_bwd_x3_launch(w, points, nullptr, dfeat, nullptr, nullptr, dsigma, sred, gpart, B, P, stream);
 }
 
 extern "C" int cips_siren_bwd_x3_rays(const cips_siren_weights* w, const cips_ray_params* rays, const float* dfeat,
                                       const float* dsigma, float* sred, float* gpart, int B, cips_stream_t stream) {
   if (!rays) return (int)hipErrorInvalidValue;
-  return siren_bwd_x3_launch(w, nullptr, rays, dfeat, dsigma, sred, gpart, B, rays->W * rays->H * rays->S, stream);
+  return siren_bwd_x3_launch(w, nullptr, rays, dfeat, nullptr, nullptr, dsigma, sred, gpart, B, rays->W * rays->H * rays->S,
+                             stream);
+}
+
+extern "C" int cips_siren_bwd_x3_rays_w(const cips_siren_weights* w, const cips_ray_params* rays, const float* wsamp,
+                                        const float* dfea, const float* dsigma, float* sred, float* gpart, int B,
+                                        cips_stream_t stream) {
+  if (!rays || !wsamp || !dfea) return (int)hipErrorInvalidValue;
+  return siren_bwd_x3_launch(w, nullptr, rays, nullptr, wsamp, dfea, dsigma, sred, gpart, B, rays->W * rays->H * rays->S,
+                             stream);
 }
 
 static int siren_bwd_x3_launch(const cips_siren_weights* w, const float* points, const cips_ray_params* rays,
-                               const float* dfeat, const float* dsigma, float* sred, float* gpart, int B, int P,
-                               cips_stream_t stream) {
-  if (!w || !dfeat || !dsigma || !sred || !gpart || B <= 0 || P <= 0) return (int)hipErrorInvalidValue;
+                               const float* dfeat, const float* wsamp, const float* dfea, const float* dsigma, float* sred,
+                               float* gpart, int B, int P, cips_stream_t stream) {
+  const bool wg = wsamp != nullptr;
+  if (!w || (!dfeat && !wg) || !dsigma || !sred || !gpart || B <= 0 || P <= 0) return (int)hipErrorInvalidValue;
   BwdX3Args a;
-  a.w = *w; a.points = points; a.dfeat = dfeat; a.dsigma = dsigma; a.sred = sred; a.gpart = gpart;
+  a.w = *w; a.points = points; a.dfeat = dfeat; a.wsamp = wsamp; a.dfea = dfea; a.dsigma = dsigma; a.sred = sred; a.gpart = gpart;
   a.B = B; a.P = P;
   a.rg = RayGen{};
   if (!points) { const int rc = fill_raygen(a.rg, rays); if (rc) return rc; }
@@ -812,9 +824,15 @@
   if (!attr4) {
     hipFuncSetAttribute((const void*)siren_bwd_x4_kernel<false>, hipFuncAttributeMaxDynamicSharedMemorySize, SMEM_BYTES);
     hipFuncSetAttribute((const void*)siren_bwd_x4_kernel<true>, hipFuncAttributeMaxDynamicSharedMemorySize, SMEM_BYTES);
+    hipFuncSetAttribute((const void*)siren_bwd_x4_kernel<false, true>, hipFuncAttributeMaxDynamicSharedMemorySize, SMEM_BYTES);
+    hipFuncSetAttribute((const void*)siren_bwd_x4_kernel<true, true>, hipFuncAttributeMaxDynamicSharedMemorySize, SMEM_BYTES);
     attr4 = true;
   }
-  if (w->trig_mode & 1)
+  if (wg && (w->trig_mode & 1))
+    hipLaunchKernelGGL((siren_bwd_x4_kernel<true, true>), grid, dim3(256), SMEM_BYTES, (hipStream_t)stream, a);
+  else if (wg)
+    hipLaunchKernelGGL((siren_bwd_x4_kernel<false, true>), grid, dim3(256), SMEM_BYTES, (hipStream_t)stream, a);
+  else if (w->trig_mode & 1)
     hipLaunchKernelGGL(siren_bwd_x4_kernel<true>, grid, dim3(256), SMEM_BYTES, (hipStream_t)stream, a);
   else
     hipLaunchKernelGGL(siren_bwd_x4_kernel<false>, grid, dim3(256), SMEM_BYTES, (hipStream_t)stream, a);
diff --git a/cips3d_amd/csrc/siren_bwd_x4.inc b/cips3d_amd/csrc/siren_bwd_x4.inc
--- a/cips3d_amd/csrc/siren_bwd_x4.inc
+++ b/cips3d_amd/csrc/siren_bwd_x4.inc
@@ -9,7 +9,7 @@
   float s_, c_; sincos_reduced(reduce_2pi(x), &s_, &c_); return s_;
 }
 
-template <bool HW>
+template <bool HW, bool WG = false>
 __global__ __launch_bounds__(256, 1) void siren_bwd_x4_kernel(BwdX3Args a) {
   extern __shared__ __attribute__((aligned(1024))) uchar smem[];
   const int b = blockIdx.y;
@@ -87,10 +87,18 @@
     const unsigned m_dc = c7 == 6 ? ~0u : 0u, m_df = c7 == 7 ? ~0u : 0u;
 
     float4 df4[4];
+    float wsm = 0.f;
     {
       const int p = pbase + prow;
       const bool valid = p < cend;
-      const float* dp = a.dfeat + ((long long)b * a.P + (valid ? p : cend - 1)) * CF + 4 * hf;
+      const int pc = valid ? p : cend - 1;
+      const float* dp;
+      if (WG) {
+        dp = a.dfea + ((long long)b * a.rg.n + pc / a.rg.S) * CF + 4 * hf;
+        wsm = valid ? a.wsamp[(long long)b * a.P + pc] : 0.f;
+      } else {
+        dp = a.dfeat + ((long long)b * a.P + pc) * CF + 4 * hf;
+      }
 #pragma unroll
       for (int g = 0; g < 4; ++g) df4[g] = valid ? ld4(dp + 8 * g) : make_float4(0.f, 0.f, 0.f, 0.f);
     }
@@ -211,6 +219,10 @@
     Act<1> dfp;
 #pragma unroll
     for (int g = 0; g < 4; ++g) {
+      if (WG) {
+        df4[g].x *= wsm; df4[g].y *= wsm; df4[g].z *= wsm; df4[g].w *= wsm;
+        pinf(df4[g].x, df4[g].y, df4[g].z, df4[g].w);
+      }
       split2(df4[g].x, df4[g].y, dfp.hi[0][2 * g], dfp.lo[0][2 * g]);
       split2(df4[g].z, df4[g].w, dfp.hi[0][2 * g + 1], dfp.lo[0][2 * g + 1]);
     }
diff --git a/cips3d_amd/csrc/small_ops.hip b/cips3d_amd/csrc/small_ops.hip
--- a/cips3d_amd/csrc/small_ops.hip
+++ b/cips3d_amd/csrc/small_ops.hip
@@ -300,6 +300,96 @@
     b += g;
   }
   dgamma[c] = a; dbeta[c] = b;
+}
+
+constexpr int MB_T = 1024, MB_MAXB = 64, MB_MAXIN = 256, MB_MAXOUT = 128;
+constexpr size_t MB_SMEM = (size_t)(2 * MB_MAXB * MB_MAXOUT + MB_MAXB * MB_MAXIN) * sizeof(float);
+
+__global__ __launch_bounds__(MB_T) void mapping_bwd_kernel(cips_mapping_bwd_desc d) {
+  extern __shared__ __attribute__((aligned(16))) float sm[];
+  float* xb = sm + 2 * MB_MAXB * MB_MAXOUT;
+  const int t = threadIdx.x, B = d.B;
+  int cur = 0;
+  for (int l = d.layers - 1; l >= 0; --l) {
+    const int in = d.in_dim[l], out = d.out_dim[l], in4 = in >> 2, out4 = out >> 2;
+    float* g = sm + cur * (MB_MAXB * MB_MAXOUT);
+    const float* __restrict__ xin = l ? d.act[l - 1] : d.x0;
+    for (int i = t; i < B * out; i += MB_T) {
+      float v = (l == d.layers - 1) ? d.dy[i] : g[i];
+      if (d.lrelu[l]) v *= (d.act[l][i] > 0.f) ? 1.f : d.slope;
+      g[i] = v;
+    }
+    for (int i = t; i < B * in4; i += MB_T) reinterpret_cast<float4*>(xb)[i] = reinterpret_cast<const float4*>(xin)[i];
+    __syncthreads();
+    for (int tile = t; tile < out4 * in4; tile += MB_T) {
+      const int og = tile / in4, i4 = tile - og * in4;
+      float4 acc[4];
+#pragma unroll
+      for (int oo = 0; oo < 4; ++oo) acc[oo] = make_float4(0.f, 0.f, 0.f, 0.f);
+#pragma unroll 4
+      for (int b = 0; b < B; ++b) {
+        const float4 gv = reinterpret_cast<const float4*>(g + b * out)[og];
+        const float4 xv = reinterpret_cast<const float4*>(xb + b * in)[i4];
+        const float gg[4] = {gv.x, gv.y, gv.z, gv.w};
+#pragma unroll
+        for (int oo = 0; oo < 4; ++oo) {
+          acc[oo].x = fmaf(gg[oo], xv.x, acc[oo].x); acc[oo].y = fmaf(gg[oo], xv.y, acc[oo].y);
+          acc[oo].z = fmaf(gg[oo], xv.z, acc[oo].z); acc[oo].w = fmaf(gg[oo], xv.w, acc[oo].w);
+        }
+      }
+#pragma unroll
+      for (int oo = 0; oo < 4; ++oo) reinterpret_cast<float4*>(d.dw[l] + (long long)(4 * og + oo) * in)[i4] = acc[oo];
+    }
+    if (d.db[l] && t < out) {
+      float sb = 0.f;
+      for (int b = 0; b < B; ++b) sb += g[b * out + t];
+      d.db[l][t] = sb;
+    }
+    if (l == 0 && !d.dz) break;
+    __syncthreads();
+    float* gn = l ? sm + (cur ^ 1) * (MB_MAXB * MB_MAXOUT) : xb;
+    for (int tile = t; tile < ((B + 3) >> 2) * in4; tile += MB_T) {
+      const int bg = tile / in4, i4 = tile - bg * in4, b0 = 4 * bg;
+      const float* __restrict__ w = d.w[l];
+      float4 tot[4];
+      for (int o0 = 0; o0 < out; o0 += 16) {
+        const int o1 = min(out, o0 + 16);
+        float4 acc[4];
+#pragma unroll
+        for (int r = 0; r < 4; ++r) acc[r] = make_float4(0.f, 0.f, 0.f, 0.f);
+#pragma unroll 4
+        for (int o = o0; o < o1; ++o) {
+          const float4 wv = reinterpret_cast<const float4*>(w + (long long)o * in)[i4];
+#pragma unroll
+          for (int r = 0; r < 4; ++r) {
+            const float gg = (b0 + r < B) ? g[(b0 + r) * out + o] : 0.f;
+            acc[r].x = fmaf(gg, wv.x, acc[r].x); acc[r].y = fmaf(gg, wv.y, acc[r].y);
+            acc[r].z = fmaf(gg, wv.z, acc[r].z); acc[r].w = fmaf(gg, wv.w, acc[r].w);
+          }
+        }
+#pragma unroll
+        for (int r = 0; r < 4; ++r) {
+          if (o0 == 0) tot[r] = acc[r];
+          else { tot[r].x += acc[r].x; tot[r].y += acc[r].y; tot[r].z += acc[r].z; tot[r].w += acc[r].w; }
+        }
+      }
+#pragma unroll
+      for (int r = 0; r < 4; ++r)
+        if (b0 + r < B) reinterpret_cast<float4*>(gn + (b0 + r) * in)[i4] = tot[r];
+    }
+    __syncthreads();
+    cur ^= 1;
+    if (l == 0) {
+      const int cols = in, lane = t & 63, wave = t >> 6;
+      for (int b = wave; b < B; b += MB_T / 64) {
+        const float r = d.stats[2 * b + 1];
+        float s_ = 0.f;
+        for (int c = lane; c < cols; c += 64) s_ = fmaf(xb[b * cols + c], d.x0[b * cols + c], s_);
+        const float m = wave_sum_dpp(s_) / (float)cols;
+        for (int c = lane; c < cols; c += 64) d.dz[b * cols + c] = r * (xb[b * cols + c] - d.x0[b * cols + c] * m);
+      }
+    }
+  }
 }
 
 
@@ -423,6 +513,21 @@
   return CIPS_CHECK_LAUNCH();
 }
 
+extern "C" int cips_mapping_bwd(const cips_mapping_bwd_desc* d, cips_stream_t stream) {
+  if (!d || !d->x0 || !d->stats || !d->dy || d->B <= 0 || d->layers <= 0) return (int)hipErrorInvalidValue;
+  if (d->B > MB_MAXB || d->layers > CIPS_MAPPING_MAX_LAYERS) return (int)hipErrorNotSupported;
+  for (int l = 0; l < d->layers; ++l) {
+    if (!d->w[l] || !d->dw[l] || !d->act[l] || d->in_dim[l] <= 0 || d->out_dim[l] <= 0) return (int)hipErrorInvalidValue;
+    if ((d->in_dim[l] & 3) || (d->out_dim[l] & 3) || d->in_dim[l] > MB_MAXIN || d->out_dim[l] > MB_MAXOUT) return (int)hipErrorNotSupported;
+    if (l && d->in_dim[l] != d->out_dim[l - 1]) return (int)hipErrorInvalidValue;
+  }
+  static bool attr_set = false;
+  CIPS_PER_DEVICE(attr_set, false);
+  if (!attr_set) { (void)hipFuncSetAttribute((const void*)mapping_bwd_kernel, hipFuncAttributeMaxDynamicSharedMemorySize, (int)MB_SMEM); attr_set = true; }
+  hipLaunchKernelGGL(mapping_bwd_kernel, dim3(1), dim3(MB_T), MB_SMEM, (hipStream_t)stream, *d);
+  return CIPS_CHECK_LAUNCH();
+}
+
 namespace {
 __global__ __launch_bounds__(256) void eql_sum_chunks_kernel(const float* __restrict__ part, float* __restrict__ y, int nch, int n,
                                                              int O, const float* __restrict__ bias, float bias_scale) {
diff --git a/cips3d_amd/generator.py b/cips3d_amd/generator.py
--- a/cips3d_amd/generator.py
+++ b/cips3d_amd/generator.py
@@ -84,8 +84,12 @@
             self.add_module(name, head_net)
 
     def _base_hip(self, z):
+        mods = list(self.base_net)
+        if ops.mapping_base_fusable(mods, z):
+            lins = [(k, m) for k, m in enumerate(mods) if isinstance(m, nn.Linear)]
+            lrelu = tuple(k + 1 < len(mods) and isinstance(mods[k + 1], nn.LeakyReLU) for k, _ in lins)
+            return ops.MappingBaseFunction.apply(z, lrelu, *[p for _, m in lins for p in (m.weight, m.bias)])
         x = ops.RowNormFunction.apply(z, None, None, 4)
-        mods = list(self.base_net)
         i = 0
         while i < len(mods):
             m = mods[i]
diff --git a/cips3d_amd/ops.py b/cips3d_amd/ops.py
--- a/cips3d_amd/ops.py
+++ b/cips3d_amd/ops.py
@@ -177,9 +177,9 @@
         return (None,) + _siren_backward(t, dfeat, dsigma, B, P, points=points)
 
 
-def _siren_backward(t, dfeat, dsigma, B, P, points=None, rays=None):
-    lib = _lib.load()
-    dev = dfeat.device
+def _siren_backward(t, dfeat, dsigma, B, P, points=None, rays=None, wsamp_dfea=None):
+    lib = _lib.load()
+    dev = dsigma.device
     sw = _siren_struct(t)
     if True:
         if SIREN_BWD_MODE == "x3" or points is None:
@@ -191,6 +191,10 @@
             if points is not None:
                 check(lib.cips_siren_bwd_x3(C.byref(sw), _p(points), _p(dfeat), _p(dsigma), _p(sred), _p(gpart), B, P,
                                             _stream()), "cips_siren_bwd_x3")
+            elif wsamp_dfea is not None:
+                wsamp, dfea = wsamp_dfea
+                check(lib.cips_siren_bwd_x3_rays_w(C.byref(sw), C.byref(rays), _p(wsamp), _p(dfea), _p(dsigma), _p(sred),
+                                                   _p(gpart), B, _stream()), "cips_siren_bwd_x3_rays_w")
             else:
                 check(lib.cips_siren_bwd_x3_rays(C.byref(sw), C.byref(rays), _p(dfeat), _p(dsigma), _p(sred), _p(gpart), B,
                                                  _stream()), "cips_siren_bwd_x3_rays")
@@ -468,6 +472,78 @@
         return dx, dgamma, dbeta, None
 
 
+MAPPING_BWD_FUSED = True
+
+
+def mapping_base_fusable(mods, z):
+    from torch import nn
+    if not MAPPING_BWD_FUSED or z.shape[0] > 64 or z.shape[1] > 256:
+        return False
+    lins = [m for m in mods if isinstance(m, nn.Linear)]
+    if not lins or len(lins) > _lib.MAPPING_MAX_LAYERS or lins[0].in_features != z.shape[1]:
+        return False
+    prev = None
+    for m in mods:
+        if isinstance(m, nn.Linear):
+            if m.in_features % 4 or m.out_features % 4 or m.in_features > 256 or m.out_features > 128:
+                return False
+        elif isinstance(m, nn.LeakyReLU):
+            if not isinstance(prev, nn.Linear) or m.negative_slope != LRELU_SLOPE:
+                return False
+        else:
+            return False
+        prev = m
+    return True
+
+
+class MappingBaseFunction(torch.autograd.Function):
+
+    @staticmethod
+    def forward(ctx, z, lrelu, *wb):
+        lib = _lib.load()
+        z = _c(z.detach())
+        ws = [_c(w.detach()) for w in wb[0::2]]
+        bs = wb[1::2]
+        _chk(z, *ws)
+        rows, cols = z.shape
+        x0 = torch.empty_like(z)
+        stats = torch.empty(rows, 2, device=z.device)
+        check(lib.cips_rownorm_fwd(_p(z), None, None, _p(x0), _p(stats), rows, cols, 4, LRELU_SLOPE, _stream()),
+              "cips_rownorm_fwd")
+        x, acts = x0, []
+        for w, b, a in zip(ws, bs, lrelu):
+            x = GroupedLinearFunction.apply(x, w, b)[0]
+            if a:
+                x = RowNormFunction.apply(x, None, None, 2)
+            acts.append(x)
+        ctx.save_for_backward(x0, stats, *ws, *acts)
+        ctx.lrelu = tuple(lrelu)
+        ctx.has_bias = [b is not None for b in bs]
+        return x
+
+    @staticmethod
+    def backward(ctx, dy):
+        lib = _lib.load()
+        L = len(ctx.lrelu)
+        x0, stats = ctx.saved_tensors[:2]
+        ws, acts = ctx.saved_tensors[2:2 + L], ctx.saved_tensors[2 + L:]
+        dy = _c(dy)
+        d = _lib.MappingBwdDesc()
+        d.x0, d.stats, d.dy = _p(x0), _p(stats), _p(dy)
+        dz = torch.empty_like(x0) if ctx.needs_input_grad[0] else None
+        d.dz = _p(dz)
+        d.B, d.layers, d.slope = x0.shape[0], L, LRELU_SLOPE
+        out = [dz, None]
+        for l, (w, a) in enumerate(zip(ws, acts)):
+            dw = torch.empty_like(w)
+            db = torch.empty(w.shape[0], device=w.device) if ctx.has_bias[l] else None
+            d.w[l], d.act[l], d.dw[l], d.db[l] = _p(w), _p(a), _p(dw), _p(db)
+            d.in_dim[l], d.out_dim[l], d.lrelu[l] = w.shape[1], w.shape[0], 1 if ctx.lrelu[l] else 0
+            out += [dw, db]
+        check(lib.cips_mapping_bwd(C.byref(d), _stream()), "cips_mapping_bwd")
+        return tuple(out)
+
+
 MARCH_FUSED = True
 
 
@@ -570,14 +646,13 @@
         n = H * W
         R = B * n
         dfea = _c(dfea)
-        dfeat = torch.empty_like(feat)
+        wsamp = torch.empty_like(sigma)
         dsig = torch.empty_like(sigma)
-        check(lib.cips_composite_bwd(_p(feat), _p(sigma), _p(z), None, None, None, _p(noise), float(noise_std), None,
-                                     _p(dfea), _p(dfeat), _p(dsig), None, None, R, S, clamp_mode, flags, _p(ctx.clamp_mask),
-                                     _stream()), "cips_composite_bwd")
+        check(lib.cips_composite_bwd_w(_p(feat), _p(sigma), _p(z), _p(noise), float(noise_std), _p(dfea), _p(wsamp), _p(dsig),
+                                       R, S, clamp_mode, flags, _p(ctx.clamp_mask), _stream()), "cips_composite_bwd_w")
         _tail_gate_publish(dfea.device)
         rp = _ray_params(xg, yg, zg, zc, cam2world, jitter, H, W, S)
-        grads = _siren_backward(t, dfeat, dsig, B, n * S, rays=rp)
+        grads = _siren_backward(t, None, dsig, B, n * S, rays=rp, wsamp_dfea=(wsamp, dfea))
         return (None,) * 7 + grads
 
 
diff --git a/include/cips3d_hip.h b/include/cips3d_hip.h
--- a/include/cips3d_hip.h
+++ b/include/cips3d_hip.h
@@ -79,6 +79,10 @@
 int cips_siren_bwd_x3_rays(const cips_siren_weights* w, const cips_ray_params* rays, const float* dfeat,
                            const float* dsigma, float* sred, float* gpart, int B, cips_stream_t stream);
 
+int cips_siren_bwd_x3_rays_w(const cips_siren_weights* w, const cips_ray_params* rays, const float* wsamp,
+                             const float* dfea, const float* dsigma, float* sred, float* gpart, int B,
+                             cips_stream_t stream);
+
 int cips_march_fwd_x3(const cips_siren_weights* w, const cips_ray_params* rays, const float* noise, float noise_std,
                       int clamp_mode, int flags, float* fea, float* depth, float* weights, float* feat, float* sigma,
                       float* z, int B, const unsigned char* clamp_in, unsigned char* clamp_out, cips_stream_t stream);
@@ -103,6 +107,10 @@
                        const float* dfea,
                        float* dfeat_c, float* dsig_c, float* dfeat_f, float* dsig_f,
                        int R, int S, int clamp_mode, int flags, const unsigned char* clamp_in, cips_stream_t stream);
+
+int cips_composite_bwd_w(const float* feat, const float* sigma, const float* z, const float* noise, float noise_std,
+                         const float* dfea, float* w, float* dsigma,
+                         int R, int S, int clamp_mode, int flags, const unsigned char* clamp_in, cips_stream_t stream);
 
 typedef struct cips_gemm_desc {
   const float* A; const float* B; float* C;
@@ -254,6 +262,17 @@
                      float* dyhat, float* dgamma, float* dbeta, int rows, int cols, int mode, float slope,
                      cips_stream_t stream);
 
+#define CIPS_MAPPING_MAX_LAYERS 8
+typedef struct cips_mapping_bwd_desc {
+  const float* x0; const float* stats; const float* dy; float* dz;
+  const float* w[CIPS_MAPPING_MAX_LAYERS]; const float* act[CIPS_MAPPING_MAX_LAYERS];
+  float* dw[CIPS_MAPPING_MAX_LAYERS]; float* db[CIPS_MAPPING_MAX_LAYERS];
+  int in_dim[CIPS_MAPPING_MAX_LAYERS]; int out_dim[CIPS_MAPPING_MAX_LAYERS]; int lrelu[CIPS_MAPPING_MAX_LAYERS];
+  int B, layers;
+  float slope;
+} cips_mapping_bwd_desc;
+int cips_mapping_bwd(const cips_mapping_bwd_desc* d, cips_stream_t stream);
+
 int cips_torgb_fwd(const float* x, const float* w, const float* bias, float* rgb,
                    long long M, int K, int accumulate, cips_stream_t stream);
 int cips_torgb_bwd_partials(long long M);
```
